# lh3/psmc

Measured on AMD Instinct MI355X. Metric: genome bins/sec through forward-backward (n=64), higher is better.
Workload: dtype f64; 1 GPU; configs[2]: whole-genome .psmcfa-like batch, 30000001 bins x 64 states in 90 segments per GPU, -p 4+25*2+4+6, one E-step (EM iteration) per step, parameters of a different EM round every step; mode=fast, bins_per_gpu=30000001, bins_total=30000001, n_states=64, segments=90, longest_segment=2490000, tiles=8127, speculative_overlap_bins=3072, structured_sweeps=True, tile_bins=3712

## Files before the change

### psmc_amd/csrc/api.hip

```cpp
#include "psmc_hip_ctx.h"

static void destroy_kids(psmc_hip_ctx *c);

static int make_streams(psmc_hip_ctx *c)
{
	hipStream_t *st[5] = {&c->stream, &c->stream2, &c->stream3, &c->stream4, &c->stream5};
	for (hipStream_t *s : st) if (*s) { (void)hipStreamSynchronize(*s); (void)hipStreamDestroy(*s); *s = nullptr; }
	if (c->cu_count <= 0) {
		for (hipStream_t *s : st) if (hipStreamCreateWithFlags(s, hipStreamNonBlocking) != hipSuccess) return PSMC_HIP_EDEVICE;
		return 0;
	}
	int cus = 0;
	if (hipDeviceGetAttribute(&cus, hipDeviceAttributeMultiprocessorCount, c->device) != hipSuccess || cus <= 0) return PSMC_HIP_EDEVICE;
	if (c->cu_first < 0 || c->cu_first + c->cu_count > cus) return PSMC_HIP_EINVAL;
	std::vector<uint32_t> mask((size_t)(cus + 31) / 32, 0u);
	for (int i = c->cu_first; i < c->cu_first + c->cu_count; ++i) mask[(size_t)i >> 5] |= 1u << (i & 31);
	for (hipStream_t *s : st) if (hipExtStreamCreateWithCUMask(s, (uint32_t)mask.size(), mask.data()) != hipSuccess) return PSMC_HIP_EDEVICE;
	return 0;
}

extern "C" int psmc_hip_device_cus(int device)
{
	int cus = 0;
	if (hipDeviceGetAttribute(&cus, hipDeviceAttributeMultiprocessorCount, device) != hipSuccess) { (void)hipGetLastError(); return 0; }
// ... 29 lines not shown
extern "C" int psmc_hip_device_count(void)
{
	int n = 0;
	if (hipGetDeviceCount(&n) != hipSuccess) return 0;
	return n;
}

extern "C" const char *psmc_hip_strerror(int err)
{
	switch (err) {
	case PSMC_HIP_OK: return "ok";
	case PSMC_HIP_EINVAL: return "invalid argument";
	case PSMC_HIP_ENOMEM: return "out of memory";
	case PSMC_HIP_EDEVICE: return "HIP runtime error";
	case PSMC_HIP_ENOTSUP: return "not supported in this build";
	case PSMC_HIP_ESTATE: return "call order violated";
	case PSMC_HIP_ECONVERGE: return "fast-mode tile boundaries did not converge";
	default: return "unknown error";
	}
}
extern "C" const char *psmc_hip_last_error(const psmc_hip_ctx *ctx) { return ctx ? ctx->err.c_str() : ""; }

extern "C" int psmc_hip_create(psmc_hip_ctx **out, int n_states, int device, int mode)
{
	if (!out) return PSMC_HIP_EINVAL;
	*out = nullptr;
	if (n_states < 1) return PSMC_HIP_EINVAL;
	if (mode != PSMC_HIP_MODE_EXACT && mode != PSMC_HIP_MODE_FAST) return PSMC_HIP_EINVAL;
	if (n_states > PSMC_HIP_MAX_STATES) return PSMC_HIP_ENOTSUP;
	int nd = psmc_hip_device_count();
	if (nd <= 0 || device < 0 || device >= nd) return PSMC_HIP_EDEVICE;
	if (hipSetDevice(device) != hipSuccess) return PSMC_HIP_EDEVICE;
	psmc_hip_ctx *c = new (std::nothrow) psmc_hip_ctx();
	if (!c) return PSMC_HIP_ENOMEM;
	c->n = n_states; c->ns = n_states > 128 ? (n_states + 63) / 64 * 64 : (n_states > 64 ? 128 : 64); c->device = device; c->mode = mode;
	c->par_len = c->ns > 128 ? 2 * (size_t)c->ns * c->ns + 4 * (size_t)c->ns : psmc_hip_ctx::PAR_LEN;
	if (make_streams(c) != 0) { psmc_hip_destroy(c); return PSMC_HIP_EDEVICE; }
	for (int i = 0; i < 14; ++i)
		if (hipEventCreate(&c->evx[i]) != hipSuccess) { delete c; return PSMC_HIP_EDEVICE; }
	for (int i = 0; i < 10; ++i)
		if (hipEventCreate(&c->ev[i]) != hipSuccess) { delete c; return PSMC_HIP_EDEVICE; }
	if (hipHostMalloc((void **)&c->h_par, c->par_len * sizeof(double), hipHostMallocDefault) != hipSuccess ||
	    hipMalloc((void **)&c->d_par, c->par_len * sizeof(double)) != hipSuccess) {
		psmc_hip_destroy(c);
		return PSMC_HIP_ENOMEM;
	}
	if (const char *env = getenv("PSMC_HIP_OPTIONS")) {
		std::string all(env);
		size_t at = 0;
		while (at < all.size()) {
			size_t end = all.find(',', at);
			if (end == std::string::npos) end = all.size();
			const std::string kv = all.substr(at, end - at);
			const size_t eq = kv.find('=');
			at = end + 1;
			if (kv.empty()) continue;
			char *endp = nullptr;
			const double val = eq == std::string::npos ? 0.0 : strtod(kv.c_str() + eq + 1, &endp);
			const bool parsed = eq != std::string::npos && eq + 1 < kv.size() && endp && *endp == '\0';
			if (parsed && kv.compare(0, eq, "rccl") == 0) continue;
			if (!parsed || psmc_hip_set_option(c, kv.substr(0, eq).c_str(), val) != PSMC_HIP_OK) {
				fprintf(stderr, "[psmc_hip] PSMC_HIP_OPTIONS: bad entry \"%s\" (unknown key, value out of range, or not a number)\n", kv.c_str());
				psmc_hip_destroy(c);
				return PSMC_HIP_EINVAL;
			}
		}
	}
	*out = c;
	return PSMC_HIP_OK;
}

static void destroy_kids(psmc_hip_ctx *c)
{
	if (c->x_twin) { psmc_hip_destroy(c->x_twin); c->x_twin = nullptr; }
	for (psmc_hip_ctx *k : c->kids) psmc_hip_destroy(k);
	c->kids.clear();
	c->share_T = 0;
}

extern "C" void psmc_hip_destroy(psmc_hip_ctx *c)
{
	if (!c) return;
	(void)hipSetDevice(c->device);
	destroy_kids(c);
	if (c->parent) {
		void *mine[] = {c->d_seg_off, c->d_seg_len, c->d_work, c->d_chunks, c->d_entry, c->d_bexit, c->d_Cpart, c->d_Epart, c->d_LLpart,
		                c->d_stage, c->d_stats, c->d_warm, c->d_bentry, c->d_dirty, c->d_cnt, c->d_gate, c->d_queue, c->d_touch, c->d_items, c->d_ftiles, c->d_Kcol,
		                c->d_segA, c->d_segE, c->d_segA0, c->d_chk};
		for (void *p : mine) if (p) (void)hipFree(p);
		if (c->h_cnt) (void)hipHostFree(c->h_cnt);
		if (c->h_ritems) (void)hipHostFree(c->h_ritems);
		if (c->h_mlen) (void)hipHostFree(c->h_mlen);
		if (c->h_chunks) (void)hipHostFree(c->h_chunks);
		if (c->h_mis) (void)hipHostFree(c->h_mis);
		if (c->d_prevx) (void)hipFree(c->d_prevx);
		if (c->d_finv) (void)hipFree(c->d_finv);
		delete c;
		return;
	}
	if (c->stream) (void)hipStreamSynchronize(c->stream);
	free_wide_fast(c);
	if (c->stream2) (void)hipStreamSynchronize(c->stream2);
	if (c->stream3) (void)hipStreamSynchronize(c->stream3);
	if (c->stream4) (void)hipStreamSynchronize(c->stream4);
	if (c->stream5) (void)hipStreamSynchronize(c->stream5);
	if (!c->obs_borrowed && c->d_obs) (void)hipFree(c->d_obs);
	void *ptrs[] = {c->d_seg_off, c->d_seg_len, c->d_work, c->d_par, c->d_f, c->d_b, c->d_s, c->d_segA, c->d_segE,
	                c->d_segA0, c->d_chk, c->d_chunks, c->d_entry, c->d_bexit, c->d_Cpart, c->d_Epart, c->d_LLpart,
	                c->d_stage, c->d_stats, c->d_warm, c->d_bentry, c->d_dirty, c->d_cnt, c->d_gate, c->d_queue, c->d_touch, c->d_sb, c->d_items, c->d_ftiles, c->d_Kcol,
	                c->d_bw_seg, c->d_bw_par, c->d_bw_tab, c->d_bpar, c->d_s_all, c->d_cu_mask, c->d_lkp, c->d_lkoff, c->d_b2};
	for (void *p : ptrs) if (p) (void)hipFree(p);
	if (c->h_par) (void)hipHostFree(c->h_par);
	if (c->h_cnt) (void)hipHostFree(c->h_cnt);
	if (c->h_ritems) (void)hipHostFree(c->h_ritems);
	if (c->h_mlen) (void)hipHostFree(c->h_mlen);
	if (c->h_chunks) (void)hipHostFree(c->h_chunks);
	if (c->h_mis) (void)hipHostFree(c->h_mis);
	if (c->d_prevx) (void)hipFree(c->d_prevx);
	if (c->d_finv) (void)hipFree(c->d_finv);
	for (int i = 0; i < 10; ++i) if (c->ev[i]) (void)hipEventDestroy(c->ev[i]);
	for (int i = 0; i < 14; ++i) if (c->evx[i]) (void)hipEventDestroy(c->evx[i]);
	if (c->stream4) (void)hipStreamDestroy(c->stream4);
	if (c->stream5) (void)hipStreamDestroy(c->stream5);
	if (c->stream2) (void)hipStreamDestroy(c->stream2);
	if (c->stream3) (void)hipStreamDestroy(c->stream3);
	if (c->stream) (void)hipStreamDestroy(c->stream);
	delete c;
}

extern "C" int psmc_hip_set_option(psmc_hip_ctx *c, const char *key, double v)
{
	if (!c || !key) return PSMC_HIP_EINVAL;
	std::string k(key);
	if (k == "batch_first") { if (v < 0 || v > 1e6) return PSMC_HIP_EINVAL; c->batch_first = (int)v; return PSMC_HIP_OK; }
	destroy_kids(c);
	if (k == "chunk") { if (v < 0) return PSMC_HIP_EINVAL; c->chunk = (int)v; c->plan_dirty = true; }
	else if (k == "warmup") { if (v < 0) return PSMC_HIP_EINVAL; c->warmup = (int)v; c->warmup_set = true; c->plan_dirty = true; }
	else if (k == "max_rounds") c->max_rounds = (int)v;
	else if (k == "structured") { c->struct_opt = v != 0 ? 1 : 0; }
	else if (k == "learn") { c->learn = v != 0 ? 1 : 0; }
	else if (k == "merge") { c->merge = v != 0 ? 1 : 0; c->plan_dirty = true; c->chunk_cap = 0; }
	else if (k == "adapt") { c->adapt = v != 0 ? 1 : 0; c->plan_dirty = true; c->chunk_cap = 0; }
	else if (k == "prev_start") { c->prev_start = v != 0 ? 1 : 0; c->prev_ok = false; c->plan_dirty = true; c->chunk_cap = 0; }
	else if (k == "warm_shift") { if (v < 0 || v > 4) return PSMC_HIP_EINVAL; c->warm_shift = (int)v; c->warm_shift_set = true; c->plan_dirty = true; }
	else if (k == "merge1") { if (v < -1 || v > 1) return PSMC_HIP_EINVAL; c->merge1 = (int)v; c->plan_dirty = true; }
	else if (k == "phase1") { if (v < -1 || v > 1) return PSMC_HIP_EINVAL; c->phase1 = (int)v; }
	else if (k == "phase1_waves") { if (v < 1 || v > 4) return PSMC_HIP_EINVAL; c->phase1_waves = (int)v; }
	else if (k == "lanes8") { if (v < -1 || v > 1) return PSMC_HIP_EINVAL; c->lanes8 = (int)v; }
	else if (k == "gap_tiles") { c->gap_tiles = v != 0 ? 1 : 0; c->plan_dirty = true; c->items_dirty = true; }
	else if (k == "coarse") { if (v < -1 || v > 16) return PSMC_HIP_EINVAL; c->coarse = (int)v; c->plan_dirty = true; c->items_dirty = true; }
	else if (k == "kc_sub") { if (v < 1 || v > 16) return PSMC_HIP_EINVAL; c->kc_sub = (int)v; c->kc_sub_set = true; c->plan_dirty = true; c->items_dirty = true; }
	else if (k == "two_phase") { if (v != -1 && v != 0 && v != 2) return PSMC_HIP_EINVAL; c->two_phase = (int)v; c->plan_dirty = true; c->items_dirty = true; }
	else if (k == "kc_min") { if (v < -1) return PSMC_HIP_EINVAL; c->kc_min = (int)v; c->items_dirty = true; }
	else if (k == "ckpt") { c->ckpt = v != 0 ? 1 : 0; }
	else if (k == "fuse") { c->fuse = v != 0 ? 1 : 0; c->plan_dirty = true; }
	else if (k == "fuse128") { if (v != 0 && v != 2) return PSMC_HIP_EINVAL; c->fuse128 = (int)v; c->plan_dirty = true; c->items_dirty = true; }
	else if (k == "group_cap") { if (v < 0) return PSMC_HIP_EINVAL; c->group_cap = (int)v; c->items_dirty = true; }
	else if (k == "share_learn") { c->share_learn = v != 0 ? 1 : 0; }
	else if (k == "exact_refwd") { if (v < -1 || v > 2) return PSMC_HIP_EINVAL; c->exact_refwd = (int)v; c->reserved_refwd = -1; c->reserved_cap = 0; if (c->d_b2) { (void)hipFree(c->d_b2); c->d_b2 = nullptr; c->b2_bins = c->b2_alloc = 0; } }
	else if (k == "batch_sort") { c->batch_sort = v != 0 ? 1 : 0; }
	else if (k == "batch_tailfill") c->batch_tailfill = v != 0;
	else if (k == "batch_major") c->batch_major = v != 0;
	else if (k == "batch_bins") { if (v < 0) return PSMC_HIP_EINVAL; c->batch_bins = (int64_t)v; }
	else if (k == "overlap") c->overlap = v != 0 ? 1 : 0;
	else if (k == "warm_tol") c->warm_tol = v;
	else if (k == "wide_fast") { if (v != 0 && v != 1) return PSMC_HIP_EINVAL; c->wide_fast = (int)v; }
	else if (k == "wide_decode") { if (v != 0 && v != 1) return PSMC_HIP_EINVAL; c->wide_decode = (int)v; }
	else if (k == "rep_impl") c->rep_impl = v < 0 ? -1 : (v != 0 ? 1 : 0);
	else return PSMC_HIP_EINVAL;
	return PSMC_HIP_OK;
}

int set_segments_common(psmc_hip_ctx *c, int n_seg, const int32_t *L)
{
	destroy_kids(c);
	c->reserved_refwd = -1; c->reserved_cap = 0;
	if (c->d_b2) { (void)hipFree(c->d_b2); c->d_b2 = nullptr; c->b2_bins = c->b2_alloc = 0; }
	c->n_seg = n_seg;
	c->L.assign(L, L + n_seg);
	int rc;
	if ((rc = dev_alloc(c, &c->d_seg_off, (size_t)n_seg))) return rc;
	if ((rc = dev_alloc(c, &c->d_seg_len, (size_t)n_seg))) return rc;
	HIPCHK(c, hipMemcpy(c->d_seg_off, c->off.data(), sizeof(int64_t) * n_seg, hipMemcpyHostToDevice));
	HIPCHK(c, hipMemcpy(c->d_seg_len, c->L.data(), sizeof(int32_t) * n_seg, hipMemcpyHostToDevice));
	std::vector<int32_t> all(n_seg);
	for (int i = 0; i < n_seg; ++i) all[i] = i;
	return psmc_hip_select(c, n_seg, all.data());
}

extern "C" int psmc_hip_load_segments(psmc_hip_ctx *c, int n_seg, const uint8_t *const *seq, const int32_t *L)
{
	if (!c || n_seg < 1 || !seq || !L) return fail(c, PSMC_HIP_EINVAL, "load_segments: bad argument");
	HIPCHK(c, hipSetDevice(c->device));
	c->off.resize(n_seg);
	int64_t tot = 0;
	for (int i = 0; i < n_seg; ++i) {
		if (L[i] < 1 || !seq[i]) return fail(c, PSMC_HIP_EINVAL, "load_segments: empty segment");
		c->off[i] = tot;
		tot += ((int64_t)L[i] + 63) & ~(int64_t)63;
	}
	c->total = tot;
	std::vector<uint8_t> host((size_t)tot + 256, 2);
	for (int i = 0; i < n_seg; ++i) {
		for (int32_t j = 0; j < L[i]; ++j)
			if (seq[i][j] > 2) return fail(c, PSMC_HIP_EINVAL, "load_segments: symbol outside {0,1,2}");
		memcpy(host.data() + c->off[i], seq[i], (size_t)L[i]);
	}
	if (!c->obs_borrowed && c->d_obs) { (void)hipFree(c->d_obs); }
	c->d_obs = nullptr; c->obs_borrowed = false;
	int rc;
	if ((rc = dev_alloc(c, &c->d_obs, host.size()))) return rc;
	HIPCHK(c, hipMemcpy(c->d_obs, host.data(), host.size(), hipMemcpyHostToDevice));
	return set_segments_common(c, n_seg, L);
}

extern "C" int psmc_hip_load_segments_device(psmc_hip_ctx *c, int n_seg, const void *d_obs, const int64_t *off,
                                             const int32_t *L)
{
	if (!c || n_seg < 1 || !d_obs || !off || !L) return fail(c, PSMC_HIP_EINVAL, "load_segments_device: bad argument");
	HIPCHK(c, hipSetDevice(c->device));
	int64_t end = 0;
	for (int i = 0; i < n_seg; ++i) {
		if (L[i] < 1 || (off[i] & 63) || off[i] < end) return fail(c, PSMC_HIP_EINVAL, "load_segments_device: bad layout");
		end = off[i] + (((int64_t)L[i] + 63) & ~(int64_t)63);
	}
	if (!c->obs_borrowed && c->d_obs) (void)hipFree(c->d_obs);
	c->d_obs = (uint8_t *)d_obs; c->obs_borrowed = true;
	c->off.assign(off, off + n_seg);
	c->total = end;
	return set_segments_common(c, n_seg, L);
}

extern "C" int psmc_hip_select(psmc_hip_ctx *c, int n_sel, const int32_t *idx)
{
	if (!c || n_sel < 1 || !idx) return fail(c, PSMC_HIP_EINVAL, "select: bad argument");
	if (c->n_seg < 1) return fail(c, PSMC_HIP_ESTATE, "select: no segments loaded");
	std::vector<int32_t> pos(c->n_seg, -1);
	c->sel.assign(idx, idx + n_sel);
	c->work.clear(); c->mult.clear(); c->sel2work.resize(n_sel);
	for (int i = 0; i < n_sel; ++i) {
		if (idx[i] < 0 || idx[i] >= c->n_seg) return fail(c, PSMC_HIP_EINVAL, "select: index out of range");
		if (pos[idx[i]] < 0) { pos[idx[i]] = (int32_t)c->work.size(); c->work.push_back(idx[i]); c->mult.push_back(0); }
		c->sel2work[i] = pos[idx[i]];
		c->mult[pos[idx[i]]]++;
	}
	HIPCHK(c, hipSetDevice(c->device));
	int rc;
	if ((rc = dev_alloc(c, &c->d_work, c->work.size()))) return rc;
	HIPCHK(c, hipMemcpy(c->d_work, c->work.data(), sizeof(int32_t) * c->work.size(), hipMemcpyHostToDevice));
	c->plan_dirty = true;
	++c->sel_serial;
	return PSMC_HIP_OK;
}

bool factor_structure(int n, int S, const double *a , double *sp )
{
	double *P = sp, *R = sp + S, *qa = sp + 2 * S, *cc = sp + 3 * S, *dd = sp + 4 * S;
	memset(sp, 0, 5 * (size_t)S * sizeof(double));
	if (n < 3) return false;
	const double pl = a[(n - 1) * S + 0], pu = a[0 * S + (n - 1)];
	if (!(pl > 1e-280) || !(pu > 1e-280)) return false;
	for (int l = 0; l < n - 1; ++l) qa[l] = a[(n - 1) * S + l] / pl;
	for (int k = 1; k < n; ++k) P[k] = a[k * S + 0];
	for (int l = 1; l < n; ++l) cc[l] = a[0 * S + l] / pu;
	for (int k = 0; k < n - 1; ++k) R[k] = a[k * S + (n - 1)];
	const double tol = 64 * 2.220446049250313e-16;
	for (int k = 0; k < n; ++k) {
		for (int l = 0; l < n; ++l) {
			if (l == k) continue;
			const double v = a[k * S + l], w = l < k ? P[k] * qa[l] : R[k] * cc[l];
			if (!(fabs(v - w) <= tol * fabs(v) + 1e-290)) return false;
		}
		dd[k] = a[k * S + k] - P[k] * qa[k] - R[k] * cc[k];
		if (!(dd[k] >= 0.0)) return false;
	}
	return true;
}

static void fill_kcc(int S, const double *sp, const double *e3 , double *out )
{
	const double *P = sp, *R = sp + S, *qa = sp + 2 * S, *cv = sp + 3 * S, *dd = sp + 4 * S;
	for (int dir = 0; dir < 2; ++dir) {
		double *t = out + (size_t)dir * 11 * S;
		const double *mS = dir == 0 ? P : cv, *wS = dir == 0 ? qa : R, *mP = dir == 0 ? R : qa, *wP = dir == 0 ? cv : P;
		for (int k = 0; k < S; ++k) { t[k] = mS[k]; t[S + k] = mP[k]; }
		for (int sy = 0; sy < 3; ++sy)
			for (int k = 0; k < S; ++k) {
				const double ev = e3[sy * S + k];
				double *u = t + 2 * S + (size_t)sy * 3 * S;
				u[k] = wS[k] * ev; u[S + k] = wP[k] * ev; u[2 * S + k] = dd[k] * ev;
			}
	}
}

bool fill_params(const psmc_hip_ctx *c, const double *a, const double *e, const double *a0, double *dst)
{
	const int n = c->n;
	if (c->ns > 128) {
		const size_t S = (size_t)c->ns;
		double *pa = dst, *pt = pa + S * S, *pe = pt + S * S, *pa0 = pe + 3 * S;
		memset(pa, 0, c->par_len * sizeof(double));
		for (int k = 0; k < n; ++k) {
			for (int l = 0; l < n; ++l) { pa[k * S + l] = a[(size_t)k * n + l]; pt[l * S + k] = a[(size_t)k * n + l]; }
			pe[k] = e[k]; pe[S + k] = e[n + k];
			pa0[k] = a0[k];
		}
// ... 298 lines not shown
```

### psmc_amd/csrc/api_batch.hip

```cpp
#include "psmc_hip_ctx.h"

namespace {
struct RepSel { std::vector<int32_t> work, sel2work; int64_t bins = 0; };
}

static int batch_selections(psmc_hip_ctx *c, int n_rep, const int32_t *sel_off, const int32_t *sel_idx, std::vector<RepSel> &reps)
{
	std::vector<int32_t> pos(c->n_seg);
	reps.assign(n_rep, RepSel());
	for (int r = 0; r < n_rep; ++r) {
		const int n_sel = sel_off[r + 1] - sel_off[r];
		if (n_sel < 1) return fail(c, PSMC_HIP_EINVAL, "estep_batch: empty selection");
		std::fill(pos.begin(), pos.end(), -1);
		RepSel &R = reps[r];
		R.sel2work.resize(n_sel);
		for (int i = 0; i < n_sel; ++i) {
			const int32_t sg = sel_idx[sel_off[r] + i];
			if (sg < 0 || sg >= c->n_seg) return fail(c, PSMC_HIP_EINVAL, "estep_batch: index out of range");
			if (pos[sg] < 0) { pos[sg] = (int32_t)R.work.size(); R.work.push_back(sg); R.bins += ((int64_t)c->L[sg] + 63) & ~(int64_t)63; }
			R.sel2work[i] = pos[sg];
		}
	}
	return 0;
}
// ... 225 lines not shown
		}
		if (c->bpar_cap < (size_t)n_rep) { if ((rc = dev_alloc(c, &c->d_bpar, (size_t)n_rep * PL))) return rc; c->bpar_cap = (size_t)n_rep; }
		if (refwd && !c->d_cu_mask && (rc = dev_alloc(c, &c->d_cu_mask, (size_t)4096))) return rc;
		size_t lk_worst = 0;
		for (int g = 0; g < n_launches; ++g) {
			size_t t = 0;
			for (int i = l_first[g]; i < l_first[g + 1]; ++i) t += wseg[i] >= 0 ? (size_t)(c->L[wseg[i]] / LKP_DIV + LKP_MIN) : 1;
			lk_worst = std::max(lk_worst, t);
		}
		if (c->lkp_cap < lk_worst) { if ((rc = dev_alloc(c, &c->d_lkp, lk_worst))) return rc; c->lkp_cap = lk_worst; }
		if (c->lkoff_cap < worst_entries) { if ((rc = dev_alloc(c, &c->d_lkoff, worst_entries))) return rc; c->lkoff_cap = worst_entries; }
		if (fwd_all && c->s_all_cap < (size_t)all_bins + 128) { if ((rc = dev_alloc(c, &c->d_s_all, (size_t)all_bins + 128))) return rc; c->s_all_cap = (size_t)all_bins + 128; }
	}
	static const bool dbg_t = getenv("PSMC_HIP_DEBUG_TIMES") != nullptr;
	auto now = []() { return dbg_now(); };
	{
		std::vector<double> hp((size_t)n_rep * PL);
		for (int r = 0; r < n_rep; ++r) (void)fill_params(c, a + (size_t)r * n * n, e + (size_t)r * 2 * n, a0 + (size_t)r * n, hp.data() + (size_t)r * PL);
		HIPCHK(c, hipStreamSynchronize(c->stream));
		HIPCHK(c, hipMemcpyAsync(c->d_bw_seg, wseg.data(), sizeof(int32_t) * n_all, hipMemcpyHostToDevice, c->stream));
		HIPCHK(c, hipMemcpyAsync(c->d_bw_par, wpar.data(), sizeof(int32_t) * n_all, hipMemcpyHostToDevice, c->stream));
		HIPCHK(c, hipMemcpyAsync(c->d_bw_tab, wtab.data(), sizeof(int64_t) * n_all, hipMemcpyHostToDevice, c->stream));
		HIPCHK(c, hipMemcpyAsync(c->d_bw_tab + n_all, wtab_s.data(), sizeof(int64_t) * n_all, hipMemcpyHostToDevice, c->stream));
		HIPCHK(c, hipMemcpyAsync(c->d_bpar, hp.data(), sizeof(double) * hp.size(), hipMemcpyHostToDevice, c->stream));
		HIPCHK(c, hipStreamSynchronize(c->stream));
	}
	c->tables_batch = true;
	double fwd_all_s = 0.0;
	if (fwd_all) {
		const double t0 = now();
		EstepLaunch p;
		fill_common(c, p, c->stream, c->d_bpar);
		p.d_work = c->d_bw_seg; p.n_work = n_all; p.d_work_par = c->d_bw_par; p.d_work_tab = c->d_bw_tab + n_all; p.par_stride = (int64_t)PL; p.work_align = align;
		p.exact_refwd = 1; p.exact_only = 1; p.d_s = c->d_s_all;
		if (launch_exact(p) != 0) return fail(c, PSMC_HIP_EDEVICE, "launch_exact (batch, forward pass of all entries)", hipGetLastError());
		if (dbg_t) { (void)hipStreamSynchronize(c->stream); fwd_all_s = now() - t0; }
	}
	if ((double)n_all * (double)(S * S) * 8.0 > 16e9) {
		c->err = "estep_batch: the per-entry statistics of this call (" + std::to_string(n_all) + " entries x " + std::to_string(S) + "^2 doubles) need more than 16 GB of host memory: send fewer replicates per call at this many states";
		return PSMC_HIP_ENOMEM;
	}
	c->h_segA.resize((size_t)n_all * S * S); c->h_segE.resize((size_t)n_all * 3 * S);
	std::vector<double> lk_all((size_t)n_all, 0.0);
	std::vector<int> last_launch(n_rep, 0);
	{
		std::vector<int> launch_of((size_t)n_all, 0);
		for (int g = 0; g < n_launches; ++g) for (int i = l_first[g]; i < l_first[g + 1]; ++i) launch_of[i] = g;
		for (int r = 0; r < n_rep; ++r) for (int w : ent_of[r]) if (w >= 0) last_launch[r] = std::max(last_launch[r], launch_of[w]);
	}
	std::vector<double> sA((size_t)n * n), sE((size_t)2 * n);
	double t_sums = 0.0;
	auto finalize = [&](int r) {
		const RepSel &R = reps[r];
		std::fill(sA.begin(), sA.end(), 0.0); std::fill(sE.begin(), sE.end(), 0.0);
		double ll = 0.0;
		for (size_t i = 0; i < R.sel2work.size(); ++i) {
			const int w = ent_of[r][R.sel2work[i]];
			const double *hA = &c->h_segA[(size_t)w * S * S], *hE = &c->h_segE[(size_t)w * 3 * S];
			ll += lk_all[(size_t)w];
			for (int k = 0; k < n; ++k)
				for (int l = 0; l < n; ++l) sA[(size_t)k * n + l] += hA[k * S + l];
			for (int b = 0; b < 2; ++b)
				for (int l = 0; l < n; ++l) sE[(size_t)b * n + l] += hE[b * S + l];
		}
		if (A) memcpy(A + (size_t)r * n * n, sA.data(), sizeof(double) * n * n);
		if (E) memcpy(E + (size_t)r * 2 * n, sE.data(), sizeof(double) * 2 * n);
		if (LL) LL[r] = ll;
		if (sums) {
			double *q = sums + (size_t)r * 5 * n;
			memset(q, 0, sizeof(double) * 5 * n);
			for (int k = 0; k < n; ++k)
				for (int l = 0; l < n; ++l) {
					const double v = sA[(size_t)k * n + l];
					if (l < k) { q[k] += v; q[3 * n + l] += v; } else if (l > k) { q[n + k] += v; q[4 * n + l] += v; } else q[2 * n + k] = v;
				}
		}
	};
	std::vector<int32_t> finished;
	for (int g = 0; g < n_launches; ++g) {
		const double t_a = now();
		const int e0 = l_first[g], nw = l_first[g + 1] - e0;
		int64_t run = 0; int32_t longest = 0;
		for (int i = e0; i < e0 + nw; ++i) if (wseg[i] >= 0) { run = std::max(run, wtab[i] + padded_len(wseg[i])); longest = std::max(longest, c->L[wseg[i]]); }
		EstepLaunch p;
		fill_common(c, p, c->stream, c->d_bpar);
		p.d_work = c->d_bw_seg + e0; p.n_work = nw; p.d_work_par = c->d_bw_par + e0; p.d_work_tab = c->d_bw_tab + e0; p.par_stride = (int64_t)PL; p.work_align = align;
		p.exact_refwd = refwd ? (c->exact_refwd == 1 ? 1 : 2) : 0;
		p.d_cu_mask = c->d_cu_mask;
		if (fwd_all) { p.exact_only = 2; p.d_work_tab_s = c->d_bw_tab + n_all + e0; p.d_s = c->d_s_all; }
		p.d_segA = c->d_segA; p.d_segE = c->d_segE; p.d_segA0 = c->d_segA0; p.d_chk = c->d_chk;
		const double t_b = now();
		if (launch_exact(p) != 0) return fail(c, PSMC_HIP_EDEVICE, "launch_exact (batch)", hipGetLastError());
		if (dbg_t) (void)hipStreamSynchronize(c->stream);
		const double t_c = now();
		std::vector<int64_t> lkoff((size_t)nw);
		int64_t lk_tot = 0;
		for (int i = 0; i < nw; ++i) { lkoff[i] = lk_tot; lk_tot += wseg[e0 + i] >= 0 ? c->L[wseg[e0 + i]] / LKP_DIV + LKP_MIN : 1; }
		HIPCHK(c, hipMemcpyAsync(c->d_lkoff, lkoff.data(), sizeof(int64_t) * nw, hipMemcpyHostToDevice, c->stream));
		if (launch_lk_products(c->stream, p, fwd_all ? c->d_s_all : c->d_s, c->d_lkoff, c->d_lkp) != 0) return fail(c, PSMC_HIP_EDEVICE, "launch_lk_products", hipGetLastError());
		c->h_lkp.resize((size_t)lk_tot);
		HIPCHK(c, hipMemcpyAsync(c->h_segA.data() + (size_t)e0 * S * S, c->d_segA, sizeof(double) * nw * S * S, hipMemcpyDeviceToHost, c->stream));
		HIPCHK(c, hipMemcpyAsync(c->h_segE.data() + (size_t)e0 * 3 * S, c->d_segE, sizeof(double) * nw * 3 * S, hipMemcpyDeviceToHost, c->stream));
		HIPCHK(c, hipMemcpyAsync(c->h_lkp.data(), c->d_lkp, sizeof(double) * (size_t)lk_tot, hipMemcpyDeviceToHost, c->stream));
		HIPCHK(c, hipStreamSynchronize(c->stream));
		const double t_d = now();
		collect_timing(c);
		int n_over = 0;
		for (int i = 0; i < nw; ++i) {
			if (wseg[e0 + i] < 0) continue;
			const int32_t sg = wseg[e0 + i];
			const double *q = &c->h_lkp[(size_t)lkoff[i]];
			const int cnt = (int)q[0], cap_i = c->L[sg] / LKP_DIV + LKP_MIN;
			if (cnt >= 1 && cnt < cap_i) {
				double sum = 0.0;
				for (int j = 1; j <= cnt; ++j) sum += log(q[j]);
				lk_all[(size_t)e0 + i] = sum;
			} else {
				++n_over;
				c->h_s.resize((size_t)c->L[sg]);
				HIPCHK(c, hipMemcpyAsync(c->h_s.data(), (fwd_all ? c->d_s_all + wtab_s[e0 + i] : c->d_s + wtab[e0 + i]), sizeof(double) * (size_t)c->L[sg], hipMemcpyDeviceToHost, c->stream));
				HIPCHK(c, hipStreamSynchronize(c->stream));
				lk_all[(size_t)e0 + i] = host_lk(c->h_s.data(), c->L[sg]);
			}
		}
		if (dbg_t && n_over) fprintf(stderr, "[psmc_hip] batch launch %d: %d entries logged more products than their buffer holds (host hmm_lk)\n", g, n_over);
		if (dbg_t) fprintf(stderr, "[psmc_hip] batch launch %d: %d entries (longest %d bins), %.1f M table bins | prepare %.3f s, kernels %.3f (fwd %.0f bwd %.0f expect %.0f ms%s), read-back %.3f, hmm_lk %.3f\n",
		                   g, nw, (int)longest, run / 1e6, t_b - t_a, t_c - t_b, c->last_ms[1], c->last_ms[2], c->last_ms[3],
		                   fwd_all ? (g == 0 ? (std::string("; forward pass of all entries ") + std::to_string(fwd_all_s) + " s").c_str() : "; fwd: see launch 0") : "", t_d - t_c, now() - t_d);
		++c->last_batch_groups;
		const double t_f = now();
		finished.clear();
		for (int r = 0; r < n_rep; ++r) if (last_launch[r] == g) { finalize(r); finished.push_back(r); }
		t_sums += now() - t_f;
		if (done && !finished.empty()) done(user, (int)finished.size(), finished.data());
	}
	if (dbg_t) {
		std::string per;
		for (int g = 0; g < n_launches; ++g) per += (g ? " " : "") + std::to_string(std::count(last_launch.begin(), last_launch.end(), g));
		fprintf(stderr, "[psmc_hip] batch: %d replicates, %d entries in %d launches (replicates complete after launch 0..: %s), host sums %.3f s\n", n_rep, n_all, n_launches, per.c_str(), t_sums);
	}
	return PSMC_HIP_OK;
}

static psmc_hip_ctx *batch_child(psmc_hip_ctx *c, int r)
{
	while ((int)c->kids.size() <= r) {
		psmc_hip_ctx *k = new (std::nothrow) psmc_hip_ctx();
		if (!k) return nullptr;
		k->n = c->n; k->ns = c->ns; k->device = c->device; k->mode = c->mode; k->parent = c;
		k->chunk = c->chunk > 0 ? c->chunk : c->share_T;
		k->warmup = c->warmup; k->max_rounds = c->max_rounds; k->rep_impl = c->rep_impl;
		k->n_sub = c->n_sub; k->target_waves = c->target_waves; k->overlap = c->overlap; k->warm_tol = c->warm_tol; k->struct_opt = c->struct_opt;
		k->struct_tiles_set = c->struct_tiles_set; k->struct_tiles = c->struct_tiles;
		k->two_phase = c->two_phase; k->kc_div = c->kc_div; k->kc_min = c->kc_min; k->ckpt = c->ckpt; k->fuse = c->fuse;
		k->learn = c->learn; k->group_cap = c->group_cap; k->warm_shift = c->warm_shift; k->kc_sub = c->kc_sub; k->kcol_prio = c->kcol_prio;
		k->fuse128 = c->fuse128; k->coarse = c->coarse; k->gate = c->gate; k->lanes8 = c->lanes8; k->gap_tiles = c->gap_tiles; k->exact_refwd = c->exact_refwd;
		k->merge = c->merge; k->adapt = c->adapt; k->prev_start = c->prev_start;
		k->merge1 = c->merge1; k->merge_order = c->merge_order; k->runs_late = c->runs_late; k->warm_shift_set = c->warm_shift_set; k->kc_sub_set = c->kc_sub_set;
		k->stream = c->stream; k->stream2 = c->stream2; k->stream3 = c->stream3; k->stream4 = c->stream4; k->stream5 = c->stream5;
		for (int i = 0; i < 14; ++i) k->evx[i] = c->evx[i];
		for (int i = 0; i < 10; ++i) k->ev[i] = c->ev[i];
		k->h_par = c->h_par; k->d_par = c->d_par; k->par_len = c->par_len;
		k->d_obs = c->d_obs; k->obs_borrowed = true; k->off = c->off; k->total = c->total;
		if (set_segments_common(k, c->n_seg, c->L.data()) != 0) { c->err = k->err; psmc_hip_destroy(k); return nullptr; }
		c->kids.push_back(k);
	}
	return c->kids[r];
}

static int batch_exact_once(psmc_hip_ctx *c, int r, const int32_t *idx, int n_sel, const double *a, const double *e, const double *a0,
                            double *A, double *sums, double *E, double *LL, const char *why)
{
	const int n = c->n;
	fprintf(stderr, "[psmc_hip] replicate %d: fast E-step did not converge (%s); repeating this E-step with the exact kernels\n", c->batch_first + r, why);
	int rc = 0;
	if (!c->x_twin) {
		if ((rc = psmc_hip_create(&c->x_twin, n, c->device, PSMC_HIP_MODE_EXACT))) return fail(c, rc, "estep_batch: cannot create the exact twin context");
		if ((rc = psmc_hip_load_segments_device(c->x_twin, c->n_seg, c->d_obs, c->off.data(), c->L.data()))) {
			c->err = "exact twin: " + c->x_twin->err; psmc_hip_destroy(c->x_twin); c->x_twin = nullptr; return rc;
		}
	}
	std::vector<double> Af;
	double *Ao = A;
	if (!Ao) { Af.resize((size_t)n * n); Ao = Af.data(); }
	if ((rc = psmc_hip_select(c->x_twin, n_sel, idx)) || (rc = psmc_hip_estep(c->x_twin, a, e, a0, Ao, E, nullptr, LL, nullptr))) { c->err = "exact twin: " + c->x_twin->err; return rc; }
	if (sums) {
		memset(sums, 0, sizeof(double) * 5 * (size_t)n);
		for (int k = 0; k < n; ++k)
			for (int l = 0; l < n; ++l) {
				const double v = Ao[(size_t)k * n + l];
				if (l < k) { sums[k] += v; sums[3 * n + l] += v; } else if (l > k) { sums[n + k] += v; sums[4 * n + l] += v; } else sums[2 * n + k] = v;
			}
	}
	++c->n_exact_fallbacks;
	return PSMC_HIP_OK;
}

static int batch_fast(psmc_hip_ctx *c, int n_rep, const double *a, const double *e, const double *a0, const int32_t *sel_off,
                      const int32_t *sel_idx, double *A, double *sums, double *E, double *LL, psmc_hip_batch_done_fn done, void *user)
{
	const int n = c->n;
	if (c->share_T == 0 && c->share_learn) {
		int T = c->chunk;
		if (T <= 0) {
			std::vector<RepSel> reps;
			int rc0 = batch_selections(c, n_rep, sel_off, sel_idx, reps);
			if (rc0) return rc0;
			int64_t most = 0; size_t nw = 1;
			for (const RepSel &R : reps) {
				int64_t bins = 0;
				for (int32_t sg : R.work) bins += c->L[sg];
				if (bins > most) { most = bins; nw = R.work.size(); }
			}
			T = auto_tile_len(c, most, nw, true);
		}
		c->share_T = T;
		c->sh_glue_f.assign(c->n_seg, {}); c->sh_glue_b.assign(c->n_seg, {}); c->sh_wf.assign(c->n_seg, {}); c->sh_wb.assign(c->n_seg, {});
		for (int sg = 0; sg < c->n_seg; ++sg) {
			const size_t nt = ((size_t)c->L[sg] + T - 1) / T;
			c->sh_glue_f[sg].assign(nt, 0); c->sh_glue_b[sg].assign(nt, 0); c->sh_wf[sg].assign(nt, c->warmup); c->sh_wb[sg].assign(nt, c->warmup);
		}
	}
	static const bool dbg_t = getenv("PSMC_HIP_DEBUG_TIMES") != nullptr;
	const double t_call = dbg_now();
	double t_est = 0.0;
	for (int r = 0; r < n_rep; ++r) {
		const double t_k = dbg_now();
		psmc_hip_ctx *k = batch_child(c, c->batch_first + r);
		c->dbg_acc[0] += dbg_now() - t_k;
		if (!k) return fail(c, PSMC_HIP_ENOMEM, "estep_batch: cannot create the replicate context");
		const int n_sel = sel_off[r + 1] - sel_off[r];
		if (n_sel < 1) return fail(c, PSMC_HIP_EINVAL, "estep_batch: empty selection");
		const int32_t *idx = sel_idx + sel_off[r];
		int rc = 0;
		{
			const double t_s = dbg_now();
			if ((int)k->sel.size() != n_sel || memcmp(k->sel.data(), idx, sizeof(int32_t) * n_sel) != 0) rc = psmc_hip_select(k, n_sel, idx);
			c->dbg_acc[1] += dbg_now() - t_s;
		}
		const double t_e = dbg_now();
		const double *ar = a + (size_t)r * n * n, *er = e + (size_t)r * 2 * n, *a0r = a0 + (size_t)r * n;
		if (rc == 0) {
			double *Ar = A ? A + (size_t)r * n * n : nullptr, *Sr = sums ? sums + (size_t)r * 5 * n : nullptr, *Er = E ? E + (size_t)r * 2 * n : nullptr, *Lr = LL ? LL + r : nullptr;
			if (A) rc = psmc_hip_estep(k, ar, er, a0r, Ar, Er, nullptr, Lr, nullptr);
			if (rc == 0 && sums) rc = psmc_hip_estep_factored(k, ar, er, a0r, Sr, Er, Lr);
			if (rc == PSMC_HIP_ECONVERGE) rc = batch_exact_once(c, r, idx, n_sel, ar, er, a0r, Ar, Sr, Er, Lr, k->err.c_str());
		}
		t_est += dbg_now() - t_e;
		if (rc) { c->err = "replicate " + std::to_string(r) + ": " + k->err; return rc; }
		if (done) { const int32_t rr = r; done(user, 1, &rr); }
	}
	if (dbg_t) {
		const double *q = c->dbg_acc;
		fprintf(stderr, "[psmc_hip] fast batch on device %d: %d replicates %.3f s | contexts %.3f, select %.3f, E-steps %.3f (plan %.3f, items %.3f, launches %.3f, rest %.3f); "
		                "%.0f repair rounds, %.0f repaired tiles\n", c->device, n_rep, dbg_now() - t_call, q[0], q[1], t_est, q[2], q[3], q[4], t_est - q[2] - q[3] - q[4], q[6], q[7]);
		for (double &v : c->dbg_acc) v = 0.0;
	}
	c->tables_batch = true;
	c->last_batch_groups = n_rep;
	return PSMC_HIP_OK;
}

extern "C" int psmc_hip_estep_batch(psmc_hip_ctx *c, int n_rep, const double *a, const double *e, const double *a0,
                                    const int32_t *sel_off, const int32_t *sel_idx, double *A, double *sums, double *E, double *LL)
{
	return psmc_hip_estep_batch_cb(c, n_rep, a, e, a0, sel_off, sel_idx, A, sums, E, LL, nullptr, nullptr);
}

extern "C" int psmc_hip_estep_batch_cb(psmc_hip_ctx *c, int n_rep, const double *a, const double *e, const double *a0,
                                       const int32_t *sel_off, const int32_t *sel_idx, double *A, double *sums, double *E, double *LL,
                                       psmc_hip_batch_done_fn done, void *user)
{
	if (!c || n_rep < 1 || !a || !e || !a0 || !sel_off || !sel_idx || (!A && !sums)) return fail(c, PSMC_HIP_EINVAL, "estep_batch: bad argument");
	if (c->parent) return fail(c, PSMC_HIP_EINVAL, "estep_batch: not on a replicate context");
	if (c->n_seg < 1) return fail(c, PSMC_HIP_ESTATE, "estep_batch: no segments loaded");
	HIPCHK(c, hipSetDevice(c->device));
	c->wd_kind = WD_NONE;
	if (c->mode == PSMC_HIP_MODE_EXACT || c->ns > 128) return batch_exact(c, n_rep, a, e, a0, sel_off, sel_idx, A, sums, E, LL, done, user);
	return batch_fast(c, n_rep, a, e, a0, sel_off, sel_idx, A, sums, E, LL, done, user);
}

extern "C" int psmc_hip_batch_info(psmc_hip_ctx *c, int out[2])
{
	if (!c || !out) return PSMC_HIP_EINVAL;
	out[0] = c->last_batch_groups; out[1] = (int)c->kids.size();
	return PSMC_HIP_OK;
}
```

### psmc_amd/csrc/api_fast.hip

```cpp
#include "psmc_hip_ctx.h"

int ensure_fast_buffers(psmc_hip_ctx *c)
{
	if (c->d_stage && c->d_stats && c->d_warm && c->d_cnt && c->h_cnt && c->d_gate) return 0;
	int rc;
	const size_t sl = (size_t)c->ns * c->ns + 3 * (size_t)c->ns + 1;
	if ((rc = dev_alloc(c, &c->d_stage, (size_t)RED_ROWS * sl))) return rc;
	if ((rc = dev_alloc(c, &c->d_stats, sl))) return rc;
	if ((rc = dev_alloc(c, &c->d_warm, (size_t)2))) return rc;
	if ((rc = dev_alloc(c, &c->d_cnt, (size_t)4))) return rc;
	if ((rc = dev_alloc(c, &c->d_gate, (size_t)4))) return rc;
	if (!c->h_cnt && (hipHostMalloc((void **)&c->h_cnt, 4 * sizeof(int), hipHostMallocMapped) != hipSuccess ||
	                  hipHostGetDevicePointer((void **)&c->m_cnt, c->h_cnt, 0) != hipSuccess)) {
		c->h_cnt = nullptr;
		return fail(c, PSMC_HIP_ENOMEM, "hipHostMalloc (mapped)");
	}
	return 0;
}

int auto_tile_len(const psmc_hip_ctx *c, int64_t bins, size_t n_work, bool st)
{
	const int64_t ROUND1 = 4096;
	int64_t want = st ? c->struct_tiles : c->target_waves;
	if (st && !c->struct_tiles_set && bins < 2 * ROUND1 * (int64_t)std::max(c->warmup, 1))
		want = std::max<int64_t>(ROUND1 - (int64_t)n_work, ROUND1 / 2);
	const int T = (int)((bins + want - 1) / want);
	return std::max(256, (T + 63) & ~63);
}

static int plan_fast(psmc_hip_ctx *c)
{
	int64_t bins = 0;
	for (int32_t s : c->work) bins += c->L[s];
	int T = c->chunk;
	const bool st = c->use_struct;
	const int64_t ROUND1 = 4096;
	bool one_round = false;
	if (T <= 0) T = auto_tile_len(c, bins, c->work.size(), st);
	c->chunks.clear(); c->chunk_seg.clear(); c->chunk_idx.clear();
	for (size_t w = 0; w < c->work.size(); ++w) {
		const int32_t s = c->work[w];
		for (int32_t lo = 1; lo <= c->L[s]; lo += T) {
			c->chunk_seg.push_back(s); c->chunk_idx.push_back((lo - 1) / T);
			Chunk ch;
			ch.off = c->off[s]; ch.L = c->L[s]; ch.lo = lo; ch.hi = std::min(c->L[s], lo + T - 1); ch.mult = c->mult[w];
			ch.flags = 0; ch.wf = ch.wb = c->warmup;
			if (ch.lo - c->warmup <= 1) ch.flags |= CHUNK_ANCHOR_F;
			if ((int64_t)ch.hi + c->warmup + 1 >= ch.L) ch.flags |= CHUNK_ANCHOR_B;
			if (ch.hi == ch.L) ch.flags |= CHUNK_LAST;
			c->chunks.push_back(ch);
		}
	}
	const int nc = (int)c->chunks.size();
	c->chunk_used = T;
	c->planned_struct = st;
	one_round = st && nc <= ROUND1;
	c->two_phase_used = c->two_phase >= 0 ? c->two_phase : (one_round ? 0 : 2);
	c->merge1_used = c->merge1 >= 0 ? c->merge1 : (one_round ? 1 : 0);
	c->warm_shift_used = c->warm_shift_set ? c->warm_shift : (one_round ? 0 : 1);
	c->coarse_used = c->coarse >= 0 ? std::max(c->coarse, 1) : (one_round && nc > 2048 && T < c->warmup ? 2 : 1);
	c->kc_sub_used = c->kc_sub_set ? c->kc_sub : std::max(1, std::min(4, (int)((8 * (int64_t)T + T + c->warmup - 1) / std::max(T + c->warmup, 1))));
	c->n_sub_used = st ? (fused_counts(c) ? 1 : std::max(1, std::min(c->n_sub, (9216 + nc - 1) / std::max(nc, 1)))) : c->n_sub;
	c->glue_f.assign(nc, 0); c->glue_b.assign(nc, 0);
	if (c->parent && c->parent->share_T == T && st) {
		const psmc_hip_ctx *P = c->parent;
		for (int b = 0; b < nc; ++b) {
			const int sg = c->chunk_seg[b], ix = c->chunk_idx[b];
			if (sg >= (int)P->sh_glue_f.size() || ix >= (int)P->sh_glue_f[sg].size()) continue;
			c->glue_f[b] = P->sh_glue_f[sg][ix]; c->glue_b[b] = P->sh_glue_b[sg][ix];
			c->chunks[b].wf = std::max(c->chunks[b].wf, P->sh_wf[sg][ix]); c->chunks[b].wb = std::max(c->chunks[b].wb, P->sh_wb[sg][ix]);
		}
	}
	c->items_dirty = true;
	int rc;
	c->gap.assign(nc, 0);
	if (nc > c->chunk_cap) {
		if ((rc = dev_alloc(c, &c->d_chunks, (size_t)nc))) return rc;
		if ((rc = dev_alloc(c, &c->d_entry, (size_t)nc * c->ns))) return rc;
		if ((rc = dev_alloc(c, &c->d_bexit, (size_t)(nc + 1) * c->ns))) return rc;
		if ((rc = dev_alloc(c, &c->d_bentry, (size_t)nc * c->ns))) return rc;
		if ((rc = dev_alloc(c, &c->d_dirty, (size_t)2 * nc))) return rc;
		if ((rc = dev_alloc(c, &c->d_touch, (size_t)3 * nc))) return rc;
		if ((rc = dev_alloc(c, &c->d_finv, (size_t)nc))) return rc;
		if (c->h_mlen) { (void)hipHostFree(c->h_mlen); c->h_mlen = nullptr; c->m_mlen = nullptr; }
		if (c->h_mis) { (void)hipHostFree(c->h_mis); c->h_mis = nullptr; c->m_mis = nullptr; }
		if (c->prev_start && (rc = dev_alloc(c, &c->d_prevx, (size_t)nc * c->ns))) return rc;
		if ((c->merge || c->adapt) &&
		    (hipHostMalloc((void **)&c->h_mlen, (size_t)nc * sizeof(int), hipHostMallocMapped) != hipSuccess ||
		     hipHostGetDevicePointer((void **)&c->m_mlen, c->h_mlen, 0) != hipSuccess ||
		     hipHostMalloc((void **)&c->h_mis, (size_t)2 * nc * sizeof(double), hipHostMallocMapped) != hipSuccess ||
		     hipHostGetDevicePointer((void **)&c->m_mis, c->h_mis, 0) != hipSuccess))
			return fail(c, PSMC_HIP_ENOMEM, "hipHostMalloc (mapped)");
		if ((rc = dev_alloc(c, &c->d_LLpart, (size_t)nc))) return rc;
		if ((rc = dev_alloc(c, &c->d_items, (size_t)32 * nc + 64))) return rc;
		if ((rc = dev_alloc(c, &c->d_ftiles, (size_t)2 * (nc + 16)))) return rc;
		if (c->h_ritems) { (void)hipHostFree(c->h_ritems); c->h_ritems = nullptr; }
		if (hipHostMalloc((void **)&c->h_ritems, (size_t)4 * nc * sizeof(int), hipHostMallocMapped) != hipSuccess ||
		    hipHostGetDevicePointer((void **)&c->m_ritems, c->h_ritems, 0) != hipSuccess)
			return fail(c, PSMC_HIP_ENOMEM, "hipHostMalloc (mapped)");
		c->chunk_cap = nc;
	}
	if ((rc = dev_alloc(c, &c->d_Epart, (size_t)nc * c->n_sub_used * 3 * c->ns))) return rc;
	if ((rc = ensure_fast_buffers(c))) return rc;
	HIPCHK(c, hipMemcpy(c->d_chunks, c->chunks.data(), sizeof(Chunk) * nc, hipMemcpyHostToDevice));
	if (st && c->gap_tiles) {
		std::vector<int> fl(nc, 0);
		if (launch_tile_allmiss(c->stream, c->d_obs, c->d_chunks, nc, c->d_dirty) != 0) return fail(c, PSMC_HIP_EDEVICE, "k_tile_allmiss", hipGetLastError());
		HIPCHK(c, hipMemcpyAsync(fl.data(), c->d_dirty, sizeof(int) * nc, hipMemcpyDeviceToHost, c->stream));
		HIPCHK(c, hipMemsetAsync(c->d_dirty, 0, sizeof(int) * nc, c->stream));
		HIPCHK(c, hipStreamSynchronize(c->stream));
		for (int b = 0; b < nc; ++b) {
			const Chunk &ch = c->chunks[b];
			c->gap[b] = fl[b] && ch.lo > 1 && ch.hi < ch.L && ch.hi - ch.lo + 1 == T;
		}
		auto same = [&](int x, int y) { return x >= 0 && y < nc && c->chunks[x].off == c->chunks[y].off; };
		for (int b = 0; b < nc; ++b) {
			if (c->gap[b]) { if (same(b - 1, b)) c->glue_f[b] = 1; if (same(b, b + 1)) c->glue_b[b] = 1; }
			if (b > 0 && c->gap[b - 1] && same(b - 1, b)) c->glue_f[b] = 1;
			if (b + 1 < nc && c->gap[b + 1] && same(b, b + 1)) c->glue_b[b] = 1;
		}
	}
	c->plan_dirty = false; c->chunks_dirty = false; c->prev_ok = false;
	return 0;
}

static int build_items(psmc_hip_ctx *c, bool two_phase_bwd, int coarse)
{
	const int nc = (int)c->chunks.size(), W = c->warmup;
	const int cf = std::max(1, coarse), cb = two_phase_bwd ? 1 : cf;
	std::vector<int> odd(nc, 0), idx(nc, 0);
	for (int b = 1; b < nc; ++b) if (c->chunks[b].off == c->chunks[b - 1].off) { odd[b] = !odd[b - 1]; idx[b] = idx[b - 1] + 1; }
	std::vector<std::pair<long long, std::pair<int, int>>> kf, kb;
	auto key = [](int steps, bool run, bool phase_b) { return (run ? -(1ll << 40) : (phase_b ? (1ll << 40) : 0ll)) - steps; };
	std::vector<char> from_above(nc, 0), in_run(nc, 0), in_run_f(nc, 0), in_run_b(nc, 0);
	std::vector<std::pair<int, int>> gf, gb;
	auto same_seg = [&](int x, int y) { return c->chunks[x].off == c->chunks[y].off; };
	const bool gaps = c->gap_tiles && (int)c->gap.size() == nc;
	std::vector<int64_t> eff(nc + 1, 0);
	for (int b = 0; b < nc; ++b) eff[b + 1] = eff[b] + ((gaps && c->gap[b]) ? 0 : c->chunks[b].hi - c->chunks[b].lo + 1);
	auto span_ok = [&](int b, int e) { return eff[e + 1] - eff[b] <= (int64_t)c->group_cap; };
	for (int b = 0; b < nc;) {
		int e = b + 1;
		while (e < nc && c->glue_f[e] && same_seg(e, b) && span_ok(b, e)) ++e;
		if (e - b > 1) for (int t = b; t < e; ++t) in_run[t] = in_run_f[t] = 1;
		else
			while (e < nc && e - b < cf && same_seg(e, b) && idx[e] % cf != 0 && !c->glue_f[e] && !(e + 1 < nc && c->glue_f[e + 1] && same_seg(e + 1, e))) ++e;
		gf.push_back({b, e - b});
		b = e;
	}
	for (int b = 0; b < nc;) {
		int e = b + 1;
		while (e < nc && c->glue_b[e - 1] && same_seg(e, b) && span_ok(b, e) &&
		       c->chunks[e].lo < c->chunks[e].L)
			++e;
		if (e - b > 1) for (int t = b; t < e; ++t) in_run[t] = in_run_b[t] = 1;
		else
			while (e < nc && e - b < cb && same_seg(e, b) && idx[e] % cb != 0 && !c->glue_b[e - 1] && !(e + 1 < nc && c->glue_b[e] && same_seg(e + 1, e)) &&
			       c->chunks[e].lo < c->chunks[e].L)
				++e;
		gb.push_back({b, e - b});
		b = e;
	}
	int n_run = 0;
	for (int b = 0; b < nc; ++b) n_run += in_run[b];
	const int cap_b = (nc + 7) / 8 * 4;
	c->runs_in_b = two_phase_bwd && c->runs_late && n_run > 0 && n_run <= cap_b / 2;
	int above_budget = c->runs_in_b ? cap_b - n_run : nc;
	for (const auto &gr : gb) {
		const int b = gr.first, e = b + gr.second;
		const Chunk &lo = c->chunks[b], &top = c->chunks[e - 1];
		bool pb = two_phase_bwd && e - b == 1 && odd[b] && b + 1 < nc && c->chunks[b + 1].off == lo.off && c->chunks[b + 1].lo < c->chunks[b + 1].L;
		if (pb && c->runs_in_b && (in_run[b] || in_run[b + 1] || above_budget <= 0)) pb = false;
		if (pb) { from_above[b] = 1; --above_budget; }
		kb.push_back({key(std::min(top.hi + chunk_warm_b(top, W) + 1, top.L) - lo.lo, in_run_b[b] != 0, pb), {b, e - b}});
	}
	std::vector<int> la, lb;
	{
		std::vector<int> freet;
		for (int b = 0; b < nc; ++b) {
			if (from_above[b]) lb.push_back(b | (1 << 30));
			else if (b > 0 && from_above[b - 1]) la.push_back(b);
			else if (c->runs_in_b && in_run[b]) lb.push_back(b);
			else freet.push_back(b);
		}
		const bool single = lb.empty() && nc <= 4096;
		for (int b : freet) { if (single || la.size() <= lb.size()) la.push_back(b); else lb.push_back(b); }
	}
	for (const auto &gr : gf) {
		const int b = gr.first, e = b + gr.second;
		const Chunk &h = c->chunks[b], &l = c->chunks[e - 1];
		kf.push_back({key(l.hi - std::max(1, h.lo - chunk_warm_f(h, W)) + 1, in_run_f[b] != 0, false), {b, e - b}});
	}
	std::sort(kf.begin(), kf.end()); std::sort(kb.begin(), kb.end());
	std::vector<int> h((size_t)4 * nc, 0), mem((size_t)4 * nc, 0);
	c->n_mem_f = c->n_mem_b = 0;
	for (size_t i = 0; i < kf.size(); ++i) {
		h[2 * i] = kf[i].second.first; h[2 * i + 1] = kf[i].second.second;
		if (in_run_f[kf[i].second.first])
			for (int t = 0; t < kf[i].second.second; ++t) { mem[2 * (size_t)c->n_mem_f] = kf[i].second.first + t; mem[2 * (size_t)c->n_mem_f + 1] = 1; ++c->n_mem_f; }
	}
	for (size_t i = 0; i < kb.size(); ++i) {
		h[(size_t)2 * nc + 2 * i] = kb[i].second.first; h[(size_t)2 * nc + 2 * i + 1] = kb[i].second.second;
		if (in_run_b[kb[i].second.first])
			for (int t = 0; t < kb[i].second.second; ++t) {
				mem[(size_t)2 * nc + 2 * (size_t)c->n_mem_b] = kb[i].second.first + t; mem[(size_t)2 * nc + 2 * (size_t)c->n_mem_b + 1] = 1; ++c->n_mem_b;
			}
	}
	c->n_items_f = (int)kf.size(); c->n_items_b = (int)kb.size();
	c->order_f.clear();
	for (const auto &it : kf) if (!in_run_f[it.second.first]) c->order_f.push_back(it.second.first);
	c->n_long_f = c->n_long_b = 0;
	while (c->n_long_f < c->n_items_f && in_run_f[kf[c->n_long_f].second.first]) ++c->n_long_f;
	while (c->n_long_b < c->n_items_b && in_run_b[kb[c->n_long_b].second.first]) ++c->n_long_b;
	c->n_B_b = 0;
	for (int b = 0; b < nc; ++b) c->n_B_b += from_above[b];
	{
		c->n_list_a = (int)la.size(); c->n_list_b = (int)lb.size();
		c->count_group = c->ns == 128 && c->fuse128 == 2 ? 16 : 4;
		while (la.size() % c->count_group) la.push_back(-1);
		while (lb.size() % c->count_group) lb.push_back(-1);
		la.insert(la.end(), lb.begin(), lb.end());
		if (!la.empty()) HIPCHK(c, hipMemcpy(c->d_ftiles, la.data(), sizeof(int) * la.size(), hipMemcpyHostToDevice));
	}
	c->items_two_phase = two_phase_bwd ? 2 : 0; c->items_coarse = coarse;
	HIPCHK(c, hipMemcpy(c->d_items, h.data(), sizeof(int) * h.size(), hipMemcpyHostToDevice));
	{
		std::vector<int> sg;
		for (size_t i = (size_t)c->n_long_b; i < kb.size(); ++i)
			for (int t = kb[i].second.second - 1; t >= 0; --t) { sg.push_back(kb[i].second.first + t); sg.push_back(1); }
		c->n_singles_b = (int)sg.size() / 2;
		if (!sg.empty()) HIPCHK(c, hipMemcpy(c->d_items + (size_t)24 * nc, sg.data(), sizeof(int) * sg.size(), hipMemcpyHostToDevice));
	}
	HIPCHK(c, hipMemcpy(c->d_items + (size_t)8 * nc, mem.data(), sizeof(int) * mem.size(), hipMemcpyHostToDevice));
	{
		std::vector<int> fx;
		for (int b = 0; b < nc; ++b)
			if (!in_run_f[b] && !(b > 0 && in_run_f[b - 1] && same_seg(b - 1, b))) { fx.push_back(b); fx.push_back(1); }
		c->n_fix_f = (int)fx.size() / 2;
		if (!fx.empty()) HIPCHK(c, hipMemcpy(c->d_items + (size_t)30 * nc, fx.data(), sizeof(int) * fx.size(), hipMemcpyHostToDevice));
	}
	{
		const int n4f = c->n_items_f - c->n_long_f, n4b = c->n_items_b - c->n_long_b - c->n_B_b;
		std::vector<std::pair<long long, int>> qk;
		for (int k = 0; 4 * k < n4f; ++k) {
			long long st = 0;
			for (int i = c->n_long_f + 4 * k; i < std::min(c->n_long_f + 4 * k + 4, c->n_items_f); ++i) {
				const Chunk &h = c->chunks[kf[i].second.first], &l = c->chunks[kf[i].second.first + kf[i].second.second - 1];
				st = std::max(st, (long long)(l.hi - std::max(1, h.lo - chunk_warm_f(h, W)) + 1));
			}
			qk.push_back({-st * 504, 2 * k});
		}
		for (int k = 0; 4 * k < n4b; ++k) {
			long long st = 0;
			for (int i = c->n_long_b + 4 * k; i < std::min(c->n_long_b + 4 * k + 4, c->n_long_b + n4b); ++i) {
				const Chunk &lo = c->chunks[kb[i].second.first], &top = c->chunks[kb[i].second.first + kb[i].second.second - 1];
				const int q = std::min(top.hi + chunk_warm_b(top, W) + 1, top.L);
				st = std::max(st, (long long)(q - (coarse > 1 ? std::min(lo.hi, lo.L - 1) : std::min(top.hi, top.L - 1))));
			}
			qk.push_back({-st * 534, 2 * k + 1});
		}
		std::stable_sort(qk.begin(), qk.end(), [](const std::pair<long long, int> &x, const std::pair<long long, int> &y) { return x.first < y.first; });
		std::vector<int> qv(qk.size());
		for (size_t i = 0; i < qk.size(); ++i) qv[i] = qk[i].second;
		if (c->queue_cap < qv.size()) { int rc; if ((rc = dev_alloc(c, &c->d_queue, qv.size()))) return rc; c->queue_cap = qv.size(); }
		c->n_queue = (int)qv.size();
		if (!qv.empty()) HIPCHK(c, hipMemcpy(c->d_queue, qv.data(), sizeof(int) * qv.size(), hipMemcpyHostToDevice));
	}
	std::vector<int> wl((size_t)4 * nc, 0), kc, runs_f, runs_b, kslot, kuniq;
	int gap_slot[2] = {-1, -1};
	auto push_kc = [&](int t, int dir) {
		const int j = (int)kc.size() / 2;
		kc.push_back(t); kc.push_back(dir);
		if (gaps && c->gap[t] && c->chunk_used % 4 == 0) {
			if (gap_slot[dir] < 0) { gap_slot[dir] = (int)kuniq.size(); kuniq.push_back(j); }
			kslot.push_back(gap_slot[dir]);
		} else { kslot.push_back((int)kuniq.size()); kuniq.push_back(j); }
	};
	c->n_wl_f = c->n_wl_b = 0;
	const int kc_min = c->kc_min >= 0 ? c->kc_min : (c->ns == 128 ? (nc > 4096 ? 12 : 8) : (nc > 4096 ? 5 : 4));
	const bool chains = kc_min >= 2;
	const int head_count = c->ns == 64 ? 0 : 1;
	auto add_runs = [&](const std::vector<std::pair<long long, std::pair<int, int>>> &k, int n_long, bool bwd) {
		int &nw = bwd ? c->n_wl_b : c->n_wl_f;
		std::vector<int> &rv = bwd ? runs_b : runs_f;
		int *w = wl.data() + (bwd ? (size_t)2 * nc : 0);
		int budget = std::max(64, nc / c->kc_div);
		for (int i = 0; i < n_long; ++i) {
			int first = k[i].second.first, count = k[i].second.second;
			int cost = 0;
			for (int tt = first; tt < first + count; ++tt) cost += (gaps && c->gap[tt] && c->chunk_used % 4 == 0) ? 0 : 1;
			cost = std::max(cost - 1, 1);
			const bool chain = chains && count >= kc_min && cost <= budget;
			if (chain) budget -= cost;
			if (chain && !bwd && c->chunks[first].lo == 1) {
				w[2 * nw] = first; w[2 * nw + 1] = (head_count == 0 && count - 1 >= 2) ? -1 : 2; ++nw;
				first += 1; count -= 1;
				if (count >= 2) {
					rv.push_back(first); rv.push_back(count); rv.push_back((int)(kc.size() / 2)); rv.push_back(0);
					for (int t = first; t < first + count - 1; ++t) push_kc(t, 0);
				}
			} else if (chain) {
				w[2 * nw] = bwd ? first + count - 1 : first; w[2 * nw + 1] = head_count; ++nw;
				rv.push_back(first); rv.push_back(count); rv.push_back((int)(kc.size() / 2)); rv.push_back(0);
				if (!bwd) for (int t = first; t < first + count - 1; ++t) push_kc(t, 0);
				else for (int t = first + count - 1; t > first; --t) push_kc(t, 1);
			} else { w[2 * nw] = first; w[2 * nw + 1] = (head_count == 0 && !bwd) ? -(count - 1) : count; ++nw; }
		}
	};
	add_runs(kf, c->n_long_f, false);
	add_runs(kb, c->n_long_b, true);
	c->n_chain_f = (int)runs_f.size() / 4; c->n_chain_b = (int)runs_b.size() / 4; c->n_kc = (int)kc.size() / 2; c->n_kuniq = (int)kuniq.size();
	if ((size_t)c->n_kc > (size_t)2 * nc || (size_t)(c->n_chain_f + c->n_chain_b) > (size_t)nc) return fail(c, PSMC_HIP_ESTATE, "build_items: list overflow");
	HIPCHK(c, hipMemcpy(c->d_items + (size_t)12 * nc, wl.data(), sizeof(int) * wl.size(), hipMemcpyHostToDevice));
	if (c->n_kc > 0) {
		std::vector<int> runs(runs_f); runs.insert(runs.end(), runs_b.begin(), runs_b.end());
		HIPCHK(c, hipMemcpy(c->d_items + (size_t)16 * nc, kc.data(), sizeof(int) * kc.size(), hipMemcpyHostToDevice));
		HIPCHK(c, hipMemcpy(c->d_items + (size_t)20 * nc, runs.data(), sizeof(int) * runs.size(), hipMemcpyHostToDevice));
		HIPCHK(c, hipMemcpy(c->d_items + (size_t)26 * nc, kslot.data(), sizeof(int) * kslot.size(), hipMemcpyHostToDevice));
		HIPCHK(c, hipMemcpy(c->d_items + (size_t)28 * nc, kuniq.data(), sizeof(int) * kuniq.size(), hipMemcpyHostToDevice));
		const size_t nsub = kcol2_on(c) ? (size_t)c->kc_sub_used : 1;
		const size_t need = (size_t)c->n_kuniq * nsub * ((size_t)c->ns * c->ns + c->ns);
		if (need > c->kcol_cap) { int rc; if ((rc = dev_alloc(c, &c->d_Kcol, need))) return rc; c->kcol_cap = need; }
	}
	c->items_dirty = false;
	if (getenv("PSMC_HIP_DEBUG"))
		fprintf(stderr, "[psmc_hip] buffers: obs %p (+%lld) chunks %p (%d) items %p entry %p bentry %p bexit %p f %p b %p s %p sb %p Cpart %p Epart %p ftiles %p touch %p par %p Kcol %p\n",
		        (void *)c->d_obs, (long long)c->total + 256, (void *)c->d_chunks, nc, (void *)c->d_items, (void *)c->d_entry, (void *)c->d_bentry, (void *)c->d_bexit,
		        (void *)c->d_f, (void *)c->d_b, (void *)c->d_s, (void *)c->d_sb, (void *)c->d_Cpart, (void *)c->d_Epart, (void *)c->d_ftiles, (void *)c->d_touch, (void *)c->d_par, (void *)c->d_Kcol);
	if (getenv("PSMC_HIP_DEBUG"))
		fprintf(stderr, "[psmc_hip] items: %d tiles of %d bins, fwd %d items (%d runs, %d run tiles, %d walks, %d chains), bwd %d items (%d runs, %d run tiles, %d walks, %d chains, %d from above), %d transfer matrices, fused lists %d + %d\n",
		        nc, c->chunk_used, c->n_items_f, c->n_long_f, c->n_mem_f, c->n_wl_f, c->n_chain_f, c->n_items_b, c->n_long_b, c->n_mem_b, c->n_wl_b, c->n_chain_b, c->n_B_b, c->n_kc, c->n_list_a, c->n_list_b);
	return 0;
}

static void learn_groups(psmc_hip_ctx *c)
{
	const int nc = (int)c->chunks.size(), W = c->warmup;
	const int cap = W << c->warm_shift_used;
	for (int b : c->flagged_f)
		if (b > 0 && b < nc && !c->glue_f[b] && c->chunks[b - 1].off == c->chunks[b].off) {
			Chunk &ch = c->chunks[b];
			if (ch.wf < cap && ch.lo - ch.wf > 1) { ch.wf = std::min(cap, std::max(2 * ch.wf, W)); c->chunks_dirty = true; }
			else c->glue_f[b] = 1;
			c->items_dirty = true;
		}
	for (int b : c->flagged_b)
		if (b >= 0 && b + 1 < nc && !c->glue_b[b] && c->chunks[b + 1].off == c->chunks[b].off) {
			Chunk &ch = c->chunks[b];
			if (ch.wb < cap && (int64_t)ch.hi + ch.wb + 1 < ch.L) { ch.wb = std::min(cap, std::max(2 * ch.wb, W)); c->chunks_dirty = true; }
			else c->glue_b[b] = 1;
			c->items_dirty = true;
		}
	if (c->parent && c->parent->share_T == c->chunk_used && (!c->flagged_f.empty() || !c->flagged_b.empty())) {
		psmc_hip_ctx *P = c->parent;
		auto put = [&](int b) {
			if (b < 0 || b >= nc) return;
			const int sg = c->chunk_seg[b], ix = c->chunk_idx[b];
			if (sg >= (int)P->sh_glue_f.size() || ix >= (int)P->sh_glue_f[sg].size()) return;
			P->sh_glue_f[sg][ix] |= c->glue_f[b]; P->sh_glue_b[sg][ix] |= c->glue_b[b];
			P->sh_wf[sg][ix] = std::max(P->sh_wf[sg][ix], c->chunks[b].wf); P->sh_wb[sg][ix] = std::max(P->sh_wb[sg][ix], c->chunks[b].wb);
		};
		for (int b : c->flagged_f) put(b);
		for (int b : c->flagged_b) put(b);
	}
}

static void adapt_warmups(psmc_hip_ctx *c)
{
	const int nc = (int)c->chunks.size();
	const int cap = c->warmup << c->warm_shift_used, floor_w = std::min(c->warmup, 256);
	const double tol = c->warm_tol;
	bool changed = false;
	for (int b = 0; b < nc; ++b) {
		const double m = c->h_mis[b];
		if (!(m > 0.0)) continue;
		if (c->glue_f[b] || (b + 1 < nc && c->glue_f[b + 1] && c->chunks[b + 1].off == c->chunks[b].off)) continue;
		Chunk &ch = c->chunks[b];
		if (ch.lo - ch.wf <= 1) continue;
		int w = ch.wf;
		if (m > tol) {
			const int ml = c->h_mlen[b];
			w = std::min(std::max(cap, w), w + (ml > 0 ? 16 * ml + 64 : w));
		} else {
			const double slack = log10(tol / std::max(m, 1e-17)), keep = 2.0;
			if (slack > keep) w = std::max(floor_w, w - (((int)std::min((slack - keep) * 160.0, w / 8.0) + 15) & ~15));
		}
		if (w != ch.wf) { ch.wf = w; changed = true; }
	}
	if (changed) {
		c->chunks_dirty = true;
		int64_t total = 0, waste = 0;
		for (size_t i = 0; i + 3 < c->order_f.size(); i += 4) {
			int64_t s4 = 0, mx = 0;
			for (int r = 0; r < 4; ++r) { const Chunk &ch = c->chunks[c->order_f[i + r]]; const int64_t st = (int64_t)ch.hi - std::max(1, ch.lo - ch.wf) + 1; s4 += st; mx = std::max(mx, st); }
			total += 4 * mx; waste += 4 * mx - s4;
		}
		if (total > 0 && waste * 100 > total * 3) c->items_dirty = true;
	}
}

int enqueue_fast(psmc_hip_ctx *c, const double *a, const double *e, const double *a0, double *d_out,
                        hipStream_t st)
{
	HIPCHK(c, hipSetDevice(c->device));
	if (c->n_seg < 1) return fail(c, PSMC_HIP_ESTATE, "estep: no segments loaded");
	int rc;
	c->dec_kind = DEC_NONE;
	const unsigned long long serial0 = dbg_root(c)->tab_serial;
	if ((rc = ensure_tables(c, false))) return rc;
	c->tables_batch = false;
	if ((rc = stage_params(c, a, e, a0, st))) return rc;
	if (!c->want_factored && !(c->use_struct && fused_counts(c)) && (rc = ensure_tables(c, true))) return rc;
	if (c->ns == 128 && !c->use_struct)
		return fail(c, PSMC_HIP_ENOTSUP, "fast mode beyond 64 states needs a transition matrix of the PSMC form (structured sweeps)");
	if (c->want_factored && !c->use_struct)
		return fail(c, PSMC_HIP_ENOTSUP, "factored statistics need a transition matrix of the PSMC form");
	{
		const double t0 = dbg_now();
		if ((c->plan_dirty || c->planned_struct != c->use_struct) && (rc = plan_fast(c))) return rc;
		dbg_root(c)->dbg_acc[2] += dbg_now() - t0;
	}
	EstepLaunch p;
	fill_common(c, p, st);
	p.d_chunks = c->d_chunks; p.n_chunks = (int)c->chunks.size(); p.warmup = c->warmup; p.n_sub = c->n_sub_used;
	const bool two_phase_bwd = c->two_phase_used >= 1 && p.fused == 1;
	p.merge1 = c->merge1_used; p.merge_order = c->merge_order >= 0 ? c->merge_order : (c->chunk_used < c->warmup ? 1 : 0);
	if (c->chunks_dirty) {
		psmc_hip_ctx *R = dbg_root(c);
		if (R->h_chunks_cap < c->chunks.size()) {
			if (R->h_chunks) { (void)hipHostFree(R->h_chunks); R->h_chunks = nullptr; }
			if (hipHostMalloc((void **)&R->h_chunks, sizeof(Chunk) * c->chunks.size(), hipHostMallocDefault) != hipSuccess) return fail(c, PSMC_HIP_ENOMEM, "hipHostMalloc");
			R->h_chunks_cap = c->chunks.size();
		}
		HIPCHK(c, hipStreamSynchronize(st));
		memcpy(R->h_chunks, c->chunks.data(), sizeof(Chunk) * c->chunks.size());
		HIPCHK(c, hipMemcpyAsync(c->d_chunks, R->h_chunks, sizeof(Chunk) * c->chunks.size(), hipMemcpyHostToDevice, st));
		c->chunks_dirty = false;
	}
	const int coarse = (c->use_struct && p.fused != 0) ? c->coarse_used : 1;
	{
		const double t0 = dbg_now();
		if (c->use_struct && (c->items_dirty || c->items_two_phase != (two_phase_bwd ? 2 : 0) || c->items_coarse != coarse) && (rc = build_items(c, two_phase_bwd, coarse))) return rc;
		dbg_root(c)->dbg_acc[3] += dbg_now() - t0;
	}
	p.lanes8 = (c->lanes8 >= 0 ? c->lanes8 != 0 && p.fused != 0 : p.fused == 2 && p.n_chunks > 4096) && c->ns == 64 ? 1 : 0;
	{
		const size_t nc_ = c->chunks.size(), S_ = (size_t)c->ns;
		const size_t need = p.fused == 2 ? nc_ * 7 * S_ + 64 : (p.fused == 1 ? (nc_ / 4 + 8) * S_ * S_ : nc_ * (size_t)c->n_sub_used * S_ * S_);
		if (c->cpart_cap < need) { if ((rc = dev_alloc(c, &c->d_Cpart, need))) return rc; c->cpart_cap = need; }
	}
	{
		c->merge_used = c->merge != 0 && c->h_mlen && c->use_struct && p.fused == 1 && c->ns == 64 && c->chunk_used % 16 == 0;
		p.merge = c->merge_used ? 1 : 0;
		p.d_fmerge = c->d_touch + 2 * (size_t)p.n_chunks; p.d_finv = c->d_finv; p.m_mlen = c->m_mlen; p.h_mlen = c->h_mlen; p.m_mis = c->m_mis;
		p.d_fix_f = c->d_items + 30 * (size_t)p.n_chunks; p.n_fix_f = c->n_fix_f;
		if (c->h_mlen) memset(c->h_mlen, 0, sizeof(int) * p.n_chunks);
		if (c->h_mis) for (int b = 0; b < p.n_chunks; ++b) c->h_mis[b] = -1.0;
		const bool prev = c->prev_start && c->d_prevx && c->prev_ok && c->use_struct && c->prev_serial == serial0 && c->prev_f == c->d_f && c->prev_ckpt == p.ckpt;
		p.d_prevx = prev ? c->d_prevx : nullptr;
		c->prev_ok = false;
	}
	p.d_gate = (c->gate >= 0 ? c->gate != 0 : coarse > 1) ? c->d_gate : nullptr;
	if (c->phase1 != 0 && c->use_struct && p.fused == 1 && c->ns == 64 && !p.lanes8 && !p.merge1 && c->overlap && c->n_queue > 0) {
		int cus = c->cu_count;
		if (cus <= 0 && (hipDeviceGetAttribute(&cus, hipDeviceAttributeMultiprocessorCount, c->device) != hipSuccess || cus <= 0)) return fail(c, PSMC_HIP_EDEVICE, "hipDeviceGetAttribute");
		p.d_queue = c->d_queue; p.n_queue = c->n_queue; p.d_qhead = c->d_gate + 2;
		p.q_grid = std::min(c->n_queue, 4 * cus * c->phase1_waves);
	}
	p.coarse = coarse; p.d_singles_b = c->d_items + 24 * (size_t)p.n_chunks; p.n_singles_b = c->n_singles_b;
	p.n_B_b = c->n_B_b; p.runs_in_b = c->runs_in_b ? 1 : 0; p.n_list_a = c->n_list_a; p.n_list_b = c->n_list_b; p.d_ftiles = c->d_ftiles; p.count_group = c->count_group;
	c->timing_two_launches = p.fused == 1 && p.n_list_b > 0;
	p.d_items_f = c->d_items; p.d_items_b = c->d_items + 2 * p.n_chunks;
	p.d_ritems_f = c->d_items + 4 * p.n_chunks; p.d_ritems_b = c->d_items + 6 * p.n_chunks;
	p.n_items_f = c->n_items_f; p.n_items_b = c->n_items_b; p.tile_len = c->chunk_used; p.h_ritems = c->h_ritems; p.m_ritems = c->m_ritems; p.m_cnt = c->m_cnt;
	c->flagged_f.clear(); c->flagged_b.clear();
	p.flagged_f = &c->flagged_f; p.flagged_b = &c->flagged_b;
	p.d_entry = c->d_entry; p.d_bentry = c->d_bentry; p.d_bexit = c->d_bexit; p.d_Cpart = c->d_Cpart; p.d_Epart = c->d_Epart;
	p.d_dirty = c->d_dirty; p.d_cnt = c->d_cnt; p.h_cnt = c->h_cnt; p.tol = c->warm_tol; p.max_rounds = c->max_rounds;
	p.d_touch_f = c->d_touch; p.d_touch_b = c->d_touch + p.n_chunks; p.d_dirty_b = c->d_dirty + p.n_chunks;
	p.stream2 = c->stream2; p.stream3 = c->stream3; p.stream4 = c->stream4; p.overlap = c->overlap;
	p.n_long_f = c->n_long_f; p.n_long_b = c->n_long_b; p.n_mem_f = c->n_mem_f; p.n_mem_b = c->n_mem_b;
	p.d_members_f = c->d_items + 8 * p.n_chunks; p.d_members_b = c->d_items + 10 * p.n_chunks;
	p.d_wl_f = c->d_items + 12 * (size_t)p.n_chunks; p.d_wl_b = c->d_items + 14 * (size_t)p.n_chunks; p.n_wl_f = c->n_wl_f; p.n_wl_b = c->n_wl_b;
	p.d_kc = c->d_items + 16 * (size_t)p.n_chunks; p.d_kruns = c->d_items + 20 * (size_t)p.n_chunks;
	p.n_kc = c->n_kc; p.n_chain_f = c->n_chain_f; p.n_chain_b = c->n_chain_b;
	p.d_kslot = c->d_items + 26 * (size_t)p.n_chunks; p.d_kuniq = c->d_items + 28 * (size_t)p.n_chunks; p.n_kuniq = c->n_kuniq;
	p.kcol_prio = c->kcol_prio;
	p.d_Kcol = c->d_Kcol; p.kc_sub = kcol2_on(c) ? c->kc_sub_used : 1;
	p.d_Kexp = c->d_Kcol ? c->d_Kcol + (size_t)c->n_kuniq * p.kc_sub * c->ns * c->ns : nullptr; p.stream5 = c->stream5;
	for (int i = 0; i < 14; ++i) p.evx[i] = c->evx[i];
	p.d_LLpart = c->d_LLpart; p.d_stage = c->d_stage; p.d_stats = d_out; p.d_warm = c->d_warm;
	p.tiny_total = (double)c->sel.size() * HMM_TINY_H;
	if (p.d_prevx) launch_gather_prev(p, st, c->n_long_f, c->n_items_f - c->n_long_f, c->d_prevx);
	{
		const double t0 = dbg_now();
		if (launch_fast(p, &c->report) != 0) return fail(c, PSMC_HIP_EDEVICE, "launch_fast", hipGetLastError());
		psmc_hip_ctx *R = dbg_root(c);
		R->dbg_acc[4] += dbg_now() - t0;
		R->dbg_acc[6] += c->report.fwd_rounds + c->report.bwd_rounds; R->dbg_acc[7] += c->report.fwd_tiles + c->report.bwd_tiles;
	}
	if (getenv("PSMC_HIP_DEBUG_FLAGGED")) {
		auto dump = [&](const char *dir, const std::vector<int> &fl, const std::vector<uint8_t> &glue, bool bwd) {
			std::vector<int> u(fl); std::sort(u.begin(), u.end()); u.erase(std::unique(u.begin(), u.end()), u.end());
			fprintf(stderr, "[psmc_hip] flagged %s: %zu tile repairs, %zu distinct tiles, rounds %d:", dir, fl.size(), u.size(), bwd ? c->report.bwd_rounds : c->report.fwd_rounds);
			for (size_t i = 0; i < u.size() && i < 400; ++i) {
				const int b = u[i]; const Chunk &ch = c->chunks[b];
				int seg = 0; while (seg + 1 < c->n_seg && c->off[seg + 1] <= ch.off) ++seg;
				fprintf(stderr, " [t%d seg%d %d..%d w%d g%d x%d m%.1e ml%d]", b, seg, ch.lo, ch.hi, bwd ? ch.wb : ch.wf, (int)glue[b], (int)std::count(fl.begin(), fl.end(), b),
				        c->h_mis ? c->h_mis[(bwd ? c->chunks.size() : 0) + b] : 0.0, (!bwd && c->h_mlen) ? c->h_mlen[b] : 0);
			}
			fprintf(stderr, "\n");
		};
		dump("fwd", c->flagged_f, c->glue_f, false); dump("bwd", c->flagged_b, c->glue_b, true);
	}
	if (!c->report.converged) return fail(c, PSMC_HIP_ECONVERGE, "fast mode: tile boundaries did not converge within max_rounds");
	if (c->merge_used && c->h_mlen)
		for (size_t b = 0; b < c->chunks.size(); ++b) {
			c->report.merged += c->h_mlen[b] > 0;
			if (c->h_mlen[b] < 0 || (c->h_mlen[b] > 0 && !c->adapt)) c->flagged_f.push_back((int)b);
		}
	if (c->use_struct && c->adapt && c->merge_used && c->h_mis) adapt_warmups(c);
	if (c->use_struct && c->learn) learn_groups(c);
	if (c->use_struct) { c->prev_ok = true; c->prev_serial = dbg_root(c)->tab_serial; c->prev_f = c->d_f; c->prev_ckpt = p.ckpt; }
	c->dec_kind = c->merge_used ? DEC_MERGED : (p.fused != 0 ? DEC_NO_BT : DEC_FAST);
	c->dec_serial = dbg_root(c)->tab_serial;
	return 0;
}

int read_warm(psmc_hip_ctx *c, hipStream_t st)
{
	unsigned long long w[2];
	HIPCHK(c, hipMemcpyAsync(w, c->d_warm, sizeof(w), hipMemcpyDeviceToHost, st));
	HIPCHK(c, hipStreamSynchronize(st));
	memcpy(&c->warm_err[0], &w[0], 8); memcpy(&c->warm_err[1], &w[1], 8);
	return 0;
}

extern "C" int psmc_hip_estep_device(psmc_hip_ctx *c, const double *a, const double *e, const double *a0,
                                     void *d_stats, void *stream)
{
	if (!c || !a || !e || !a0 || !d_stats) return fail(c, PSMC_HIP_EINVAL, "estep_device: bad argument");
	if (c->mode != PSMC_HIP_MODE_FAST) return fail(c, PSMC_HIP_ENOTSUP, "estep_device: fast mode only");
	c->timing_valid = false;
	return enqueue_fast(c, a, e, a0, (double *)d_stats, (hipStream_t)stream);
}

extern "C" int psmc_hip_fast_diag(psmc_hip_ctx *c, double *wf, double *wb, int *n_chunks, int *warmup_used)
{
	if (!c) return PSMC_HIP_EINVAL;
	if (c->mode != PSMC_HIP_MODE_FAST || !c->d_warm) return fail(c, PSMC_HIP_ESTATE, "fast_diag: no fast E-step yet");
	HIPCHK(c, hipSetDevice(c->device));
	unsigned long long w[2];
	HIPCHK(c, hipMemcpy(w, c->d_warm, sizeof(w), hipMemcpyDeviceToHost));
	memcpy(&c->warm_err[0], &w[0], 8); memcpy(&c->warm_err[1], &w[1], 8);
	if (wf) *wf = c->warm_err[0];
	if (wb) *wb = c->warm_err[1];
	if (n_chunks) *n_chunks = (int)(c->wf_ran ? c->wf_chunks.size() : c->chunks.size());
	if (warmup_used) *warmup_used = c->wf_ran ? c->wf_W : c->warmup;
	return PSMC_HIP_OK;
}

extern "C" int psmc_hip_fast_repairs(psmc_hip_ctx *c, int out[6])
{
	if (!c || !out) return PSMC_HIP_EINVAL;
	out[0] = c->report.fwd_rounds; out[1] = c->report.bwd_rounds;
	out[2] = c->report.fwd_tiles; out[3] = c->report.bwd_tiles;
	out[4] = c->report.merged; out[5] = c->report.recounted;
	return PSMC_HIP_OK;
}

void unpack_factored(const double *h, int n, double *sums, double *E, double *LL)
{
	if (sums) memcpy(sums, h, sizeof(double) * 5 * n);
	if (E) memcpy(E, h + (size_t)5 * n, sizeof(double) * 2 * n);
	if (LL) *LL = h[(size_t)7 * n];
}

extern "C" int psmc_hip_estep_factored(psmc_hip_ctx *c, const double *a, const double *e, const double *a0, double *sums,
                                       double *E, double *LL)
{
	if (!c || !a || !e || !a0) return fail(c, PSMC_HIP_EINVAL, "estep_factored: bad argument");
	if (c->mode != PSMC_HIP_MODE_FAST) return fail(c, PSMC_HIP_ENOTSUP, "estep_factored: fast mode only");
	HIPCHK(c, hipSetDevice(c->device));
	if (c->ns > 128 && c->wide_fast) return estep_factored_wide(c, a, e, a0, sums, E, LL);
	int rc;
	if ((rc = ensure_fast_buffers(c))) return rc;
	c->want_factored = true;
	rc = enqueue_fast(c, a, e, a0, c->d_stats, c->stream);
	c->want_factored = false;
	if (rc) return rc;
	if ((rc = read_warm(c, c->stream))) return rc;
	collect_timing(c);
	const int n = c->n;
	std::vector<double> h((size_t)7 * n + 1);
	HIPCHK(c, hipMemcpy(h.data(), c->d_stats, sizeof(double) * h.size(), hipMemcpyDeviceToHost));
	unpack_factored(h.data(), n, sums, E, LL);
	return PSMC_HIP_OK;
}

extern "C" int psmc_hip_estep_factored_device(psmc_hip_ctx *c, const double *a, const double *e, const double *a0, void *d_stats, void *stream)
{
	if (!c || !a || !e || !a0 || !d_stats) return fail(c, PSMC_HIP_EINVAL, "estep_factored_device: bad argument");
	if (c->mode != PSMC_HIP_MODE_FAST) return fail(c, PSMC_HIP_ENOTSUP, "estep_factored_device: fast mode only");
	HIPCHK(c, hipSetDevice(c->device));
	c->timing_valid = false;
	if (c->ns > 128 && c->wide_fast) return estep_wide_fast(c, a, e, a0, (double *)d_stats, (hipStream_t)stream);
	c->want_factored = true;
	const int rc = enqueue_fast(c, a, e, a0, (double *)d_stats, (hipStream_t)stream);
	c->want_factored = false;
	return rc;
}

extern "C" int psmc_hip_fast_info(psmc_hip_ctx *c, int out[8])
{
	if (!c || !out) return PSMC_HIP_EINVAL;
	if (c->wf_ran) {
		const int nc = (int)c->wf_chunks.size();
		out[0] = 1; out[1] = c->wf_T; out[2] = nc; out[3] = nc; out[4] = 3; out[5] = 0; out[6] = 1; out[7] = 0;
		return PSMC_HIP_OK;
	}
	out[0] = c->use_struct ? 1 : 0; out[1] = c->chunk_used; out[2] = c->use_struct ? c->n_items_f : (int)c->chunks.size();
	out[3] = c->use_struct ? c->n_items_b : (int)c->chunks.size();
	out[4] = c->last_fused; out[5] = c->last_ckpt; out[6] = c->timing_two_launches ? 2 : 1; out[7] = c->merge1_used;
	return PSMC_HIP_OK;
}

extern "C" int psmc_hip_fast_plan(psmc_hip_ctx *c, double out[8])
{
	if (!c || !out) return PSMC_HIP_EINVAL;
	if (c->plan_dirty || c->chunks.empty()) return fail(c, PSMC_HIP_ESTATE, "fast_plan: no current plan (run a fast E-step first)");
	const int nc = (int)c->chunks.size();
	double sf = 0, sb = 0, mf = 0, mb = 0; int nf = 0, nb = 0, gf = 0, gb = 0;
	for (int b = 0; b < nc; ++b) {
		const Chunk &ch = c->chunks[b];
		if (c->glue_f[b]) ++gf; else if (!(ch.flags & CHUNK_ANCHOR_F)) { sf += ch.wf; mf = std::max(mf, (double)ch.wf); ++nf; }
		if (c->glue_b[b]) ++gb; else if (!(ch.flags & (CHUNK_ANCHOR_B | CHUNK_LAST))) { sb += ch.wb; mb = std::max(mb, (double)ch.wb); ++nb; }
	}
	out[0] = nc; out[1] = c->chunk_used; out[2] = nf ? sf / nf : 0.0; out[3] = nb ? sb / nb : 0.0; out[4] = mf; out[5] = mb; out[6] = gf; out[7] = gb;
	return PSMC_HIP_OK;
}

int estep_fast(psmc_hip_ctx *c, const double *a, const double *e, const double *a0, double *A, double *E,
                      double *A0, double *LL, double *chk)
{
	const int n = c->n;
	int rc = enqueue_fast(c, a, e, a0, c->d_stats, c->stream);
	if (rc) return rc;
	if ((rc = read_warm(c, c->stream))) return rc;
	collect_timing(c);
	std::vector<double> h((size_t)n * n + 2 * n + 1);
	HIPCHK(c, hipMemcpy(h.data(), c->d_stats, sizeof(double) * h.size(), hipMemcpyDeviceToHost));
	if (A) memcpy(A, h.data(), sizeof(double) * n * n);
	if (E) memcpy(E, h.data() + (size_t)n * n, sizeof(double) * 2 * n);
	if (LL) *LL = h[(size_t)n * n + 2 * n];
	if (A0) memset(A0, 0, sizeof(double) * n);
	if (chk) for (size_t i = 0; i < c->sel.size(); ++i) chk[i] = 1.0;
	return PSMC_HIP_OK;
}

extern "C" int psmcdbg_check_bentry(psmc_hip_ctx *c)
{
	if (!c || c->ns != 64 || !c->d_bentry || !c->d_ftiles) return -1;
	(void)hipSetDevice(c->device);
	(void)hipDeviceSynchronize();
	const int nc = (int)c->chunks.size();
	const int ga = (c->n_list_a + 3) / 4, gb = (c->n_list_b + 3) / 4, ng = ga + gb;
	std::vector<int> tl(4 * (size_t)ng), tf(nc), tb(nc);
	const std::vector<Chunk> &ch = c->chunks;
	(void)hipMemcpy(tl.data(), c->d_ftiles, sizeof(int) * tl.size(), hipMemcpyDeviceToHost);
	(void)hipMemcpy(tf.data(), c->d_touch, sizeof(int) * tf.size(), hipMemcpyDeviceToHost);
	(void)hipMemcpy(tb.data(), c->d_touch + nc, sizeof(int) * tb.size(), hipMemcpyDeviceToHost);
	const double *d_e = c->d_par + 4 * 4096;
	{
			std::vector<double> ha(64 * 64), he(3 * 64), hb((size_t)nc * 64), hx((size_t)nc * 64);
			(void)hipMemcpy(ha.data(), c->d_par, sizeof(double) * ha.size(), hipMemcpyDeviceToHost);
			(void)hipMemcpy(he.data(), d_e, sizeof(double) * he.size(), hipMemcpyDeviceToHost);
			(void)hipMemcpy(hb.data(), c->d_bentry, sizeof(double) * hb.size(), hipMemcpyDeviceToHost);
			(void)hipMemcpy(hx.data(), c->d_bexit, sizeof(double) * hx.size(), hipMemcpyDeviceToHost);
			for (int k = 0; k < 64; ++k) he[128 + k] = 1.0;
			std::vector<int> from_above(nc, 0), in_list(nc, 0);
			for (size_t i = 0; i < tl.size(); ++i) if (tl[i] >= 0) { from_above[tl[i] & ~(1 << 30)] = (tl[i] >> 30) & 1; in_list[tl[i] & ~(1 << 30)] = i < 4 * (size_t)ga ? 1 : 2; }
			for (int b0 = 0; b0 < nc;) {
				int b1 = b0; while (b1 + 1 < nc && ch[b1 + 1].off == ch[b0].off) ++b1;
				const int L = ch[b0].L;
				std::vector<uint8_t> o(L);
				(void)hipMemcpy(o.data(), c->d_obs + ch[b0].off, (size_t)L, hipMemcpyDeviceToHost);
				std::vector<double> bt(64), y(64);
				for (int k = 0; k < 64; ++k) bt[k] = he[(o[L - 1] & 3) * 64 + k];
				int b = b1;
				for (int pp = L - 1; pp >= 1; --pp) {
					while (b >= b0 && std::min(ch[b].hi, L - 1) < ch[b].lo) --b;
					if (b >= b0 && pp == std::min(ch[b].hi, L - 1)) {
						double sx = 0, sy = 0, num = 0, den = 0;
						for (int k = 0; k < 64; ++k) { sx += hb[(size_t)b * 64 + k]; sy += bt[k]; }
						for (int k = 0; k < 64; ++k) { num = std::max(num, std::fabs(hb[(size_t)b * 64 + k] / sx - bt[k] / sy)); den = std::max(den, bt[k] / sy); }
						if (!(num / den < 1e-9))
							fprintf(stderr, "[psmc_hip] RECHECK bentry of tile %d (lo %d hi %d L %d list %d from_above %d tf %d tb %d; above: tf %d tb %d list %d) off by %.2e, sum %.3e; rounds %d/%d\n",
							        b, ch[b].lo, ch[b].hi, L, in_list[b], from_above[b], tf[b], tb[b], b + 1 <= b1 ? tf[b + 1] : -1, b + 1 <= b1 ? tb[b + 1] : -1, b + 1 <= b1 ? in_list[b + 1] : -1, num / den, sx,
							        c->report.fwd_rounds, c->report.bwd_rounds);
						--b;
					}
					double tot = 0;
					for (int k = 0; k < 64; ++k) { double acc = 0; for (int l = 0; l < 64; ++l) acc += ha[k * 64 + l] * bt[l]; y[k] = acc; }
					for (int k = 0; k < 64; ++k) { bt[k] = he[(o[pp - 1] & 3) * 64 + k] * y[k]; tot += bt[k]; }
					for (int k = 0; k < 64; ++k) bt[k] /= tot;
				}
				b0 = b1 + 1;
			}
		}
	return 0;
}
```

### psmc_amd/csrc/estep_fast.hip

```cpp
#include <hip/hip_runtime.h>
#include <cmath>
#include <algorithm>
#include "wave_prims.h"
#include "psmc_hip_internal.h"

namespace psmc {

typedef double d4_t __attribute__((ext_vector_type(4)));

__device__ __forceinline__ double pick_ef(int sym, double e0, double e1) {
	return sym == 0 ? e0 : (sym == 1 ? e1 : 1.0);
}

__device__ __forceinline__ double fast_rcp(double x) {
	double r = __builtin_amdgcn_rcp(x);
	double t = __builtin_fma(-x, r, 1.0);
	r = __builtin_fma(r, t, r);
	t = __builtin_fma(-x, r, 1.0);
	r = __builtin_fma(r, t, r);
	return r;
}

__device__ __forceinline__ double wave_max(double v) {
#pragma unroll
// ... 280 lines not shown
	for (int m = 0; m < 4; ++m)
#pragma unroll
		for (int nn = 0; nn < 4; ++nn)
#pragma unroll
			for (int r = 0; r < 4; ++r) out[(16 * m + t + 4 * r) * S + 16 * nn + i] = acc[m][nn][r] * mult;
	if (qn == 0) {
		double *os = Spart + (int64_t)part * (3 * S) + 64 * qm;
#pragma unroll
		for (int b = 0; b < 3; ++b)
#pragma unroll
			for (int m = 0; m < 4; ++m) {
				double v = Sacc[b][m];
				v += __shfl_xor(v, 16, 64);
				v += __shfl_xor(v, 32, 64);
				if (t == 0) os[b * S + 16 * m + i] = v * mult;
			}
	}
}

template <int S>
__global__ __launch_bounds__(64) void k_ll(const Chunk *__restrict__ chunks, const double *__restrict__ f,
                                             const double *__restrict__ invd, const double *__restrict__ entry,
                                             double *__restrict__ LLpart, const int *__restrict__ fmerge, const double *__restrict__ finv)
{
	const int lane = threadIdx.x;
	const Chunk c = chunks[blockIdx.x];
	const double *io = invd + c.off;
	double prod = 1.0, ll = 0.0;
	const int first = (max(c.lo, 2) + NORM_EVERY - 1) & ~(NORM_EVERY - 1);
	for (int p = first + NORM_EVERY * lane; p <= c.hi; p += NORM_EVERY * 64) {
		prod *= io[p - 1];
		if (prod > 1e280 || prod < 1e-280) { ll -= log(prod); prod = 1.0; }
	}
	ll -= log(prod);
	ll = wave_add(ll);
	if (c.lo > 1) {
		double u = f[(c.off + c.lo - 2) * S + lane], v = entry[(int64_t)blockIdx.x * S + lane];
		if (S == 128) { u += f[(c.off + c.lo - 2) * S + 64 + lane]; v += entry[(int64_t)blockIdx.x * S + 64 + lane]; }
		ll += log(wave_add(u)) - log(wave_add(v));
	}
	if (c.hi == c.L) {
		double v = f[(c.off + c.L - 1) * S + lane];
		if (S == 128) v += f[(c.off + c.L - 1) * S + 64 + lane];
		ll += log(wave_add(v));
	}
	if (fmerge && fmerge[blockIdx.x] > 0) ll -= log(finv[blockIdx.x]);
	if (lane == 0) LLpart[blockIdx.x] = ll * (double)c.mult;
}

template <int S>
__global__ __launch_bounds__(256) void k_reduce1(const double *__restrict__ Cpart, const double *__restrict__ Spart,
                                                   int nC, int nS, const double *__restrict__ LLpart, int nchunks,
                                                   double *__restrict__ stage)
{
	constexpr int SL = S * S + 3 * S + 1;
	const int y = blockIdx.y, tid = threadIdx.x;
	double *st = stage + (int64_t)y * SL;
	if ((int)blockIdx.x < S * S / 256) {
		const int i = blockIdx.x * 256 + tid;
		double s = 0.0;
		for (int j = y; j < nC; j += RED_ROWS) s += Cpart[(int64_t)j * (S * S) + i];
		st[i] = s;
	} else {
		for (int i = tid; i < 3 * S; i += 256) {
			double s = 0.0;
			for (int j = y; j < nS; j += RED_ROWS) s += Spart[(int64_t)j * (3 * S) + i];
			st[S * S + i] = s;
		}
		if (tid == 255) {
			double s = 0.0;
			for (int j = y; j < nchunks; j += RED_ROWS) s += LLpart[j];
			st[S * S + 3 * S] = s;
		}
	}
}
template <int S>
__global__ __launch_bounds__(256) void k_reduce2(const double *__restrict__ stage, const double *__restrict__ a,
                                                   const double *__restrict__ e, double tiny_total, int n,
                                                   double *__restrict__ out)
{
	constexpr int SL = S * S + 3 * S + 1;
	const int i = blockIdx.x * 256 + threadIdx.x;
	if (i >= SL) return;
	double s = 0.0;
	for (int y = 0; y < RED_ROWS; ++y) s += stage[(int64_t)y * SL + i];
	if (i < S * S) {
		const int k = i / S, l = i % S;
		if (k < n && l < n) out[k * n + l] = a[i] * s + tiny_total;
	} else if (i < S * S + 3 * S) {
		const int b = (i - S * S) / S, k = (i - S * S) % S;
		if (b < 2 && k < n) out[n * n + b * n + k] = s + tiny_total;
	} else {
		out[n * n + 2 * n] = s;
	}
}

template <bool REPAIR>
static void launch_fwd(const EstepLaunch &p, hipStream_t st)
{
	const dim3 g(p.n_chunks), b(64);
	if (p.rep_impl == 0)
		hipLaunchKernelGGL((k_fwd_fast<0, REPAIR>), g, b, 0, st, p.d_a, p.d_e, p.d_a0, p.d_obs, p.d_chunks, p.warmup,
		                   p.tol, p.d_dirty, p.d_f, p.d_s, p.d_entry, p.d_touch_f);
	else
		hipLaunchKernelGGL((k_fwd_fast<1, REPAIR>), g, b, 0, st, p.d_a, p.d_e, p.d_a0, p.d_obs, p.d_chunks, p.warmup,
		                   p.tol, p.d_dirty, p.d_f, p.d_s, p.d_entry, p.d_touch_f);
}
template <bool REPAIR>
static void launch_bwd(const EstepLaunch &p, hipStream_t st)
{
	const dim3 g(p.n_chunks), b(64);
	const double *aT = p.d_aeT + 2 * 4096;
	if (p.rep_impl == 0)
		hipLaunchKernelGGL((k_bwd_fast<0, REPAIR>), g, b, 0, st, aT, p.d_e, p.d_obs, p.d_chunks, p.warmup, p.tol,
		                   p.d_dirty_b, p.d_b, p.d_sb, p.d_bentry, p.d_bexit, p.d_touch_b);
	else
		hipLaunchKernelGGL((k_bwd_fast<1, REPAIR>), g, b, 0, st, aT, p.d_e, p.d_obs, p.d_chunks, p.warmup, p.tol,
		                   p.d_dirty_b, p.d_b, p.d_sb, p.d_bentry, p.d_bexit, p.d_touch_b);
}
static void launch_expect(const EstepLaunch &p, hipStream_t st, int redo)
{
	const int nC = p.n_chunks * p.n_sub;
	{
		if (p.ns == 128)
			hipLaunchKernelGGL(k_expect_mfma<128>, dim3(nC * 4), dim3(64), 0, st, p.d_chunks, p.n_sub, p.d_obs, p.d_f, p.d_b, p.d_sb,
			                   p.d_re, p.d_Cpart, p.d_Epart, p.d_touch_f, p.d_touch_b, redo);
		else
			hipLaunchKernelGGL(k_expect_mfma<64>, dim3(nC), dim3(64), 0, st, p.d_chunks, p.n_sub, p.d_obs, p.d_f, p.d_b, p.d_sb,
			                   p.d_re, p.d_Cpart, p.d_Epart, p.d_touch_f, p.d_touch_b, redo);
	}
}

int launch_fast(const EstepLaunch &p, FastReport *rep)
{
	if (p.n_chunks <= 0) return 0;
	(void)hipGetLastError();
	const dim3 g(p.n_chunks), b(64);
	const bool ov = p.overlap != 0;
	hipStream_t sm = p.stream, sa = ov ? p.stream2 : p.stream, sx = ov ? p.stream3 : p.stream;
	rep->fwd_rounds = rep->bwd_rounds = rep->fwd_tiles = rep->bwd_tiles = rep->merged = rep->recounted = 0;
	rep->converged = 1;
	(void)hipMemsetAsync(p.d_warm, 0, 2 * sizeof(unsigned long long), sm);
	(void)hipMemsetAsync(p.d_touch_f, 0, 3 * sizeof(int) * (size_t)p.n_chunks, sm);
	if (p.d_gate) (void)hipMemsetAsync(p.d_gate, 0, 2 * sizeof(int), sm);
	if (p.q_grid > 0) (void)hipMemsetAsync(p.d_qhead, 0, sizeof(int), sm);
	if (p.ev[0]) (void)hipEventRecord(p.ev[0], sm);
	(void)hipEventRecord(p.evx[0], sm);
	if (ov) (void)hipStreamWaitEvent(sa, p.evx[0], 0);
	const bool lw = p.structured && (p.n_long_f > 0 || p.n_long_b > 0) && (ov || p.fused);
	const bool lf = lw && p.n_long_f > 0, lb = lw && p.n_long_b > 0;
	const int ff0 = lf ? p.n_long_f : 0, fb0 = lb ? p.n_long_b : 0;
	const bool mg = p.merge1 && p.structured && p.fused && ov;
	hipStream_t sw = ov ? (mg ? sa : p.stream4) : sm, sk = ov ? p.stream5 : sm;
	if (lw) {
		if (ov && sw != sa) (void)hipStreamWaitEvent(sw, p.evx[0], 0);
		launch_walks(p, sw);
	}
	const bool gated = lw && ov && p.d_gate != nullptr && sw != sm;
	const int rw = p.lanes8 && p.ns == 64 && p.fused ? 8 : 4;
	if (gated) launch_gate(sm, p.d_gate, walk_blocks(p));
	if (mg) {
		launch_sweeps(p, sm, ff0, p.n_items_f - ff0, fb0, p.n_items_b - fb0 - p.n_B_b, true);
		if (p.merge) launch_fwd_struct(p, sm, 6, 0, p.n_fix_f);
		(void)hipEventRecord(p.evx[1], sm);
	}
	if (lw) {
		if (p.n_kc > 0) {
			if (ov) (void)hipStreamWaitEvent(sk, p.evx[0], 0);
			if (gated && sk != sm) launch_gate(sk, p.d_gate + 1, std::min(2048, mg ? (p.n_items_f - ff0 + rw - 1) / rw + (p.n_items_b - fb0 - p.n_B_b + rw - 1) / rw : (p.q_grid > 0 ? p.q_grid : (p.structured ? (p.n_items_f - ff0 + rw - 1) / rw : 0))));
			launch_kchain(p, sk, sw, p.evx[8]);
		}
		(void)hipEventRecord(p.evx[6], sw);
		if (lf) launch_fwd_struct(p, sw, 3, 0, p.n_mem_f);
		(void)hipEventRecord(p.evx[7], sw);
		if (ov) (void)hipStreamWaitEvent(sk, p.fused ? p.evx[7] : p.evx[6], 0);
		if (lb && !p.fused) launch_bwd_struct(p, sk, 3, 0, p.n_mem_b);
		if (p.fused != 2) (void)hipEventRecord(p.evx[9], sk);
	}
	const bool one = p.structured && !p.fused;
	if (mg) {
	} else if (one) {
		if (p.ev[7]) (void)hipEventRecord(p.ev[7], sm);
		launch_sweeps(p, sm, ff0, p.n_items_f - ff0, fb0, p.n_items_b - fb0, false);
		if (p.ev[6]) (void)hipEventRecord(p.ev[6], sm);
	} else if (p.q_grid > 0) launch_phase1_queue(p, sm, ff0, p.n_items_f - ff0, fb0, p.n_items_b - fb0 - p.n_B_b);
	else if (p.structured) launch_fwd_struct(p, sm, 0, ff0, p.n_items_f - ff0);
	else launch_fwd<false>(p, sm);
	if (!mg && p.merge) launch_fwd_struct(p, sm, 6, 0, p.n_fix_f);
	if (!mg) (void)hipEventRecord(p.evx[1], sm);
	if (p.merge && lf) {
		if (ov && sw != sm) (void)hipStreamWaitEvent(sw, p.evx[1], 0);
		launch_fwd_struct(p, sw, 7, 0, p.n_mem_f);
		(void)hipEventRecord(p.evx[7], sw);
	}
	if (p.ev[5]) (void)hipEventRecord(p.ev[5], sm);
	if (one && ov) (void)hipStreamWaitEvent(sa, p.evx[1], 0);
	if (!one && p.ev[7]) (void)hipEventRecord(p.ev[7], sa);
	if (p.fused) {
		if (!mg && p.q_grid <= 0) launch_bwd_struct(p, sa, 4, fb0, p.n_items_b - fb0 - p.n_B_b);
		if (p.fused == 2 && lw) {
			if (lb) { if (ov) (void)hipStreamWaitEvent(sk, p.evx[1], 0); launch_bwd_acc(p, sk, 3, 0, p.n_mem_b); }
			(void)hipEventRecord(p.evx[9], sk);
		}
		(void)hipStreamWaitEvent(sa, p.evx[1], 0);
		const bool late = p.fused == 1 && p.runs_in_b && p.n_list_b > 0;
		if (lw && ov && sw != sa && !late) (void)hipStreamWaitEvent(sa, p.evx[7], 0);
		if (p.ev[8]) (void)hipEventRecord(p.ev[8], sa);
		if (p.fused == 2) { if (p.coarse > 1) launch_bwd_acc(p, sa, 6, 0, p.n_singles_b); else launch_bwd_acc(p, sa, 0, fb0, p.n_items_b - fb0); }
		else {
			launch_bwd_count(p, sa, 0, false);
			if (p.n_list_b > 0) {
				if (lw && ov && sw != sa && late) (void)hipStreamWaitEvent(sa, p.evx[7], 0);
				(void)hipEventRecord(p.evx[11], sa);
				(void)hipEventRecord(p.evx[12], sa);
				launch_bwd_count(p, sa, 1, false);
			}
		}
		if (p.ev[9]) (void)hipEventRecord(p.ev[9], sa);
		if (p.ev[6]) (void)hipEventRecord(p.ev[6], sa);
	} else {
		if (!one) {
			if (p.structured) launch_bwd_struct(p, sa, 0, fb0, p.n_items_b - fb0);
			else launch_bwd<false>(p, sa);
			if (p.ev[6]) (void)hipEventRecord(p.ev[6], sa);
		}
		if (ov) {
			(void)hipEventRecord(p.evx[2], sa);
			(void)hipStreamWaitEvent(sx, p.evx[1], 0); (void)hipStreamWaitEvent(sx, p.evx[2], 0);
			if (lw) { (void)hipStreamWaitEvent(sx, p.evx[7], 0); (void)hipStreamWaitEvent(sx, p.evx[9], 0); }
			if (p.ev[8]) (void)hipEventRecord(p.ev[8], sx);
			launch_expect(p, sx, 0);
			if (p.ev[9]) (void)hipEventRecord(p.ev[9], sx);
			(void)hipEventRecord(p.evx[3], sx);
		}
	}
	struct Chain { hipStream_t st; hipEvent_t rb; int slot; bool bwd, done, pending; int round; };
	Chain ch[2] = {{sm, p.evx[4], 0, false, false, false, 0}, {sa, p.evx[5], 1, true, false, false, 0}};
	auto post_verify = [&](Chain &c) -> int {
		(void)hipMemsetAsync(p.d_cnt + c.slot, 0, sizeof(int), c.st);
		(void)hipMemsetAsync(p.d_warm + c.slot, 0, sizeof(unsigned long long), c.st);
#define PSMC_LV(BW, S, MINE, DIRTY, CNT) hipLaunchKernelGGL((k_verify<BW, S>), g, b, 0, c.st, p.d_chunks, p.n_chunks, p.tol, p.d_f, \
			MINE, p.d_bexit, DIRTY, CNT, p.d_warm, (BW && !p.fused) ? 1 : 0, \
			(p.m_mis && c.round == 0 && (BW || !p.merge)) ? p.m_mis + (BW ? p.n_chunks : 0) : nullptr)
		if (!c.bwd) { if (p.ns == 128) PSMC_LV(false, 128, p.d_entry, p.d_dirty, p.d_cnt); else PSMC_LV(false, 64, p.d_entry, p.d_dirty, p.d_cnt); }
		else { if (p.ns == 128) PSMC_LV(true, 128, p.d_bentry, p.d_dirty_b, p.d_cnt + 1); else PSMC_LV(true, 64, p.d_bentry, p.d_dirty_b, p.d_cnt + 1); }
#undef PSMC_LV
		launch_compact(p, c.st, c.bwd);
		if (hipEventRecord(c.rb, c.st) != hipSuccess) return -1;
		c.pending = true;
		return 0;
	};
	if (lw && ov) { if (sw != sm) (void)hipStreamWaitEvent(sm, p.evx[7], 0); (void)hipStreamWaitEvent(sa, p.evx[9], 0); }
	auto launch_ll = [&](hipStream_t st) {
		const int *fm = p.merge ? p.d_fmerge : nullptr;
		if (p.ns == 128) hipLaunchKernelGGL(k_ll<128>, g, b, 0, st, p.d_chunks, p.d_f, p.d_s, p.d_entry, p.d_LLpart, fm, p.d_finv);
		else hipLaunchKernelGGL(k_ll<64>, g, b, 0, st, p.d_chunks, p.d_f, p.d_s, p.d_entry, p.d_LLpart, fm, p.d_finv);
		PSMC_DBG("k_ll", p.n_chunks, 0, 0);
	};
	auto launch_reduce = [&](hipStream_t sm) {
		const int nS = p.n_chunks * p.n_sub, nC = p.fused == 1 ? (p.n_list_a + p.count_group - 1) / p.count_group + (p.n_list_b + p.count_group - 1) / p.count_group : nS;
		if (p.fused == 2) {
			launch_reduce_factored(p, sm);
		} else if (p.ns == 128) {
			hipLaunchKernelGGL(k_reduce1<128>, dim3(128 * 128 / 256 + 1, RED_ROWS), dim3(256), 0, sm, p.d_Cpart, p.d_Epart, nC, nS, p.d_LLpart,
			                   p.n_chunks, p.d_stage);
			hipLaunchKernelGGL(k_reduce2<128>, dim3((128 * 128 + 3 * 128 + 1 + 255) / 256), dim3(256), 0, sm, p.d_stage, p.d_a, p.d_e,
			                   p.tiny_total, p.n_states, p.d_stats);
		} else {
			hipLaunchKernelGGL(k_reduce1<64>, dim3(17, RED_ROWS), dim3(256), 0, sm, p.d_Cpart, p.d_Epart, nC, nS, p.d_LLpart,
			                   p.n_chunks, p.d_stage);
			hipLaunchKernelGGL(k_reduce2<64>, dim3((STATS_LEN + 255) / 256), dim3(256), 0, sm, p.d_stage, p.d_a, p.d_e,
			                   p.tiny_total, p.n_states, p.d_stats);
		}
		if (p.ev[4]) (void)hipEventRecord(p.ev[4], sm);
	};
	if (post_verify(ch[0]) || post_verify(ch[1])) return -1;
	static const bool recheck = getenv("PSMC_HIP_DEBUG_RECHECK") != nullptr;
	const bool optimistic = p.fused != 0 && ov && !recheck;
	if (optimistic) {
		(void)hipStreamWaitEvent(sx, p.evx[4], 0);
		launch_ll(sx);
		(void)hipEventRecord(p.evx[2], sa); (void)hipStreamWaitEvent(sx, p.evx[2], 0);
		if (p.ev[1]) (void)hipEventRecord(p.ev[1], sx);
		if (p.ev[2]) (void)hipEventRecord(p.ev[2], sx);
		if (p.ev[3]) (void)hipEventRecord(p.ev[3], sx);
		launch_reduce(sx);
		(void)hipEventRecord(p.evx[10], sx);
	}
	bool ll_stale = !optimistic;
	while (!(ch[0].done && ch[1].done)) {
		bool progressed = false;
		for (int d = 0; d < 2; ++d) {
			Chain &c = ch[d];
			if (c.done || !c.pending) continue;
			const hipError_t q = ov ? hipEventQuery(c.rb) : hipEventSynchronize(c.rb);
			if (q == hipErrorNotReady) continue;
			if (q != hipSuccess) return -1;
			c.pending = false; progressed = true;
			const int nd = p.h_cnt[c.slot];
			if (nd == 0) { c.done = true; continue; }
			if (c.round >= p.max_rounds) { rep->converged = 0; c.done = true; continue; }
			++c.round;
			if (p.structured) {
				std::vector<int> *fl = c.bwd ? p.flagged_b : p.flagged_f;
				if (fl) for (int i = 0; i < nd; ++i) fl->push_back(p.h_ritems[(size_t)c.slot * 2 * p.n_chunks + 2 * i]);
			}
			if (!c.bwd) {
				rep->fwd_rounds++; rep->fwd_tiles += nd; ll_stale = true;
				if (p.structured) launch_fwd_struct(p, c.st, 1, 0, nd); else launch_fwd<true>(p, c.st);
			} else {
				rep->bwd_rounds++; rep->bwd_tiles += nd;
				if (p.fused == 2) launch_bwd_acc(p, c.st, 1, 0, nd);
				else if (p.fused) launch_bwd_struct(p, c.st, 5, 0, nd);
				else if (p.structured) launch_bwd_struct(p, c.st, 1, 0, nd);
				else launch_bwd<true>(p, c.st);
			}
			if (post_verify(c)) return -1;
		}
		if (!progressed) __builtin_ia32_pause();
	}
	const bool repaired = rep->fwd_rounds + rep->bwd_rounds > 0;
	if (optimistic) (void)hipStreamWaitEvent(sm, p.evx[10], 0);
	if (optimistic && !repaired) return (int)hipGetLastError();
	if (hipStreamSynchronize(sm) != hipSuccess) return -1;
	if (p.ev[1]) (void)hipEventRecord(p.ev[1], sm);
	if (ll_stale) launch_ll(sm);
	if (p.fused) {
		if (ov) { (void)hipEventRecord(p.evx[2], sa); (void)hipStreamWaitEvent(sm, p.evx[2], 0); }
// ... 55 lines not shown
```

### psmc_amd/csrc/estep_struct.hip

```cpp
#include <hip/hip_runtime.h>
#include "wave_prims.h"
#include "struct_prims.h"
#include "psmc_hip_internal.h"

namespace psmc {

#ifdef PSMC_TRACE_SWEEP
__device__ unsigned long long g_trace_f[4 * 16384], g_trace_b[4 * 16384], g_trace_w[4 * 16384];
__device__ __forceinline__ void trace_put(unsigned long long *t, int block, int slot, unsigned long long v) {
	if ((threadIdx.x & 63) == 0 && block < 16384) t[4 * block + slot] = v;
}
__device__ __forceinline__ unsigned long long trace_hw() {
	const unsigned hw = __builtin_amdgcn_s_getreg((31 << 11) | (0 << 6) | 4), xcc = __builtin_amdgcn_s_getreg((31 << 11) | (0 << 6) | 20);
	return (unsigned long long)hw | ((unsigned long long)(xcc & 0xf) << 32);
}
#define PSMC_TRACE(t, block, slot, v) trace_put(t, block, slot, v)
#else
#define PSMC_TRACE(t, block, slot, v) ((void)0)
#endif

template <int J> __device__ __forceinline__ int sym_of(unsigned w) { return (int)((w >> (8 * J)) & 3u); }
__device__ __forceinline__ unsigned sym_word(const uint4 sv, int g) { return g == 0 ? sv.x : (g == 1 ? sv.y : (g == 2 ? sv.z : sv.w)); }
__device__ __forceinline__ int64_t readlane_i64(int64_t v, int lane) {
	const unsigned lo = (unsigned)__builtin_amdgcn_readlane((int)(unsigned)v, lane);
// ... 329 lines not shown
__device__ __forceinline__ void bwd_block(const StructParN<NPL> &c, const Half8Masks &hm, const double *lds_e, int k0, int m, const uint4 sv, int base,
                                          int p_first, int p_low, int T, BwdCursor &cur, double (&x)[NPL], double *bto,
                                          double *sbo, double *bentry, double *bexit)
{
#pragma unroll 1
	for (int g = 3; g >= 0; --g) {
		const unsigned w = sym_word(sv, g);
		const int pb = base + 4 * g;
		bwd_step<MODE, 3, NPL, LPT>(c, hm, lds_e, k0, m, w, pb, p_first, p_low, T, cur, x, bto, sbo, bentry, bexit);
		bwd_step<MODE, 2, NPL, LPT>(c, hm, lds_e, k0, m, w, pb, p_first, p_low, T, cur, x, bto, sbo, bentry, bexit);
		bwd_step<MODE, 1, NPL, LPT>(c, hm, lds_e, k0, m, w, pb, p_first, p_low, T, cur, x, bto, sbo, bentry, bexit);
		bwd_step<MODE, 0, NPL, LPT>(c, hm, lds_e, k0, m, w, pb, p_first, p_low, T, cur, x, bto, sbo, bentry, bexit);
	}
}

template <bool REPAIR, int NPL, int LPT = 16>
__device__ __forceinline__ void bwd_struct_body(int block, const double *__restrict__ sp, const double *__restrict__ e,
                                                const uint8_t *__restrict__ obs, const Chunk *__restrict__ chunks,
                                                const SweepItem *__restrict__ items, int n_items, int W, int T,
                                                int flags, double *__restrict__ bt, double *__restrict__ sb,
                                                double *__restrict__ bentry, double *__restrict__ bexit,
                                                int *__restrict__ touch_b)
{
	constexpr int S = LPT * NPL, R = 64 / LPT;
	__shared__ double lds_e[4 * S];
	const int lane = threadIdx.x, m = lane & (LPT - 1), k0 = NPL * m;
	const Half8Masks hm = half8_masks(lane);
	fill_lds_e<NPL, LPT>(lds_e, e, lane);
	__syncthreads();
	const int slot = block * R + lane / LPT;
	const SweepItem it = items[slot < n_items ? slot : 0];
#ifdef PSMC_TRACE_SWEEP
	const bool trb = !REPAIR && (flags & (SWEEP_TOP_ONLY | SWEEP_COARSE));
	const unsigned long long trb_c0 = __builtin_readcyclecounter();
	if (trb) PSMC_TRACE(g_trace_b, block, 0, wall_clock64());
#endif
	if (REPAIR || (__any(it.count > 1) && !(flags & SWEEP_COARSE))) __builtin_amdgcn_s_setprio(3);
	else if ((flags & (SWEEP_TOP_ONLY | SWEEP_COARSE)) && (flags & SWEEP_MERGED)) __builtin_amdgcn_s_setprio(1);
	const int t_top = it.first + it.count - 1;
	const Chunk c = chunks[t_top];
	const int L = c.L;
	BwdCursor cur;
	cur.lo = c.lo; cur.top = min(c.hi, L - 1); cur.tile = t_top;
	const int p_low = (flags & SWEEP_TOP_ONLY) ? cur.top
	                  : ((!REPAIR && (flags & SWEEP_WALK)) ? min(chunks[it.first].hi, chunks[it.first].L - 1) : chunks[it.first].lo);
	const bool valid = slot < n_items && cur.top >= cur.lo;
	const bool walk = (flags & (SWEEP_WALK | SWEEP_TOP_ONLY)) != 0, from_entry = (flags & SWEEP_FROM_ENTRY) != 0;
	cur.store = !walk;
	const uint8_t *o = obs + c.off;
	double *bto = bt + c.off * S + k0, *sbo = sb + c.off;
	StructParN<NPL> sc;
	load_struct_par<NPL, LPT>(sp, k0, false, sc);
	double x[NPL];
	int p_first;
	if (REPAIR) {
		if (valid && m == 0 && !(flags & SWEEP_NO_TOUCH)) touch_b[t_top] = 1;
		if (from_entry) loadN<NPL>(bentry + (int64_t)t_top * S + k0, x);
		else loadN<NPL>(bexit + (int64_t)(t_top + 1) * S + k0, x);
		p_first = cur.top;
	} else {
		const int q = min(c.hi + chunk_warm_b(c, W) + 1, L);
		ev_load<NPL, LPT>(lds_e + ((int)o[q - 1] & 3) * S, k0, x);
		p_first = q - 1;
	}
	const int b_first = max((p_first - 1) >> 4, 0);
	const int nblk = valid ? b_first - ((p_low - 1) >> 4) + 1 : 0;
	int64_t roff[R]; int rbf[R], rnb[R];
	int nb_max = 0;
#pragma unroll
	for (int r = 0; r < R; ++r) {
		roff[r] = readlane_i64(c.off, LPT * r);
		rbf[r] = __builtin_amdgcn_readlane(b_first, LPT * r);
		rnb[r] = __builtin_amdgcn_readlane(nblk, LPT * r);
		nb_max = max(nb_max, rnb[r]);
	}
#ifdef PSMC_TRACE_SWEEP
	if (trb) PSMC_TRACE(g_trace_b, block, 3, trace_hw() | ((unsigned long long)nb_max << 40));
#endif
	for (int bi = 0; bi < nb_max; ++bi) {
		int bb[R];
#pragma unroll
		for (int r = 0; r < R; ++r) bb[r] = rbf[r] - min(bi, max(rnb[r] - 1, 0));
		const uint4 sv = row_symbols(obs, roff, bb, lane / LPT);
		if (bi < nblk) {
			const int base = (b_first - bi) << 4;
			int mode = (base + 1 > cur.lo && base + 16 < cur.top) ? 1 : ((base + 1 > cur.top && base + 16 <= p_first) ? 2 : 0);
			if (walk && mode == 1) mode = 2;
			if (__all(mode == 1)) bwd_block<1, NPL, LPT>(sc, hm, lds_e, k0, m, sv, base, p_first, p_low, T, cur, x, bto, sbo, bentry, bexit);
			else if (__all(mode == 2)) bwd_block<2, NPL, LPT>(sc, hm, lds_e, k0, m, sv, base, p_first, p_low, T, cur, x, bto, sbo, bentry, bexit);
			else bwd_block<0, NPL, LPT>(sc, hm, lds_e, k0, m, sv, base, p_first, p_low, T, cur, x, bto, sbo, bentry, bexit);
		}
	}
#ifdef PSMC_TRACE_SWEEP
	if (trb) { PSMC_TRACE(g_trace_b, block, 2, wall_clock64()); PSMC_TRACE(g_trace_b, block, 1, __builtin_readcyclecounter() - trb_c0); }
#endif
}

template <bool REPAIR, int NPL, int LPT = 16>
__global__ __launch_bounds__(64) void k_bwd_struct(const double *__restrict__ sp, const double *__restrict__ e,
                                                     const uint8_t *__restrict__ obs, const Chunk *__restrict__ chunks,
                                                     const SweepItem *__restrict__ items, int n_items, int W, int T,
                                                     int flags, double *__restrict__ bt, double *__restrict__ sb,
                                                     double *__restrict__ bentry, double *__restrict__ bexit,
                                                     int *__restrict__ touch_b)
{
	bwd_struct_body<REPAIR, NPL, LPT>(blockIdx.x, sp, e, obs, chunks, items, n_items, W, T, flags, bt, sb, bentry, bexit, touch_b);
}

template <bool CK>
__global__ __launch_bounds__(64) void k_phase1_queue(const double *__restrict__ sp, const double *__restrict__ e,
                                                       const double *__restrict__ a0, const uint8_t *__restrict__ obs,
                                                       const Chunk *__restrict__ chunks, const SweepItem *__restrict__ items_f, int n_f,
                                                       const SweepItem *__restrict__ items_b, int n_b, int W, int T, int flags_f,
                                                       int flags_b, double *__restrict__ f, double *__restrict__ invd,
                                                       double *__restrict__ entry, double *__restrict__ bt, double *__restrict__ sb,
                                                       double *__restrict__ bentry, double *__restrict__ bexit, int *__restrict__ touch_f,
                                                       int *__restrict__ touch_b, const int *__restrict__ q, int n_q,
                                                       int *__restrict__ head, int *__restrict__ started, const FwdCtl ctl)
{
	announce_start(started);
	for (;;) {
		int i = 0;
		if (threadIdx.x == 0) i = atomicAdd(head, 1);
		i = __builtin_amdgcn_readfirstlane(i);
		if (i >= n_q) break;
		const int w = q[i];
		__builtin_amdgcn_s_setprio(0);
		if ((w & 1) == 0)
			fwd_struct_body<false, 4, CK>(w >> 1, sp, e, a0, obs, chunks, items_f, n_f, W, T, flags_f, f, invd, entry, touch_f, ctl);
		else
			bwd_struct_body<false, 4>(w >> 1, sp, e, obs, chunks, items_b, n_b, W, T, flags_b, bt, sb, bentry, bexit, touch_b);
	}
}

template <int NPL>
__global__ __launch_bounds__(64) void k_walk_struct(const double *__restrict__ sp, const double *__restrict__ e,
                                                      const double *__restrict__ a0, const uint8_t *__restrict__ obs,
                                                      const Chunk *__restrict__ chunks, const SweepItem *__restrict__ items_f,
                                                      int n_f, const SweepItem *__restrict__ items_b, int n_b, int W, int T,
                                                      double *__restrict__ entry, double *__restrict__ bentry,
                                                      double *__restrict__ bexit, int *__restrict__ started)
{
	announce_start(started);
	const int nbf = (n_f + 3) / 4;
	if ((int)blockIdx.x < nbf)
		fwd_struct_body<false, NPL>(blockIdx.x, sp, e, a0, obs, chunks, items_f, n_f, W, T, SWEEP_WALK, nullptr, nullptr, entry, nullptr);
	else
		bwd_struct_body<false, NPL>(blockIdx.x - nbf, sp, e, obs, chunks, items_b, n_b, W, T, SWEEP_WALK, nullptr, nullptr, bentry, bexit,
		                       nullptr);
}

__device__ __forceinline__ double walk_ev(int sym, double e0, double e1) { return sym == 0 ? e0 : (sym == 1 ? e1 : 1.0); }

__global__ __launch_bounds__(64) void k_walk1_struct(const double *__restrict__ sp, const double *__restrict__ e,
                                                       const double *__restrict__ a0, const uint8_t *__restrict__ obs,
                                                       const Chunk *__restrict__ chunks, const SweepItem *__restrict__ items_f,
                                                       int n_f, const SweepItem *__restrict__ items_b, int n_b, int W, int T,
                                                       double *__restrict__ entry, double *__restrict__ bentry,
                                                       double *__restrict__ bexit, int *__restrict__ started)
{
	const int lane = threadIdx.x, block = (int)blockIdx.x;
	announce_start(started);
#ifdef PSMC_TRACE_SWEEP
	PSMC_TRACE(g_trace_w, block, 0, wall_clock64()); PSMC_TRACE(g_trace_w, block, 3, trace_hw());
	struct TraceEnd { int b; __device__ ~TraceEnd() { if (threadIdx.x == 0 && b < 16384) g_trace_w[4 * b + 2] = wall_clock64(); } } trace_end{block};
#endif
	__builtin_amdgcn_s_setprio(3);
	const WaveScanMasks wm = wave_scan_masks(lane);
	const double e0 = e[lane], e1 = e[64 + lane];
	if (block < n_f) {
		const SweepItem it = items_f[block];
		const Chunk c = chunks[it.first];
		const bool warm_only = it.count <= 0;
		const int thru = warm_only ? -it.count : it.count;
		const int p_last = thru == 0 ? c.lo - 1 : chunks[it.first + thru - 1].hi;
		const uint8_t *o = obs + c.off;
		StructPar1 s1; s1.mS = sp[lane]; s1.wS = sp[128 + lane]; s1.mP = sp[64 + lane]; s1.wP = sp[192 + lane]; s1.dd = sp[256 + lane];
		double x = a0[lane];
		int p_first;
		const int ws = max(1, c.lo - chunk_warm_f(c, W));
		if (ws == 1) { x *= walk_ev((int)o[0] & 3, e0, e1); p_first = 2; } else p_first = ws;
		int tile = c.lo >= p_first ? it.first : it.first + 1, next_lo = c.lo >= p_first ? c.lo : c.lo + T;
		const int g_first = (p_first - 1) >> 2, g_last = (p_last - 1) >> 2;
		unsigned w = *reinterpret_cast<const unsigned *>(o + 4 * g_first);
		for (int g = g_first; g <= g_last; ++g) {
			const unsigned wn = *reinterpret_cast<const unsigned *>(o + 4 * min(g + 1, g_last));
#pragma unroll
			for (int j = 0; j < 4; ++j) {
				const int p = 4 * g + j + 1;
				if (p < p_first || p > p_last) continue;
				if (p == next_lo) { entry[(int64_t)tile * 64 + lane] = x; ++tile; next_lo += T; }
				double ev = walk_ev((int)((w >> (8 * j)) & 3u), e0, e1);
				if (j == 3) ev *= rcp_newton(first_lane_f64(wave_sum_nat(x)));
				x = struct_step1(s1, x, wm) * ev;
			}
			w = wn;
		}
		if (warm_only) entry[(int64_t)(it.first + thru) * 64 + lane] = x;
	} else {
		const SweepItem it = items_b[block - n_f];
		const bool warm_only = it.count == 0;
		int tile = it.first + max(it.count, 1) - 1;
		const Chunk c = chunks[tile];
		int lo = c.lo, top = min(c.hi, c.L - 1);
		const int L = c.L, p_low = warm_only ? top + 1 : chunks[it.first + 1].lo;
		if (top < lo) return;
		const uint8_t *o = obs + c.off;
		StructPar1 s1; s1.mS = sp[192 + lane]; s1.wS = sp[64 + lane]; s1.mP = sp[128 + lane]; s1.wP = sp[lane]; s1.dd = sp[256 + lane];
		const int q = min(c.hi + chunk_warm_b(c, W) + 1, L);
		double x = walk_ev((int)o[q - 1] & 3, e0, e1);
		const int p_first = q - 1;
		const int g_first = (p_first - 1) >> 2, g_last = (p_low - 1) >> 2;
		unsigned w = *reinterpret_cast<const unsigned *>(o + 4 * g_first);
		for (int g = g_first; g >= g_last; --g) {
			const unsigned wn = *reinterpret_cast<const unsigned *>(o + 4 * max(g - 1, g_last));
#pragma unroll
			for (int j = 3; j >= 0; --j) {
				const int p = 4 * g + j + 1;
				if (p > p_first || p < p_low) continue;
				double ev = walk_ev((int)((w >> (8 * j)) & 3u), e0, e1);
				if (j == 3) ev *= rcp_newton(first_lane_f64(wave_sum_nat(x)));
				if (p == top) bentry[(int64_t)tile * 64 + lane] = x;
				x = struct_step1(s1, x, wm) * ev;
				if (p == lo) { bexit[(int64_t)tile * 64 + lane] = x; --tile; top = lo - 1; lo -= T; }
			}
			w = wn;
		}
		if (warm_only || it.count > 1) bentry[(int64_t)tile * 64 + lane] = x;
	}
}

struct KcTile { int tile, dir; };
__host__ __device__ inline void kc_range(const Chunk &c, int dir, int &lo, int &top)
{
	const bool fwd = dir == 0;
	top = fwd ? c.hi : min(c.hi, c.L - 1);
	lo = fwd ? c.lo : min(((c.lo + 3) & ~3) + 1, top + 1);
}

template <int NPL>
__global__ __launch_bounds__(64) void k_kcol_struct(const double *__restrict__ sp, const double *__restrict__ e,
                                                      const uint8_t *__restrict__ obs, const Chunk *__restrict__ chunks,
                                                      const KcTile *__restrict__ kc, const int *__restrict__ uniq, double *__restrict__ Kcol,
                                                      double *__restrict__ Kexp)
{
	constexpr int S = 16 * NPL, BPT = S / 4;
	__shared__ double lds_e[4 * S];
	const int lane = threadIdx.x, m = lane & 15, k0 = NPL * m;
	fill_lds_e<NPL, 16>(lds_e, e, lane);
	__syncthreads();
	const int j = blockIdx.x / BPT, col = 4 * (blockIdx.x % BPT) + (lane >> 4);
	__builtin_amdgcn_s_setprio(2);
	const KcTile kt = kc[uniq[j]];
	const Chunk c = chunks[kt.tile];
	const bool fwd = kt.dir == 0;
	const int top = fwd ? c.hi : min(c.hi, c.L - 1);
	const int lo = fwd ? c.lo : min(((c.lo + 3) & ~3) + 1, top + 1);
	const uint8_t *o = obs + c.off;
	StructParN<NPL> sc;
	load_struct_par<NPL>(sp, k0, fwd, sc);
	double x[NPL];
#pragma unroll
	for (int i = 0; i < NPL; ++i) x[i] = (k0 + i == col) ? 1.0 : 0.0;
	int E = 0;
	const int n = top - lo + 1;
	for (int q = 0; q < n; ++q) {
		const int p = fwd ? lo + q : top - q;
		const int sym = (int)o[p - 1] & 3;
		double ev[NPL];
		ev_load<NPL>(lds_e + sym * S, k0, ev);
		if ((p & 3) == 0) {
			const double s = row_sum16(lane_sum<NPL>(x));
			const int ex = s > 0.0 ? __builtin_amdgcn_frexp_exp(s) : 0;
#pragma unroll
			for (int i = 0; i < NPL; ++i) x[i] = __builtin_amdgcn_ldexp(x[i], -ex);
			E += ex;
		}
		struct_step<NPL>(sc, x);
#pragma unroll
		for (int i = 0; i < NPL; ++i) x[i] *= ev[i];
	}
	storeN<NPL>(Kcol + ((int64_t)j * S + col) * S + k0, x);
	if (m == 0) Kexp[(int64_t)j * S + col] = (double)E;
}

template <int NQ>
__global__ __launch_bounds__(64 * NQ) void k_kcol2_struct(const double *__restrict__ kcc, const uint8_t *__restrict__ obs,
                                                            const Chunk *__restrict__ chunks, const KcTile *__restrict__ kc, const int *__restrict__ uniq,
                                                            double *__restrict__ Kcol, double *__restrict__ Kexp, int sub, int prio)
{
	constexpr int S = 32 * NQ, NCG = S / 64, KD = 11 * S;
	__shared__ double xch[2][NQ][2][64];
	__shared__ double tab[KD];
	const int lane = threadIdx.x & 63;
	const int w = __builtin_amdgcn_readfirstlane((int)(threadIdx.x >> 6));
	const int j = (int)blockIdx.x / NCG, cg = (int)blockIdx.x % NCG, jt = j / sub, js = j % sub;
	const int col = 64 * cg + lane;
	if (prio >= 2) __builtin_amdgcn_s_setprio(2); else if (prio == 1) __builtin_amdgcn_s_setprio(1);
	const KcTile kt = kc[uniq[jt]];
	const Chunk c = chunks[kt.tile];
	const bool fwd = kt.dir == 0;
	for (int i = threadIdx.x; i < KD; i += 64 * NQ) tab[i] = kcc[(fwd ? 0 : KD) + i];
	__syncthreads();
	int top, lo;
	kc_range(c, kt.dir, lo, top);
	const uint8_t *o = obs + c.off;
	const double *cc = tab + 32 * w;
	double x[32];
#pragma unroll
	for (int k = 0; k < 32; ++k) x[k] = (32 * w + k == col) ? 1.0 : 0.0;
	int E = 0;
	const int n = max(top - lo + 1, 0);
	const int q0 = (int)((int64_t)n * js / sub), q1 = (int)((int64_t)n * (js + 1) / sub);
	for (int q = q0; q < q1; ++q) {
		const int p = fwd ? lo + q : top - q;
		const int sym = min((int)o[p - 1] & 3, 2);
		const double *ce = cc + 2 * S + sym * 3 * S;
		double y[32], sS = 0.0, sP = 0.0;
#pragma unroll
		for (int k = 31; k >= 0; --k) { sS = __builtin_fma(x[k], cc[k], sS); y[k] = ce[k] * sS; }
#pragma unroll
		for (int k = 0; k < 32; ++k) {
			sP = __builtin_fma(x[k], cc[S + k], sP);
			y[k] = __builtin_fma(ce[2 * S + k], x[k], __builtin_fma(ce[S + k], sP, y[k]));
		}
		xch[q & 1][w][0][lane] = sS; xch[q & 1][w][1][lane] = sP;
		__syncthreads();
		if constexpr (NQ == 2) {
			const double S0 = xch[q & 1][0][0][lane], S1 = xch[q & 1][1][0][lane], P0 = xch[q & 1][0][1][lane], P1 = xch[q & 1][1][1][lane];
			const double T = w == 0 ? S1 : P0;
			const double *cz = ce + (w == 0 ? 0 : S);
			if ((p & 3) == 0) {
				const double mag = (S0 + S1) + (P0 + P1);
				const int ex = mag > 0.0 ? __builtin_amdgcn_frexp_exp(mag) : 0;
				const double sc = __builtin_amdgcn_ldexp(1.0, -ex);
#pragma unroll
				for (int k = 0; k < 32; ++k) x[k] = __builtin_fma(cz[k], T, y[k]) * sc;
				E += ex;
			} else {
#pragma unroll
				for (int k = 0; k < 32; ++k) x[k] = __builtin_fma(cz[k], T, y[k]);
			}
		} else {
			double Ts = 0.0, Tp = 0.0, mag = 0.0;
#pragma unroll
			for (int v = 0; v < NQ; ++v) {
				const double Sv = xch[q & 1][v][0][lane], Pv = xch[q & 1][v][1][lane];
				Ts += v > w ? Sv : 0.0; Tp += v < w ? Pv : 0.0; mag += Sv + Pv;
			}
			double sc = 1.0;
			if ((p & 3) == 0) {
				const int ex = mag > 0.0 ? __builtin_amdgcn_frexp_exp(mag) : 0;
				sc = __builtin_amdgcn_ldexp(1.0, -ex);
				E += ex;
			}
#pragma unroll
			for (int k = 0; k < 32; ++k) x[k] = __builtin_fma(ce[k], Ts, __builtin_fma(ce[S + k], Tp, y[k])) * sc;
		}
	}
	double *out = Kcol + ((int64_t)j * S + col) * S + 32 * w;
#pragma unroll
	for (int k = 0; k < 32; ++k) out[k] = x[k];
	if (w == 0) Kexp[(int64_t)j * S + col] = (double)E;
}

__device__ __forceinline__ double wave_max_f64(double v) {
#pragma unroll
	for (int m = 32; m >= 1; m >>= 1) v = fmax(v, __shfl_xor(v, m, 64));
	return v;
}
struct KcRun { int first, count, kc0, pad; };

template <int PER>
__device__ __forceinline__ void struct_step1n(const StructPar1 (&c)[PER], double (&x)[PER], const WaveScanMasks &m)
{
	if constexpr (PER == 1) { x[0] = struct_step1(c[0], x[0], m); }
	else {
		const double s1 = wave_suffix_incl(x[1] * c[1].mS, m), s0 = wave_suffix_incl(x[0] * c[0].mS, m);
		const double p0 = wave_prefix_incl_bc(x[0] * c[0].mP), p1 = wave_prefix_incl_bc(x[1] * c[1].mP);
		const double tot1 = readlane_f64(s1, 0), tot0 = readlane_f64(p0, 63);
		const double y0 = __builtin_fma(c[0].wS, s0 + tot1, __builtin_fma(c[0].wP, p0, c[0].dd * x[0]));
		const double y1 = __builtin_fma(c[1].wS, s1, __builtin_fma(c[1].wP, p1 + tot0, c[1].dd * x[1]));
		x[0] = y0; x[1] = y1;
	}
}

template <int PER>
__global__ __launch_bounds__(64 * (PER == 1 ? 2 : 8)) void k_kchain_struct(const KcRun *__restrict__ runs, int n_f, const int *__restrict__ kslot,
                                                        const double *__restrict__ Kcol,
                                                        const double *__restrict__ Kexp, const double *__restrict__ sp,
                                                        const double *__restrict__ e, const uint8_t *__restrict__ obs,
                                                        const Chunk *__restrict__ chunks, double *__restrict__ entry,
                                                        double *__restrict__ bentry, int sub)
{
	constexpr int S = 64 * PER, RW = 32 / PER, NW = S / RW;
	__shared__ double part[2][NW][S];
	const int lane = threadIdx.x & 63;
	const int w = __builtin_amdgcn_readfirstlane((int)(threadIdx.x >> 6));
	__builtin_amdgcn_s_setprio(3);
	const bool fwd = (int)blockIdx.x < n_f;
	const KcRun r = runs[blockIdx.x];
	double *vec = fwd ? entry : bentry;
	int t = fwd ? r.first : r.first + r.count - 1;
	double x[PER];
	const WaveScanMasks wm = wave_scan_masks(lane);
	StructPar1 s1[PER];
	double e0[PER], e1[PER];
#pragma unroll
	for (int q = 0; q < PER; ++q) {
		const int k = lane + 64 * q;
		x[q] = vec[(int64_t)t * S + k];
		s1[q].mS = sp[3 * S + k]; s1[q].wS = sp[S + k]; s1[q].mP = sp[2 * S + k]; s1[q].wP = sp[k]; s1[q].dd = sp[4 * S + k];
		e0[q] = e[k]; e1[q] = e[S + k];
	}
	const int n_mats = (r.count - 1) * sub;
	const int row0 = RW * w, src_h = row0 >> 6, src_l = row0 & 63;
	double ma[RW][PER], mb[RW][PER], ea[PER], eb[PER];
	auto load = [&](int j, double (&m)[RW][PER], double (&ex)[PER]) {
		const int64_t kb = ((int64_t)kslot[r.kc0 + j / sub] * sub + j % sub) * S;
#pragma unroll
		for (int i = 0; i < RW; ++i)
#pragma unroll
			for (int h = 0; h < PER; ++h) m[i][h] = Kcol[(kb + row0 + i) * S + lane + 64 * h];
#pragma unroll
		for (int h = 0; h < PER; ++h) ex[h] = Kexp[kb + lane + 64 * h];
	};
	auto product = [&](int j, const double (&m)[RW][PER], const double (&ex)[PER]) {
		double xs[PER], y[PER], em = -1e300;
#pragma unroll
		for (int h = 0; h < PER; ++h) em = fmax(em, x[h] > 0.0 ? ex[h] : -1e300);
		const double emax = wave_max_f64(em);
#pragma unroll
		for (int h = 0; h < PER; ++h) { xs[h] = x[h] > 0.0 ? __builtin_amdgcn_ldexp(x[h], (int)(ex[h] - emax)) : 0.0; y[h] = 0.0; }
		double src = xs[0];
		if constexpr (PER == 2) src = src_h ? xs[1] : xs[0];
#pragma unroll
		for (int i = 0; i < RW; ++i) {
			const double v = readlane_f64(src, src_l + i);
#pragma unroll
			for (int h = 0; h < PER; ++h) y[h] = __builtin_fma(v, m[i][h], y[h]);
		}
		double (*pp)[S] = part[j & 1];
#pragma unroll
		for (int h = 0; h < PER; ++h) pp[w][lane + 64 * h] = y[h];
		__syncthreads();
#pragma unroll
		for (int h = 0; h < PER; ++h) {
			double tsum = pp[0][lane + 64 * h];
#pragma unroll
// ... 56 lines not shown
                                                       double *__restrict__ entry, double *__restrict__ bt,
                                                       double *__restrict__ sb, double *__restrict__ bentry,
                                                       double *__restrict__ bexit, int *__restrict__ started, const double *__restrict__ prevx)
{
	announce_start(started);
	constexpr int R = 64 / LPT;
	const int nbf = (n_f + R - 1) / R, nbb = (n_b + R - 1) / R, both = 2 * min(nbf, nbb), b = blockIdx.x;
	bool fwd; int blk;
	if (!(flags_b & SWEEP_ALTERNATE)) { fwd = b < nbf; blk = fwd ? b : b - nbf; }
	else if (b < both) { fwd = (b & 1) == 0; blk = b >> 1; }
	else { fwd = nbf > nbb; blk = b - both + min(nbf, nbb); }
	if (fwd) fwd_struct_body<false, NPL, CK, LPT>(blk, sp, e, a0, obs, chunks, items_f, n_f, W, T, flags_f, f, invd, entry, nullptr, FwdCtl{prevx, 0.0, nullptr, nullptr, nullptr, nullptr});
	else bwd_struct_body<false, NPL, LPT>(blk, sp, e, obs, chunks, items_b, n_b, W, T, flags_b, bt, sb, bentry, bexit, nullptr);
}

__global__ __launch_bounds__(64) void k_compact(const int *__restrict__ dirty, int n, SweepItem *__restrict__ out,
                                                  SweepItem *__restrict__ host_out, int *__restrict__ host_cnt)
{
	const int lane = threadIdx.x;
	int base = 0;
	for (int i0 = 0; i0 < n; i0 += 64) {
		const int i = i0 + lane;
		const bool d = i < n && dirty[i] != 0;
		const unsigned long long mask = __ballot(d);
		if (d) {
			SweepItem s; s.first = i; s.count = 1;
			const int at = base + __popcll(mask & ((1ull << lane) - 1ull));
			out[at] = s;
			if (host_out) host_out[at] = s;
		}
		base += __popcll(mask);
	}
	if (lane == 0) *host_cnt = base;
	__threadfence_system();
}

void launch_fwd_struct(const EstepLaunch &p, hipStream_t st, int which, int first, int n_items)
{
	if (n_items <= 0) return;
	const bool l8 = p.lanes8 && p.ns == 64 && which == 0;
	const dim3 g(l8 ? (n_items + 7) / 8 : (n_items + 3) / 4), b(64);
	const SweepItem *items = (const SweepItem *)(which == 1 ? p.d_ritems_f : (which == 3 || which == 7 ? p.d_members_f : (which == 6 ? p.d_fix_f : p.d_items_f))) + first;
	const bool fixp = which == 6 || which == 7;
	const int flags = (which == 3 ? (SWEEP_FROM_ENTRY | SWEEP_NO_TOUCH) : 0)
	                  | (p.ckpt ? SWEEP_CKPT : 0) | (which == 0 && p.coarse > 1 ? SWEEP_COARSE : 0) | (fixp ? SWEEP_MERGE : 0);
	const FwdCtl ctl = {which == 0 ? p.d_prevx : nullptr, p.tol, fixp ? p.m_mis : nullptr, fixp ? p.m_mlen : nullptr, p.d_fmerge, p.d_finv};
#define PSMC_LF(REP, NPL, CK) hipLaunchKernelGGL((k_fwd_struct<REP, NPL, CK>), g, b, 0, st, p.d_sp, p.d_e, p.d_a0, p.d_obs, p.d_chunks, \
		items, n_items, p.warmup, p.tile_len, flags, p.d_f, p.d_s, p.d_entry, p.d_touch_f, which == 0 && p.d_gate ? p.d_gate + 1 : nullptr, ctl)
	const bool rep = which != 0;
	if (l8) {
#define PSMC_LF8(CK) hipLaunchKernelGGL((k_fwd_struct<false, 8, CK, 8>), g, b, 0, st, p.d_sp, p.d_e, p.d_a0, p.d_obs, p.d_chunks, \
		items, n_items, p.warmup, p.tile_len, flags, p.d_f, p.d_s, p.d_entry, p.d_touch_f, p.d_gate ? p.d_gate + 1 : nullptr, ctl)
		if (p.ckpt) PSMC_LF8(true); else PSMC_LF8(false);
#undef PSMC_LF8
	} else if (p.ns == 128) { if (rep) PSMC_LF(true, 8, false); else PSMC_LF(false, 8, false); }
	else if (p.ckpt) { if (rep) PSMC_LF(true, 4, true); else PSMC_LF(false, 4, true); }
	else { if (rep) PSMC_LF(true, 4, false); else PSMC_LF(false, 4, false); }
	PSMC_DBG("launch_fwd_struct", which, first, n_items);
#undef PSMC_LF
}
void launch_bwd_struct(const EstepLaunch &p, hipStream_t st, int which, int first, int n_items)
{
	if (n_items <= 0) return;
	const bool l8 = p.lanes8 && p.ns == 64 && which == 4;
	const dim3 g(l8 ? (n_items + 7) / 8 : (n_items + 3) / 4), b(64);
	const SweepItem *items = (const SweepItem *)(which == 1 || which == 5 ? p.d_ritems_b : (which == 3 ? p.d_members_b : p.d_items_b)) + first;
	const int flags = which == 5 ? SWEEP_WALK : (which == 3 ? (SWEEP_FROM_ENTRY | SWEEP_NO_TOUCH) : (which == 4 ? (p.coarse > 1 ? (SWEEP_WALK | SWEEP_COARSE) : SWEEP_TOP_ONLY) : 0));
#define PSMC_LB(REP, NPL) hipLaunchKernelGGL((k_bwd_struct<REP, NPL>), g, b, 0, st, p.d_sp, p.d_e, p.d_obs, p.d_chunks, items, \
		n_items, p.warmup, p.tile_len, flags, p.d_b, p.d_sb, p.d_bentry, p.d_bexit, p.d_touch_b)
	const bool rep = !(which == 0 || which == 4);
	if (l8)
		hipLaunchKernelGGL((k_bwd_struct<false, 8, 8>), g, b, 0, st, p.d_sp, p.d_e, p.d_obs, p.d_chunks, items, n_items, p.warmup, p.tile_len, flags,
		                   p.d_b, p.d_sb, p.d_bentry, p.d_bexit, p.d_touch_b);
	else if (p.ns == 128) { if (rep) PSMC_LB(true, 8); else PSMC_LB(false, 8); }
	else { if (rep) PSMC_LB(true, 4); else PSMC_LB(false, 4); }
	PSMC_DBG("launch_bwd_struct", which, first, n_items);
#undef PSMC_LB
}
void launch_phase1_queue(const EstepLaunch &p, hipStream_t st, int ff, int nf, int fb, int nb)
{
	if (p.n_queue <= 0 || p.q_grid <= 0) return;
	const int flags_f = (p.ckpt ? SWEEP_CKPT : 0) | (p.coarse > 1 ? SWEEP_COARSE : 0);
	const int flags_b = p.coarse > 1 ? (SWEEP_WALK | SWEEP_COARSE) : SWEEP_TOP_ONLY;
	const FwdCtl ctl = {p.d_prevx, p.tol, nullptr, nullptr, p.d_fmerge, p.d_finv};
#define PSMC_LQ(CK) hipLaunchKernelGGL(k_phase1_queue<CK>, dim3(p.q_grid), dim3(64), 0, st, p.d_sp, p.d_e, p.d_a0, p.d_obs, p.d_chunks, \
		(const SweepItem *)p.d_items_f + ff, nf, (const SweepItem *)p.d_items_b + fb, nb, p.warmup, p.tile_len, flags_f, flags_b, p.d_f, p.d_s, \
		p.d_entry, p.d_b, p.d_sb, p.d_bentry, p.d_bexit, p.d_touch_f, p.d_touch_b, p.d_queue, p.n_queue, p.d_qhead, p.d_gate ? p.d_gate + 1 : nullptr, ctl)
	if (p.ckpt) PSMC_LQ(true); else PSMC_LQ(false);
#undef PSMC_LQ
	PSMC_DBG("launch_phase1_queue", nf, nb, p.q_grid);
}
void launch_compact(const EstepLaunch &p, hipStream_t st, bool bwd)
{
	hipLaunchKernelGGL(k_compact, dim3(1), dim3(64), 0, st, bwd ? p.d_dirty_b : p.d_dirty, p.n_chunks,
	                   (SweepItem *)(bwd ? p.d_ritems_b : p.d_ritems_f),
	                   (SweepItem *)(p.m_ritems ? p.m_ritems + (size_t)(bwd ? 1 : 0) * 2 * p.n_chunks : nullptr), p.m_cnt + (bwd ? 1 : 0));
	PSMC_DBG("verify + launch_compact", bwd, p.n_chunks, 0);
}
void launch_sweeps(const EstepLaunch &p, hipStream_t st, int ff, int nf, int fb, int nb, bool top_only)
{
	const bool l8 = p.lanes8 && p.ns == 64 && top_only;
	const int nblk = l8 ? (nf + 7) / 8 + (nb + 7) / 8 : (nf + 3) / 4 + (nb + 3) / 4;
	if (nblk <= 0) return;
	const int co = top_only && p.coarse > 1 ? SWEEP_COARSE : 0;
	const int flags_f = (p.ckpt ? SWEEP_CKPT : 0) | co,
	          flags_b = (top_only ? (co ? SWEEP_WALK | co : SWEEP_TOP_ONLY) : 0) | (top_only && p.merge_order ? SWEEP_MERGED : SWEEP_ALTERNATE);
#define PSMC_LS(NPL, CK) hipLaunchKernelGGL((k_sweep_struct<NPL, CK>), dim3(nblk), dim3(64), 0, st, p.d_sp, p.d_e, p.d_a0, p.d_obs, p.d_chunks, \
		(const SweepItem *)p.d_items_f + ff, nf, (const SweepItem *)p.d_items_b + fb, nb, p.warmup, p.tile_len, flags_f, flags_b, \
		p.d_f, p.d_s, p.d_entry, p.d_b, p.d_sb, p.d_bentry, p.d_bexit, p.d_gate ? p.d_gate + 1 : nullptr, p.d_prevx)
#define PSMC_LS8(CK) hipLaunchKernelGGL((k_sweep_struct<8, CK, 8>), dim3(nblk), dim3(64), 0, st, p.d_sp, p.d_e, p.d_a0, p.d_obs, p.d_chunks, \
		(const SweepItem *)p.d_items_f + ff, nf, (const SweepItem *)p.d_items_b + fb, nb, p.warmup, p.tile_len, flags_f, flags_b, \
		p.d_f, p.d_s, p.d_entry, p.d_b, p.d_sb, p.d_bentry, p.d_bexit, p.d_gate ? p.d_gate + 1 : nullptr, p.d_prevx)
	if (l8) { if (p.ckpt) PSMC_LS8(true); else PSMC_LS8(false); }
	else if (p.ns == 128) PSMC_LS(8, false); else if (p.ckpt) PSMC_LS(4, true); else PSMC_LS(4, false);
#undef PSMC_LS8
	PSMC_DBG("launch_sweeps", nf, nb, top_only);
#undef PSMC_LS
}
__global__ __launch_bounds__(64) void k_gather_prev(const Chunk *__restrict__ chunks, const SweepItem *__restrict__ items, int S, const double *__restrict__ f,
                                                      const double *__restrict__ a0, double *__restrict__ prevx, int ck)
{
	const SweepItem it = items[blockIdx.x];
	const Chunk c = chunks[it.first];
	const int ws = max(1, c.lo - c.wf);
	const bool have = ws > 1 && !(ck && ((ws - 1) & 7));
	for (int k = threadIdx.x; k < S; k += 64) {
		double v = a0[k];
		if (have) { const double t = f[(c.off + ws - 2) * S + k]; v = (t > 0.0 && t < 1e300) ? t : v; }
		prevx[(int64_t)it.first * S + k] = v;
	}
}
void launch_gather_prev(const EstepLaunch &p, hipStream_t st, int first, int n_items, double *prevx)
{
	if (n_items <= 0) return;
	hipLaunchKernelGGL(k_gather_prev, dim3(n_items), dim3(64), 0, st, p.d_chunks, (const SweepItem *)p.d_items_f + first, p.ns, p.d_f, p.d_a0, prevx, p.ckpt);
}

__global__ __launch_bounds__(64) void k_tile_allmiss(const uint8_t *__restrict__ obs, const Chunk *__restrict__ chunks, int *__restrict__ flags)
{
	const Chunk c = chunks[blockIdx.x];
	const uint8_t *o = obs + c.off;
	int bad = 0;
	for (int p = c.lo + (int)threadIdx.x; p <= c.hi; p += 64) bad |= ((int)o[p - 1] & 3) != 2;
	const int any_bad = __any(bad);
	if (threadIdx.x == 0) flags[blockIdx.x] = any_bad ? 0 : 1;
}
int launch_tile_allmiss(hipStream_t st, const uint8_t *d_obs, const Chunk *d_chunks, int n_chunks, int *d_flags)
{
	if (n_chunks <= 0) return 0;
	hipLaunchKernelGGL(k_tile_allmiss, dim3(n_chunks), dim3(64), 0, st, d_obs, d_chunks, d_flags);
	return (int)hipGetLastError();
}

void launch_kchain(const EstepLaunch &p, hipStream_t st_cols, hipStream_t st_chain, hipEvent_t ev_cols)
{
	if (p.n_kc <= 0) return;
	if (p.ns == 128)
		hipLaunchKernelGGL(k_kcol_struct<8>, dim3(p.n_kuniq * 32), dim3(64), 0, st_cols, p.d_sp, p.d_e, p.d_obs, p.d_chunks,
		                   (const KcTile *)p.d_kc, p.d_kuniq, p.d_Kcol, p.d_Kexp);
	else
		hipLaunchKernelGGL(k_kcol2_struct<2>, dim3(p.n_kuniq * p.kc_sub), dim3(128), 0, st_cols, p.d_kcc, p.d_obs, p.d_chunks, (const KcTile *)p.d_kc, p.d_kuniq,
		                   p.d_Kcol, p.d_Kexp, p.kc_sub, p.kcol_prio);
	if (st_cols != st_chain) { (void)hipEventRecord(ev_cols, st_cols); (void)hipStreamWaitEvent(st_chain, ev_cols, 0); }
	if (p.ns == 128)
		hipLaunchKernelGGL(k_kchain_struct<2>, dim3(p.n_chain_f + p.n_chain_b), dim3(512), 0, st_chain, (const KcRun *)p.d_kruns, p.n_chain_f, p.d_kslot,
		                   p.d_Kcol, p.d_Kexp, p.d_sp, p.d_e, p.d_obs, p.d_chunks, p.d_entry, p.d_bentry, p.kc_sub);
	else
		hipLaunchKernelGGL(k_kchain_struct<1>, dim3(p.n_chain_f + p.n_chain_b), dim3(128), 0, st_chain, (const KcRun *)p.d_kruns, p.n_chain_f, p.d_kslot,
		                   p.d_Kcol, p.d_Kexp, p.d_sp, p.d_e, p.d_obs, p.d_chunks, p.d_entry, p.d_bentry, p.kc_sub);
	PSMC_DBG("launch_kchain", p.n_kc, p.n_chain_f, p.n_chain_b);
}
int walk_blocks(const EstepLaunch &p) { return p.ns == 64 ? p.n_wl_f + p.n_wl_b : (p.n_wl_f + 3) / 4 + (p.n_wl_b + 3) / 4; }
void launch_walks(const EstepLaunch &p, hipStream_t st)
{
	if (p.n_wl_f + p.n_wl_b <= 0) return;
	if (p.ns == 64) {
		hipLaunchKernelGGL(k_walk1_struct, dim3(p.n_wl_f + p.n_wl_b), dim3(64), 0, st, p.d_sp, p.d_e, p.d_a0, p.d_obs, p.d_chunks,
		                   (const SweepItem *)p.d_wl_f, p.n_wl_f, (const SweepItem *)p.d_wl_b, p.n_wl_b, p.warmup,
		                   p.tile_len, p.d_entry, p.d_bentry, p.d_bexit, p.d_gate);
		PSMC_DBG("launch_walks", p.n_wl_f, p.n_wl_b, 0);
		return;
	}
	hipLaunchKernelGGL(k_walk_struct<8>, dim3((p.n_wl_f + 3) / 4 + (p.n_wl_b + 3) / 4), dim3(64), 0, st, p.d_sp, p.d_e, p.d_a0, p.d_obs, p.d_chunks,
	                   (const SweepItem *)p.d_wl_f, p.n_wl_f, (const SweepItem *)p.d_wl_b, p.n_wl_b, p.warmup, p.tile_len,
	                   p.d_entry, p.d_bentry, p.d_bexit, p.d_gate);
	PSMC_DBG("launch_walks (four per wave)", p.n_wl_f, p.n_wl_b, 0);
}

}

#ifdef PSMC_TRACE_SWEEP
extern "C" int psmc_hip_debug_trace(int which, unsigned long long *out, int n)
{
	if (n > 16384) n = 16384;
	return (int)(which == 0 ? hipMemcpyFromSymbol(out, HIP_SYMBOL(psmc::g_trace_f), sizeof(unsigned long long) * 4 * n)
	             : which == 1 ? hipMemcpyFromSymbol(out, HIP_SYMBOL(psmc::g_trace_b), sizeof(unsigned long long) * 4 * n)
	                          : hipMemcpyFromSymbol(out, HIP_SYMBOL(psmc::g_trace_w), sizeof(unsigned long long) * 4 * n));
}
#endif
```

### psmc_amd/csrc/psmc_hip_ctx.h

```cpp
#pragma once
#include <hip/hip_runtime.h>
#include <math.h>
#include <stdio.h>
#include <stdlib.h>
#include <string.h>
#include <algorithm>
#include <atomic>
#include <chrono>
#include <string>
#include <thread>
#include <vector>
#include "psmc_hip.h"
#include "psmc_hip_internal.h"

using namespace psmc;

#define HMM_TINY_H 1e-25

constexpr int DEC_NONE = 0;
constexpr int DEC_FAST = 1;
constexpr int DEC_EXACT = 2;
constexpr int DEC_NO_BT = 3;
constexpr int DEC_MERGED = 4;
constexpr int DEC_WIDE = 5;
constexpr int WD_NONE = 0;
constexpr int WD_OK = 1;
constexpr int WD_FAILED = 2;

struct psmc_hip_ctx {
	int n = 0, ns = 64, device = 0, mode = PSMC_HIP_MODE_EXACT;
	std::string err;
	int chunk = 0, warmup = 3072, max_rounds = 4096, rep_impl = -1, n_sub = 6, target_waves = 1536, overlap = 1;
	double warm_tol = 1e-12;
	int struct_opt = 1;
	bool struct_tiles_set = false;
	int struct_tiles = 8192;
	bool use_struct = false, planned_struct = false;
	int last_fused = 0, last_ckpt = 0;
	int dec_kind = 0; unsigned long long dec_serial = 0;
	bool want_factored = false;
	int kc_sub = 4;
	int kcol_prio = 2;
	int two_phase = -1;
	int two_phase_used = 2;
	int merge1 = -1;
	int merge1_used = 0;
	int merge_order = -1;
	int lanes8 = -1;
	int gate = -1;
	int *d_gate = nullptr;
	int phase1 = -1;
	int phase1_waves = 2;
	int *d_queue = nullptr;
	size_t queue_cap = 0; int n_queue = 0;
	int coarse = -1;
	int coarse_used = 1, items_coarse = -1;
	bool warm_shift_set = false, kc_sub_set = false;
	int warm_shift_used = 1, kc_sub_used = 4;
	int kc_div = 16;
	int kc_min = -1;
	int n_wl_f = 0, n_wl_b = 0, n_kc = 0, n_chain_f = 0, n_chain_b = 0, n_singles_b = 0;
	double *d_Kcol = nullptr; size_t kcol_cap = 0;
	hipStream_t stream5 = nullptr;
	int ckpt = 1;
	int fuse = 1;
	int fuse128 = 2;
	int count_group = 4;
	int merge = 0;
	int adapt = 0;
	int prev_start = 0;
	int *h_mlen = nullptr, *m_mlen = nullptr;
	double *h_mis = nullptr, *m_mis = nullptr;
	double *d_prevx = nullptr, *d_finv = nullptr;
	std::vector<int> order_f;
	int n_fix_f = 0;
	bool merge_used = false;
	Chunk *h_chunks = nullptr; size_t h_chunks_cap = 0;
	bool prev_ok = false;
	unsigned long long prev_serial = 0, tab_serial = 0;
	const double *prev_f = nullptr; int prev_ckpt = 0;
	int learn = 1;
	int warm_shift = 1;
	bool chunks_dirty = false;
	int group_cap = 131072;
	int *d_items = nullptr;
	int *h_ritems = nullptr;
	int *m_ritems = nullptr, *m_cnt = nullptr;
	std::vector<uint8_t> glue_f, glue_b;
	std::vector<uint8_t> gap;
	int gap_tiles = 1;
	int n_kuniq = 0;
	std::vector<int> flagged_f, flagged_b;
	bool items_dirty = true;
	int n_items_f = 0, n_items_b = 0;
	int n_sub_used = 6;
	int n_seg = 0;
	std::vector<int32_t> L;
	std::vector<int64_t> off;
	int64_t total = 0;
	bool obs_borrowed = false;
	uint8_t *d_obs = nullptr;
	int64_t *d_seg_off = nullptr;
	int32_t *d_seg_len = nullptr;
	std::vector<int32_t> sel;
	std::vector<int32_t> work;
	std::vector<int32_t> sel2work;
	std::vector<int32_t> mult;
	int32_t *d_work = nullptr;
	bool plan_dirty = true;
	double *h_par = nullptr, *d_par = nullptr;
	size_t par_len = 0;
	static constexpr size_t PAR_LEN = 2 * 16384 + 3 * 128 + 128 + 3 * 128 + 5 * 128 + 2 * 11 * 128;
	static constexpr size_t RE128_OFF = 2 * 16384 + 3 * 128 + 128, SP128_OFF = RE128_OFF + 3 * 128, KCC128_OFF = SP128_OFF + 5 * 128;
	static constexpr size_t SP_OFF = 4 * 4096 + 192 + 64 + 192;
	static constexpr size_t KCC_OFF = SP_OFF + 5 * 64;
	double *d_f = nullptr, *d_b = nullptr, *d_s = nullptr, *d_sb = nullptr;
	int64_t tab_bins = 0; bool have_b = false;
	double *d_segA = nullptr, *d_segE = nullptr, *d_segA0 = nullptr, *d_chk = nullptr;
	int seg_cap = 0;
	std::vector<double> h_segA, h_segE, h_segA0, h_chk, h_s;
	std::vector<Chunk> chunks;
	Chunk *d_chunks = nullptr;
	int chunk_cap = 0, chunk_used = 0;
	double *d_entry = nullptr, *d_bentry = nullptr, *d_bexit = nullptr, *d_Cpart = nullptr, *d_Epart = nullptr,
	       *d_LLpart = nullptr;
	size_t cpart_cap = 0;
	int *d_dirty = nullptr, *d_cnt = nullptr, *h_cnt = nullptr, *d_touch = nullptr;
	hipStream_t stream2 = nullptr, stream3 = nullptr, stream4 = nullptr;
	hipEvent_t evx[14] = {nullptr, nullptr, nullptr, nullptr, nullptr, nullptr, nullptr, nullptr, nullptr, nullptr, nullptr, nullptr, nullptr, nullptr};
	bool timing_two_launches = false;
	int n_long_f = 0, n_long_b = 0, n_mem_f = 0, n_mem_b = 0;
	int n_B_b = 0, n_list_a = 0, n_list_b = 0;
	int items_two_phase = -1;
	int runs_late = 1;
	bool runs_in_b = false;
	int *d_ftiles = nullptr;
	FastReport report = {0, 0, 0, 0, 1, 0, 0};
	double *d_stage = nullptr, *d_stats = nullptr;
	unsigned long long *d_warm = nullptr;
	double warm_err[2] = {0, 0};
	hipStream_t stream = nullptr;
	hipEvent_t ev[10] = {nullptr, nullptr, nullptr, nullptr, nullptr, nullptr, nullptr, nullptr, nullptr, nullptr};
	double last_ms[7] = {0, 0, 0, 0, 0, 0, 0};
	bool timing_valid = false;
	int64_t batch_bins = 0;
	int exact_refwd = -1;
	int32_t *d_bw_seg = nullptr, *d_bw_par = nullptr; int64_t *d_bw_tab = nullptr; size_t bw_cap = 0;
	double *d_bpar = nullptr; size_t bpar_cap = 0;
	int *d_cu_mask = nullptr;
	double *d_lkp = nullptr; size_t lkp_cap = 0; std::vector<double> h_lkp;
	int64_t *d_lkoff = nullptr; size_t lkoff_cap = 0;
	double *d_s_all = nullptr; size_t s_all_cap = 0;
	int batch_sort = 1;
	int batch_tailfill = 1;
	int batch_major = 1;
	int batch_first = 0;
	double *d_b2 = nullptr; int64_t b2_bins = 0, b2_alloc = 0;
	int64_t reserved_cap = 0;
	int reserved_refwd = -1;
	int cu_first = 0, cu_count = 0;
	int last_batch_groups = 0;
	bool tables_batch = false;
	psmc_hip_ctx *x_twin = nullptr;
	int n_exact_fallbacks = 0;
	psmc_hip_ctx *parent = nullptr;
	std::vector<psmc_hip_ctx *> kids;
	int share_learn = 1;
	int share_T = 0;
	std::vector<std::vector<uint8_t>> sh_glue_f, sh_glue_b;
	std::vector<std::vector<int32_t>> sh_wf, sh_wb;
	std::vector<int32_t> chunk_seg, chunk_idx;
	double dbg_acc[8] = {0, 0, 0, 0, 0, 0, 0, 0};
	int wide_fast = 0;
	bool wf_ran = false;
	std::vector<Chunk> wf_chunks;
	Chunk *d_wf_chunks = nullptr;
	int wf_cap = 0, wf_T = 0, wf_W = 0;
	bool warmup_set = false;
	double *d_wf_X = nullptr, *d_wf_inv = nullptr; int64_t wf_bins = 0;
	double *d_wf_par = nullptr, *h_wf_par = nullptr;
	double *d_wf_entry = nullptr, *d_wf_bentry = nullptr, *d_wf_bexit = nullptr, *d_wf_part = nullptr, *d_wf_ll = nullptr;
	int *d_wf_dirty = nullptr, *d_wf_list = nullptr;
	int wide_decode = 0;
	int wd_kind = 0; unsigned long long wd_serial = 0, wd_sel = 0, sel_serial = 0;
};
inline double dbg_now() { return std::chrono::duration<double>(std::chrono::steady_clock::now().time_since_epoch()).count(); }
inline psmc_hip_ctx *dbg_root(psmc_hip_ctx *c) { return c->parent ? c->parent : c; }

inline int fail(psmc_hip_ctx *c, int code, const char *what, hipError_t e = hipSuccess)
{
	if (c) {
		c->err = what;
		if (e != hipSuccess) { c->err += ": "; c->err += hipGetErrorString(e); }
	}
	return code;
}
#define HIPCHK(c, call)                                                     \
	do {                                                                    \
		hipError_t e__ = (call);                                            \
		if (e__ != hipSuccess) return fail((c), PSMC_HIP_EDEVICE, #call, e__); \
	} while (0)

template <class T> inline int dev_alloc(psmc_hip_ctx *c, T **p, size_t n)
{
	if (*p) { (void)hipFree(*p); *p = nullptr; }
	if (n == 0) n = 1;
	hipError_t e = hipMalloc((void **)p, n * sizeof(T));
	if (e != hipSuccess) { *p = nullptr; return fail(c, PSMC_HIP_ENOMEM, "hipMalloc", e); }
	static const char *poison = getenv("PSMC_HIP_POISON");
	static int poison_count = 0;
	if (poison) {
		(void)hipMemset(*p, strcmp(poison, "vary") == 0 ? 0x3B + (poison_count++ % 8) : 0xFF, n * sizeof(T));
		(void)hipDeviceSynchronize();
// ... 26 lines not shown
```

### psmc_amd/csrc/psmc_hip_internal.h

```cpp
#pragma once
#include <cstdio>
#include <cstdlib>
#include <hip/hip_runtime.h>
#include <stdint.h>
#include <vector>

namespace psmc {

constexpr int NS = 64;
constexpr int NORM_EVERY = 4;
constexpr int STATS_LEN = NS * NS + 3 * NS + 1;

struct Chunk {
	int64_t off;
	int32_t L;
	int32_t lo;
	int32_t hi;
	int32_t mult;
	int32_t flags;
	int32_t wf, wb;
};
__host__ __device__ inline int chunk_warm_f(const Chunk &c, int) { return c.wf; }
__host__ __device__ inline int chunk_warm_b(const Chunk &c, int) { return c.wb; }
constexpr int CHUNK_ANCHOR_F = 1;
constexpr int CHUNK_ANCHOR_B = 2;
constexpr int CHUNK_LAST = 4;

struct ExWork {
	const int32_t *seg;
	const int32_t *par;
	const int64_t *tab;
	const int64_t *tab_s;
	int n;
	int64_t par_stride;
};

struct FastReport { int fwd_rounds, bwd_rounds, fwd_tiles, bwd_tiles, converged, merged, recounted; };

struct EstepLaunch {
	hipStream_t stream, stream2, stream3;
	hipEvent_t evx[14];
	int overlap;
	int rep_impl, n_states;
	const int64_t *d_work_tab_s;
	int *d_cu_mask = nullptr;
	int exact_only;
	int exact_refwd;
	int ns;
	const double *d_a;
	const double *d_aeT;
	const double *d_e;
	const double *d_a0;
	const double *d_re;
	const double *d_sp;
	int structured;
	const double *d_kcc;
	int kc_sub;
	int kcol_prio;
	int fused;
	int ckpt;
	int merge_order;
	int merge1;
	const int *d_items_f, *d_items_b;
	int n_items_f, n_items_b, tile_len;
	int n_long_f, n_long_b;
	const int *d_members_f, *d_members_b;
	int n_mem_f, n_mem_b;
	int lanes8;
	int *d_gate;
	const int *d_queue; int n_queue;
	int q_grid; int *d_qhead;
	int coarse;
	const int *d_singles_b; int n_singles_b;
	int n_B_b;
	const int *d_ftiles; int n_list_a, n_list_b;
	int count_group;
	int runs_in_b;
	hipStream_t stream4, stream5;
	const int *d_wl_f, *d_wl_b; int n_wl_f, n_wl_b;
	const int *d_kc, *d_kruns; int n_kc, n_chain_f, n_chain_b;
	const int *d_kslot, *d_kuniq; int n_kuniq;
	double *d_Kcol, *d_Kexp;
	int *d_ritems_f, *d_ritems_b;
	int *h_ritems;
	int *m_ritems, *m_cnt;
	std::vector<int> *flagged_f, *flagged_b;
	const uint8_t *d_obs;
	const int64_t *d_seg_off;
	const int32_t *d_seg_len;
	const int32_t *d_work;
	int n_work;
	const int32_t *d_work_par; const int64_t *d_work_tab; int64_t par_stride; int work_align;
	double *d_f, *d_b, *d_s;
	double *d_segA, *d_segE, *d_segA0, *d_chk;
	const Chunk *d_chunks;
	int n_chunks, warmup, n_sub;
	double *d_entry, *d_bentry, *d_bexit;
	int *d_dirty, *d_dirty_b, *d_cnt, *h_cnt;
	int *d_touch_f, *d_touch_b;
	int merge;
	const int *d_fix_f; int n_fix_f;
	int *d_fmerge;
	double *d_finv;
	int *m_mlen, *h_mlen;
	double *m_mis;
	const double *d_prevx;
	double *d_sb;
	double tol; int max_rounds;
	double *d_Cpart;
	double *d_Epart;
	double *d_LLpart;
	double *d_stage;
	double *d_stats;
	unsigned long long *d_warm;
	double tiny_total;
	hipEvent_t ev[10];
};

inline bool dbg_sync_on() { static const bool on = getenv("PSMC_HIP_DEBUG_SYNC") != nullptr; return on; }
#define PSMC_DBG(NAME, A, B, C) do { if (psmc::dbg_sync_on()) { hipError_t e_ = hipDeviceSynchronize(); \
	fprintf(stderr, "[psmc_hip] %s(%d, %d, %d): %s\n", NAME, (int)(A), (int)(B), (int)(C), hipGetErrorString(e_)); fflush(stderr); } } while (0)

constexpr int RED_ROWS = 64;

int launch_exact(const EstepLaunch &p);
constexpr int LKP_DIV = 16, LKP_MIN = 64;
int launch_lk_products(hipStream_t st, const EstepLaunch &p, const double *d_s, const int64_t *d_lk_off, double *d_out);
int launch_exact_wide(const EstepLaunch &p);
int launch_post_decode_wide(hipStream_t st, const double *f, const double *b, const double *s, int64_t off, int L, int n, int S, int32_t *path, double *maxp);
int launch_post_full_wide(hipStream_t st, const double *a, const double *e, const uint8_t *obs, const double *f, const double *b, const double *s,
                          int64_t off, int L, int n, int S, double *post, double *recomb);
int launch_post_counts_wide(hipStream_t st, const double *f, const double *b, const double *s, int64_t off, int min_l, const int32_t *cnt1,
                            int n_cnt, int n, int S, double *cnt);
int launch_fast(const EstepLaunch &p, FastReport *rep);
void launch_fwd_struct(const EstepLaunch &p, hipStream_t st, int which, int first, int n_items);
void launch_bwd_struct(const EstepLaunch &p, hipStream_t st, int which, int first, int n_items);
void launch_compact(const EstepLaunch &p, hipStream_t st, bool bwd);
void launch_gather_prev(const EstepLaunch &p, hipStream_t st, int first, int n_items, double *prevx);
int launch_tile_allmiss(hipStream_t st, const uint8_t *d_obs, const Chunk *d_chunks, int n_chunks, int *d_flags);
void launch_walks(const EstepLaunch &p, hipStream_t st);
void launch_gate(hipStream_t st, const int *ctr, int want);
int walk_blocks(const EstepLaunch &p);
void launch_kchain(const EstepLaunch &p, hipStream_t st_cols, hipStream_t st_chain, hipEvent_t ev_cols);
void launch_sweeps(const EstepLaunch &p, hipStream_t st, int ff, int nf, int fb, int nb, bool top_only);
void launch_phase1_queue(const EstepLaunch &p, hipStream_t st, int ff, int nf, int fb, int nb);
void launch_bwd_count(const EstepLaunch &p, hipStream_t st, int list, bool redo, bool all_from_bentry = false);
void launch_bwd_acc(const EstepLaunch &p, hipStream_t st, int which, int first, int n);
void launch_reduce_factored(const EstepLaunch &p, hipStream_t st);
int launch_post_decode(hipStream_t st, const double *f, const double *b, const double *s, int64_t off, int L, int n,
                       int ns, int32_t *path, double *maxp);
int launch_post_full(hipStream_t st, const double *a, const double *e, const uint8_t *obs, const double *f, const double *b,
                     const double *s, int64_t off, int L, int n, int ns, double *post, double *recomb);
int launch_post_counts(hipStream_t st, const double *f, const double *b, const double *s, int64_t off, int min_l,
                       const int32_t *cnt1, int n_cnt, int n, int ns, double *cnt);
int launch_post_fast(hipStream_t st, const double *f, const double *b, const double *sb, const double *re, const double *a,
                     const uint8_t *obs, int64_t off, int L, int n, int ns, double *post, double *recomb, int32_t *path, double *maxp);
int launch_scales_fast(hipStream_t st, const double *f, const double *invd, const double *entry, const double *a0, const double *e,
                       const uint8_t *obs, int64_t off, int L, int T, int first, int ns, double *s);
int post_counts_fast_blocks(int min_l);
int launch_post_counts_fast(hipStream_t st, const double *f, const double *b, const double *re, const uint8_t *obs, int64_t off,
                            int L, int min_l, const int32_t *cnt1, int n_cnt, int n, int ns, double *part, double *cnt);
int run_selftest(hipStream_t stream, unsigned *d_flags);
int run_microbench(hipStream_t stream, double *d_out);
int run_pipe_probe(hipStream_t stream, double *d_out, int n_waves, unsigned mask, int rounds);
int run_pipe_probe2(hipStream_t stream, double *d_out, const int *kinds8, int rounds, const void *gsrc);
int run_place_probe(hipStream_t stream, double *d_out, int n_waves, int wpb, int steps);
int run_stream_probe(hipStream_t stream, const double *src, double *dst, size_t n);
int run_hbm_probe(hipStream_t stream, int which, double *a, double *b, size_t bytes);
int run_load_probe(hipStream_t stream, double *d_out, int n_waves, int steps);
int run_load_probe_st(hipStream_t stream, double *d_out, int n_waves, int steps, double *tbl, int store_steps, int mode);

}
```

Before: 2.446 billion bins/s.

## Fuse short-run forward finish into walk kernel and move chain heads into kcol launch

Adds a walk_finish mode, on by default for 64 states. Walk blocks for short forward runs (up to 4 tiles) now run the forward member sweep themselves right after the walk, instead of waiting for a separate fwd_struct launch. Chain-head walks are folded into the k_kcol2 launch as extra blocks, and the remaining member sweep moves to the kchain stream with event dependencies. The intent is to cut the serial walk → member-sweep dependency and one stream hop, at the cost of more complex scheduling, event ordering, and a larger kcol grid.

```diff
diff --git a/psmc_amd/csrc/api.hip b/psmc_amd/csrc/api.hip
--- a/psmc_amd/csrc/api.hip
+++ b/psmc_amd/csrc/api.hip
@@ -205,6 +205,7 @@
 	else if (k == "kc_sub") { if (v < 1 || v > 16) return PSMC_HIP_EINVAL; c->kc_sub = (int)v; c->kc_sub_set = true; c->plan_dirty = true; c->items_dirty = true; }
 	else if (k == "two_phase") { if (v != -1 && v != 0 && v != 2) return PSMC_HIP_EINVAL; c->two_phase = (int)v; c->plan_dirty = true; c->items_dirty = true; }
 	else if (k == "kc_min") { if (v < -1) return PSMC_HIP_EINVAL; c->kc_min = (int)v; c->items_dirty = true; }
+	else if (k == "walk_finish") { if (v != 0 && v != 1) return PSMC_HIP_EINVAL; c->walk_finish = (int)v; c->items_dirty = true; }
 	else if (k == "ckpt") { c->ckpt = v != 0 ? 1 : 0; }
 	else if (k == "fuse") { c->fuse = v != 0 ? 1 : 0; c->plan_dirty = true; }
 	else if (k == "fuse128") { if (v != 0 && v != 2) return PSMC_HIP_EINVAL; c->fuse128 = (int)v; c->plan_dirty = true; c->items_dirty = true; }
diff --git a/psmc_amd/csrc/api_batch.hip b/psmc_amd/csrc/api_batch.hip
--- a/psmc_amd/csrc/api_batch.hip
+++ b/psmc_amd/csrc/api_batch.hip
@@ -401,7 +401,7 @@
 		k->warmup = c->warmup; k->max_rounds = c->max_rounds; k->rep_impl = c->rep_impl;
 		k->n_sub = c->n_sub; k->target_waves = c->target_waves; k->overlap = c->overlap; k->warm_tol = c->warm_tol; k->struct_opt = c->struct_opt;
 		k->struct_tiles_set = c->struct_tiles_set; k->struct_tiles = c->struct_tiles;
-		k->two_phase = c->two_phase; k->kc_div = c->kc_div; k->kc_min = c->kc_min; k->ckpt = c->ckpt; k->fuse = c->fuse;
+		k->two_phase = c->two_phase; k->kc_div = c->kc_div; k->kc_min = c->kc_min; k->walk_finish = c->walk_finish; k->ckpt = c->ckpt; k->fuse = c->fuse;
 		k->learn = c->learn; k->group_cap = c->group_cap; k->warm_shift = c->warm_shift; k->kc_sub = c->kc_sub; k->kcol_prio = c->kcol_prio;
 		k->fuse128 = c->fuse128; k->coarse = c->coarse; k->gate = c->gate; k->lanes8 = c->lanes8; k->gap_tiles = c->gap_tiles; k->exact_refwd = c->exact_refwd;
 		k->merge = c->merge; k->adapt = c->adapt; k->prev_start = c->prev_start;
diff --git a/psmc_amd/csrc/api_fast.hip b/psmc_amd/csrc/api_fast.hip
--- a/psmc_amd/csrc/api_fast.hip
+++ b/psmc_amd/csrc/api_fast.hip
@@ -92,7 +92,7 @@
 		     hipHostGetDevicePointer((void **)&c->m_mis, c->h_mis, 0) != hipSuccess))
 			return fail(c, PSMC_HIP_ENOMEM, "hipHostMalloc (mapped)");
 		if ((rc = dev_alloc(c, &c->d_LLpart, (size_t)nc))) return rc;
-		if ((rc = dev_alloc(c, &c->d_items, (size_t)32 * nc + 64))) return rc;
+		if ((rc = dev_alloc(c, &c->d_items, (size_t)33 * nc + 64))) return rc;
 		if ((rc = dev_alloc(c, &c->d_ftiles, (size_t)2 * (nc + 16)))) return rc;
 		if (c->h_ritems) { (void)hipHostFree(c->h_ritems); c->h_ritems = nullptr; }
 		if (hipHostMalloc((void **)&c->h_ritems, (size_t)4 * nc * sizeof(int), hipHostMallocMapped) != hipSuccess ||
@@ -196,8 +196,6 @@
 	c->n_mem_f = c->n_mem_b = 0;
 	for (size_t i = 0; i < kf.size(); ++i) {
 		h[2 * i] = kf[i].second.first; h[2 * i + 1] = kf[i].second.second;
-		if (in_run_f[kf[i].second.first])
-			for (int t = 0; t < kf[i].second.second; ++t) { mem[2 * (size_t)c->n_mem_f] = kf[i].second.first + t; mem[2 * (size_t)c->n_mem_f + 1] = 1; ++c->n_mem_f; }
 	}
 	for (size_t i = 0; i < kb.size(); ++i) {
 		h[(size_t)2 * nc + 2 * i] = kb[i].second.first; h[(size_t)2 * nc + 2 * i + 1] = kb[i].second.second;
@@ -231,7 +229,6 @@
 		c->n_singles_b = (int)sg.size() / 2;
 		if (!sg.empty()) HIPCHK(c, hipMemcpy(c->d_items + (size_t)24 * nc, sg.data(), sizeof(int) * sg.size(), hipMemcpyHostToDevice));
 	}
-	HIPCHK(c, hipMemcpy(c->d_items + (size_t)8 * nc, mem.data(), sizeof(int) * mem.size(), hipMemcpyHostToDevice));
 	{
 		std::vector<int> fx;
 		for (int b = 0; b < nc; ++b)
@@ -276,14 +273,15 @@
 			kslot.push_back(gap_slot[dir]);
 		} else { kslot.push_back((int)kuniq.size()); kuniq.push_back(j); }
 	};
-	c->n_wl_f = c->n_wl_b = 0;
 	const int kc_min = c->kc_min >= 0 ? c->kc_min : (c->ns == 128 ? (nc > 4096 ? 12 : 8) : (nc > 4096 ? 5 : 4));
 	const bool chains = kc_min >= 2;
 	const int head_count = c->ns == 64 ? 0 : 1;
+	const bool finish = c->walk_finish != 0 && c->ns == 64;
+	struct Wk { int first, count, kind, run; };
+	std::vector<Wk> wk_f, wk_b;
 	auto add_runs = [&](const std::vector<std::pair<long long, std::pair<int, int>>> &k, int n_long, bool bwd) {
-		int &nw = bwd ? c->n_wl_b : c->n_wl_f;
+		std::vector<Wk> &wk = bwd ? wk_b : wk_f;
 		std::vector<int> &rv = bwd ? runs_b : runs_f;
-		int *w = wl.data() + (bwd ? (size_t)2 * nc : 0);
 		int budget = std::max(64, nc / c->kc_div);
 		for (int i = 0; i < n_long; ++i) {
 			int first = k[i].second.first, count = k[i].second.second;
@@ -293,22 +291,42 @@
 			const bool chain = chains && count >= kc_min && cost <= budget;
 			if (chain) budget -= cost;
 			if (chain && !bwd && c->chunks[first].lo == 1) {
-				w[2 * nw] = first; w[2 * nw + 1] = (head_count == 0 && count - 1 >= 2) ? -1 : 2; ++nw;
+				wk.push_back({first, (head_count == 0 && count - 1 >= 2) ? -1 : 2, count - 1 >= 2 ? 0 : 1, i});
 				first += 1; count -= 1;
 				if (count >= 2) {
 					rv.push_back(first); rv.push_back(count); rv.push_back((int)(kc.size() / 2)); rv.push_back(0);
 					for (int t = first; t < first + count - 1; ++t) push_kc(t, 0);
 				}
 			} else if (chain) {
-				w[2 * nw] = bwd ? first + count - 1 : first; w[2 * nw + 1] = head_count; ++nw;
+				wk.push_back({bwd ? first + count - 1 : first, head_count, 0, i});
 				rv.push_back(first); rv.push_back(count); rv.push_back((int)(kc.size() / 2)); rv.push_back(0);
 				if (!bwd) for (int t = first; t < first + count - 1; ++t) push_kc(t, 0);
 				else for (int t = first + count - 1; t > first; --t) push_kc(t, 1);
-			} else { w[2 * nw] = first; w[2 * nw + 1] = (head_count == 0 && !bwd) ? -(count - 1) : count; ++nw; }
+			} else wk.push_back({first, (head_count == 0 && !bwd) ? -(count - 1) : count, (finish && !bwd && count <= 4) ? 2 : 1, i});
 		}
 	};
 	add_runs(kf, c->n_long_f, false);
 	add_runs(kb, c->n_long_b, true);
+	std::vector<int> fin((size_t)nc, -1);
+	{
+		auto by_kind = [](const Wk &x, const Wk &y) { return x.kind < y.kind; };
+		std::stable_sort(wk_f.begin(), wk_f.end(), by_kind); std::stable_sort(wk_b.begin(), wk_b.end(), by_kind);
+		c->n_wl_f = (int)wk_f.size(); c->n_wl_b = (int)wk_b.size();
+		c->n_hd_f = c->n_hd_b = c->n_mem_f = c->n_mem_f0 = c->n_mem_f0w = 0;
+		for (size_t i = 0; i < wk_f.size(); ++i) { wl[2 * i] = wk_f[i].first; wl[2 * i + 1] = wk_f[i].count; c->n_hd_f += wk_f[i].kind == 0; }
+		for (size_t i = 0; i < wk_b.size(); ++i) { wl[(size_t)2 * nc + 2 * i] = wk_b[i].first; wl[(size_t)2 * nc + 2 * i + 1] = wk_b[i].count; c->n_hd_b += wk_b[i].kind == 0; }
+		std::vector<char> fin_run((size_t)std::max(c->n_long_f, 1), 0), walked((size_t)std::max(c->n_long_f, 1), 0);
+		for (const Wk &x : wk_f) { if (x.kind == 2) fin_run[x.run] = 1; if (x.kind == 1) walked[x.run] = 1; }
+		auto put_run = [&](int i) {
+			for (int t = 0; t < kf[i].second.second; ++t) { mem[2 * (size_t)c->n_mem_f] = kf[i].second.first + t; mem[2 * (size_t)c->n_mem_f + 1] = 1; ++c->n_mem_f; }
+		};
+		for (int i = 0; i < c->n_long_f; ++i) if (!fin_run[i]) { put_run(i); if (walked[i]) c->n_mem_f0w += kf[i].second.second; }
+		c->n_mem_f0 = c->n_mem_f;
+		for (int r = 0; r < 5; ++r) c->n_fin_r[r] = 0;
+		for (size_t i = 0; i < wk_f.size(); ++i) if (wk_f[i].kind == 2) { fin[i] = c->n_mem_f; put_run(wk_f[i].run); c->n_fin_r[kf[wk_f[i].run].second.second] += 1; }
+	}
+	HIPCHK(c, hipMemcpy(c->d_items + (size_t)8 * nc, mem.data(), sizeof(int) * mem.size(), hipMemcpyHostToDevice));
+	HIPCHK(c, hipMemcpy(c->d_items + (size_t)32 * nc, fin.data(), sizeof(int) * fin.size(), hipMemcpyHostToDevice));
 	c->n_chain_f = (int)runs_f.size() / 4; c->n_chain_b = (int)runs_b.size() / 4; c->n_kc = (int)kc.size() / 2; c->n_kuniq = (int)kuniq.size();
 	if ((size_t)c->n_kc > (size_t)2 * nc || (size_t)(c->n_chain_f + c->n_chain_b) > (size_t)nc) return fail(c, PSMC_HIP_ESTATE, "build_items: list overflow");
 	HIPCHK(c, hipMemcpy(c->d_items + (size_t)12 * nc, wl.data(), sizeof(int) * wl.size(), hipMemcpyHostToDevice));
@@ -481,6 +499,8 @@
 	p.stream2 = c->stream2; p.stream3 = c->stream3; p.stream4 = c->stream4; p.overlap = c->overlap;
 	p.n_long_f = c->n_long_f; p.n_long_b = c->n_long_b; p.n_mem_f = c->n_mem_f; p.n_mem_b = c->n_mem_b;
 	p.d_members_f = c->d_items + 8 * p.n_chunks; p.d_members_b = c->d_items + 10 * p.n_chunks;
+	p.n_hd_f = c->n_hd_f; p.n_hd_b = c->n_hd_b; p.n_mem_f0 = c->n_mem_f0; p.n_mem_f0w = c->n_mem_f0w; p.d_wl_fin = c->d_items + 32 * (size_t)p.n_chunks;
+	p.walk_finish = c->walk_finish;
 	p.d_wl_f = c->d_items + 12 * (size_t)p.n_chunks; p.d_wl_b = c->d_items + 14 * (size_t)p.n_chunks; p.n_wl_f = c->n_wl_f; p.n_wl_b = c->n_wl_b;
 	p.d_kc = c->d_items + 16 * (size_t)p.n_chunks; p.d_kruns = c->d_items + 20 * (size_t)p.n_chunks;
 	p.n_kc = c->n_kc; p.n_chain_f = c->n_chain_f; p.n_chain_b = c->n_chain_b;
@@ -656,6 +676,15 @@
 	if (A0) memset(A0, 0, sizeof(double) * n);
 	if (chk) for (size_t i = 0; i < c->sel.size(); ++i) chk[i] = 1.0;
 	return PSMC_HIP_OK;
+}
+
+extern "C" int psmcdbg_fast_runs(psmc_hip_ctx *c, int out[8])
+{
+	if (!c || !out) return -1;
+	out[0] = c->n_fin_r[2]; out[1] = c->n_fin_r[3]; out[2] = c->n_fin_r[4];
+	out[3] = c->n_wl_f - c->n_hd_f - (c->n_fin_r[2] + c->n_fin_r[3] + c->n_fin_r[4]);
+	out[4] = c->n_chain_f; out[5] = c->n_chain_b; out[6] = c->n_hd_f; out[7] = c->n_hd_b;
+	return 0;
 }
 
 extern "C" int psmcdbg_check_bentry(psmc_hip_ctx *c)
diff --git a/psmc_amd/csrc/estep_fast.hip b/psmc_amd/csrc/estep_fast.hip
--- a/psmc_amd/csrc/estep_fast.hip
+++ b/psmc_amd/csrc/estep_fast.hip
@@ -456,13 +456,14 @@
 	const int ff0 = lf ? p.n_long_f : 0, fb0 = lb ? p.n_long_b : 0;
 	const bool mg = p.merge1 && p.structured && p.fused && ov;
 	hipStream_t sw = ov ? (mg ? sa : p.stream4) : sm, sk = ov ? p.stream5 : sm;
+	const bool wf = lw && lf && p.walk_finish && p.ns == 64 && p.fused == 1 && !p.ckpt && !p.merge && !mg && ov && sw != sk;
 	if (lw) {
 		if (ov && sw != sa) (void)hipStreamWaitEvent(sw, p.evx[0], 0);
-		launch_walks(p, sw);
+		launch_walks(p, sw, wf);
 	}
 	const bool gated = lw && ov && p.d_gate != nullptr && sw != sm;
 	const int rw = p.lanes8 && p.ns == 64 && p.fused ? 8 : 4;
-	if (gated) launch_gate(sm, p.d_gate, walk_blocks(p));
+	if (gated) launch_gate(sm, p.d_gate, walk_blocks(p, wf));
 	if (mg) {
 		launch_sweeps(p, sm, ff0, p.n_items_f - ff0, fb0, p.n_items_b - fb0 - p.n_B_b, true);
 		if (p.merge) launch_fwd_struct(p, sm, 6, 0, p.n_fix_f);
@@ -472,12 +473,22 @@
 		if (p.n_kc > 0) {
 			if (ov) (void)hipStreamWaitEvent(sk, p.evx[0], 0);
 			if (gated && sk != sm) launch_gate(sk, p.d_gate + 1, std::min(2048, mg ? (p.n_items_f - ff0 + rw - 1) / rw + (p.n_items_b - fb0 - p.n_B_b + rw - 1) / rw : (p.q_grid > 0 ? p.q_grid : (p.structured ? (p.n_items_f - ff0 + rw - 1) / rw : 0))));
-			launch_kchain(p, sk, sw, p.evx[8]);
-		}
-		(void)hipEventRecord(p.evx[6], sw);
-		if (lf) launch_fwd_struct(p, sw, 3, 0, p.n_mem_f);
-		(void)hipEventRecord(p.evx[7], sw);
-		if (ov) (void)hipStreamWaitEvent(sk, p.fused ? p.evx[7] : p.evx[6], 0);
+			launch_kchain(p, sk, wf ? sk : sw, p.evx[8], wf);
+		}
+		if (wf) {
+			(void)hipEventRecord(p.evx[13], sw);
+			if (p.n_kc <= 0) (void)hipStreamWaitEvent(sk, p.evx[0], 0);
+			if (p.n_mem_f0w > 0) (void)hipStreamWaitEvent(sk, p.evx[13], 0);
+			launch_fwd_struct(p, sk, 3, 0, p.n_mem_f0);
+			(void)hipStreamWaitEvent(sk, p.evx[13], 0);
+			(void)hipEventRecord(p.evx[6], sk);
+			(void)hipEventRecord(p.evx[7], sk);
+		} else {
+			(void)hipEventRecord(p.evx[6], sw);
+			if (lf) launch_fwd_struct(p, sw, 3, 0, p.n_mem_f);
+			(void)hipEventRecord(p.evx[7], sw);
+		}
+		if (ov && !wf) (void)hipStreamWaitEvent(sk, p.fused ? p.evx[7] : p.evx[6], 0);
 		if (lb && !p.fused) launch_bwd_struct(p, sk, 3, 0, p.n_mem_b);
 		if (p.fused != 2) (void)hipEventRecord(p.evx[9], sk);
 	}
diff --git a/psmc_amd/csrc/estep_struct.hip b/psmc_amd/csrc/estep_struct.hip
--- a/psmc_amd/csrc/estep_struct.hip
+++ b/psmc_amd/csrc/estep_struct.hip
@@ -505,18 +505,22 @@
 
 __device__ __forceinline__ double walk_ev(int sym, double e0, double e1) { return sym == 0 ? e0 : (sym == 1 ? e1 : 1.0); }
 
-__global__ __launch_bounds__(64) void k_walk1_struct(const double *__restrict__ sp, const double *__restrict__ e,
-                                                       const double *__restrict__ a0, const uint8_t *__restrict__ obs,
-                                                       const Chunk *__restrict__ chunks, const SweepItem *__restrict__ items_f,
-                                                       int n_f, const SweepItem *__restrict__ items_b, int n_b, int W, int T,
-                                                       double *__restrict__ entry, double *__restrict__ bentry,
-                                                       double *__restrict__ bexit, int *__restrict__ started)
-{
-	const int lane = threadIdx.x, block = (int)blockIdx.x;
-	announce_start(started);
+struct WalkArgs {
+	const double *sp, *e, *a0; const uint8_t *obs; const Chunk *chunks;
+	const SweepItem *items_f; int n_f; const SweepItem *items_b; int n_b; int W, T;
+	double *entry, *bentry, *bexit;
+};
+__device__ __forceinline__ void walk1_body(int lane, int block, int tblock, const WalkArgs &wa)
+{
+	const double *__restrict__ sp = wa.sp, *__restrict__ e = wa.e, *__restrict__ a0 = wa.a0;
+	const uint8_t *__restrict__ obs = wa.obs;
+	const Chunk *__restrict__ chunks = wa.chunks;
+	const SweepItem *__restrict__ items_f = wa.items_f, *__restrict__ items_b = wa.items_b;
+	const int n_f = wa.n_f, W = wa.W, T = wa.T;
+	double *__restrict__ entry = wa.entry, *__restrict__ bentry = wa.bentry, *__restrict__ bexit = wa.bexit;
 #ifdef PSMC_TRACE_SWEEP
-	PSMC_TRACE(g_trace_w, block, 0, wall_clock64()); PSMC_TRACE(g_trace_w, block, 3, trace_hw());
-	struct TraceEnd { int b; __device__ ~TraceEnd() { if (threadIdx.x == 0 && b < 16384) g_trace_w[4 * b + 2] = wall_clock64(); } } trace_end{block};
+	PSMC_TRACE(g_trace_w, tblock, 0, wall_clock64()); PSMC_TRACE(g_trace_w, tblock, 3, trace_hw());
+	struct TraceEnd { int b; __device__ ~TraceEnd() { if ((threadIdx.x & 63) == 0 && b < 16384) g_trace_w[4 * b + 2] = wall_clock64(); } } trace_end{tblock};
 #endif
 	__builtin_amdgcn_s_setprio(3);
 	const WaveScanMasks wm = wave_scan_masks(lane);
@@ -583,6 +587,27 @@
 	}
 }
 
+template <bool FINISH>
+__global__ __launch_bounds__(64) void k_walk1_struct(const WalkArgs wa, int *__restrict__ started, const int *__restrict__ fin,
+                                                       const SweepItem *__restrict__ members, double *__restrict__ f, double *__restrict__ invd,
+                                                       const FwdCtl ctl)
+{
+	const int lane = threadIdx.x, block = (int)blockIdx.x;
+	announce_start(started);
+	walk1_body(lane, block, block, wa);
+	if constexpr (FINISH) {
+		const int mo = block < wa.n_f ? fin[block] : -1;
+		if (mo >= 0) {
+			__threadfence_block();
+			fwd_struct_body<true, 4, false>(0, wa.sp, wa.e, wa.a0, wa.obs, wa.chunks, members + mo, 1 - wa.items_f[block].count, wa.W, wa.T,
+			                                SWEEP_FROM_ENTRY | SWEEP_NO_TOUCH, f, invd, wa.entry, nullptr, ctl);
+#ifdef PSMC_TRACE_SWEEP
+			PSMC_TRACE(g_trace_w, block, 1, wall_clock64());
+#endif
+		}
+	}
+}
+
 struct KcTile { int tile, dir; };
 __host__ __device__ inline void kc_range(const Chunk &c, int dir, int &lo, int &top)
 {
@@ -640,14 +665,21 @@
 template <int NQ>
 __global__ __launch_bounds__(64 * NQ) void k_kcol2_struct(const double *__restrict__ kcc, const uint8_t *__restrict__ obs,
                                                             const Chunk *__restrict__ chunks, const KcTile *__restrict__ kc, const int *__restrict__ uniq,
-                                                            double *__restrict__ Kcol, double *__restrict__ Kexp, int sub, int prio)
+                                                            double *__restrict__ Kcol, double *__restrict__ Kexp, int sub, int prio,
+                                                            const WalkArgs heads, int tr0)
 {
 	constexpr int S = 32 * NQ, NCG = S / 64, KD = 11 * S;
 	__shared__ double xch[2][NQ][2][64];
 	__shared__ double tab[KD];
 	const int lane = threadIdx.x & 63;
 	const int w = __builtin_amdgcn_readfirstlane((int)(threadIdx.x >> 6));
-	const int j = (int)blockIdx.x / NCG, cg = (int)blockIdx.x % NCG, jt = j / sub, js = j % sub;
+	const int n_heads = heads.n_f + heads.n_b;
+	if ((int)blockIdx.x < n_heads) {
+		if constexpr (NQ == 2) { if (w == 0) walk1_body(lane, (int)blockIdx.x, tr0 + (int)blockIdx.x, heads); }
+		return;
+	}
+	const int mb = (int)blockIdx.x - n_heads;
+	const int j = mb / NCG, cg = mb % NCG, jt = j / sub, js = j % sub;
 	const int col = 64 * cg + lane;
 	if (prio >= 2) __builtin_amdgcn_s_setprio(2); else if (prio == 1) __builtin_amdgcn_s_setprio(1);
 	const KcTile kt = kc[uniq[jt]];
@@ -1010,15 +1042,21 @@
 	return (int)hipGetLastError();
 }
 
-void launch_kchain(const EstepLaunch &p, hipStream_t st_cols, hipStream_t st_chain, hipEvent_t ev_cols)
+static WalkArgs walk_args(const EstepLaunch &p, int ff, int nf, int fb, int nb)
+{
+	return WalkArgs{p.d_sp, p.d_e, p.d_a0, p.d_obs, p.d_chunks, (const SweepItem *)p.d_wl_f + ff, nf, (const SweepItem *)p.d_wl_b + fb, nb,
+	                p.warmup, p.tile_len, p.d_entry, p.d_bentry, p.d_bexit};
+}
+void launch_kchain(const EstepLaunch &p, hipStream_t st_cols, hipStream_t st_chain, hipEvent_t ev_cols, bool heads)
 {
 	if (p.n_kc <= 0) return;
+	const WalkArgs hd = walk_args(p, 0, heads ? p.n_hd_f : 0, 0, heads ? p.n_hd_b : 0);
 	if (p.ns == 128)
 		hipLaunchKernelGGL(k_kcol_struct<8>, dim3(p.n_kuniq * 32), dim3(64), 0, st_cols, p.d_sp, p.d_e, p.d_obs, p.d_chunks,
 		                   (const KcTile *)p.d_kc, p.d_kuniq, p.d_Kcol, p.d_Kexp);
 	else
-		hipLaunchKernelGGL(k_kcol2_struct<2>, dim3(p.n_kuniq * p.kc_sub), dim3(128), 0, st_cols, p.d_kcc, p.d_obs, p.d_chunks, (const KcTile *)p.d_kc, p.d_kuniq,
-		                   p.d_Kcol, p.d_Kexp, p.kc_sub, p.kcol_prio);
+		hipLaunchKernelGGL(k_kcol2_struct<2>, dim3(hd.n_f + hd.n_b + p.n_kuniq * p.kc_sub), dim3(128), 0, st_cols, p.d_kcc, p.d_obs, p.d_chunks, (const KcTile *)p.d_kc, p.d_kuniq,
+		                   p.d_Kcol, p.d_Kexp, p.kc_sub, p.kcol_prio, hd, p.n_wl_f + p.n_wl_b - hd.n_f - hd.n_b);
 	if (st_cols != st_chain) { (void)hipEventRecord(ev_cols, st_cols); (void)hipStreamWaitEvent(st_chain, ev_cols, 0); }
 	if (p.ns == 128)
 		hipLaunchKernelGGL(k_kchain_struct<2>, dim3(p.n_chain_f + p.n_chain_b), dim3(512), 0, st_chain, (const KcRun *)p.d_kruns, p.n_chain_f, p.d_kslot,
@@ -1028,15 +1066,25 @@
 		                   p.d_Kcol, p.d_Kexp, p.d_sp, p.d_e, p.d_obs, p.d_chunks, p.d_entry, p.d_bentry, p.kc_sub);
 	PSMC_DBG("launch_kchain", p.n_kc, p.n_chain_f, p.n_chain_b);
 }
-int walk_blocks(const EstepLaunch &p) { return p.ns == 64 ? p.n_wl_f + p.n_wl_b : (p.n_wl_f + 3) / 4 + (p.n_wl_b + 3) / 4; }
-void launch_walks(const EstepLaunch &p, hipStream_t st)
-{
-	if (p.n_wl_f + p.n_wl_b <= 0) return;
+int walk_blocks(const EstepLaunch &p, bool finish)
+{
+	if (p.ns != 64) return (p.n_wl_f + 3) / 4 + (p.n_wl_b + 3) / 4;
+	return p.n_wl_f + p.n_wl_b - (finish ? p.n_hd_f + p.n_hd_b : 0);
+}
+void launch_walks(const EstepLaunch &p, hipStream_t st, bool finish)
+{
+	if (walk_blocks(p, finish) <= 0) return;
 	if (p.ns == 64) {
-		hipLaunchKernelGGL(k_walk1_struct, dim3(p.n_wl_f + p.n_wl_b), dim3(64), 0, st, p.d_sp, p.d_e, p.d_a0, p.d_obs, p.d_chunks,
-		                   (const SweepItem *)p.d_wl_f, p.n_wl_f, (const SweepItem *)p.d_wl_b, p.n_wl_b, p.warmup,
-		                   p.tile_len, p.d_entry, p.d_bentry, p.d_bexit, p.d_gate);
-		PSMC_DBG("launch_walks", p.n_wl_f, p.n_wl_b, 0);
+		const FwdCtl ctl = {nullptr, p.tol, nullptr, nullptr, p.d_fmerge, p.d_finv};
+		if (finish) {
+			const WalkArgs wa = walk_args(p, p.n_hd_f, p.n_wl_f - p.n_hd_f, p.n_hd_b, p.n_wl_b - p.n_hd_b);
+			hipLaunchKernelGGL(k_walk1_struct<true>, dim3(wa.n_f + wa.n_b), dim3(64), 0, st, wa, p.d_gate, p.d_wl_fin + p.n_hd_f,
+			                   (const SweepItem *)p.d_members_f, p.d_f, p.d_s, ctl);
+		} else {
+			const WalkArgs wa = walk_args(p, 0, p.n_wl_f, 0, p.n_wl_b);
+			hipLaunchKernelGGL(k_walk1_struct<false>, dim3(wa.n_f + wa.n_b), dim3(64), 0, st, wa, p.d_gate, nullptr, nullptr, nullptr, nullptr, ctl);
+		}
+		PSMC_DBG(finish ? "launch_walks (finish)" : "launch_walks", p.n_wl_f, p.n_wl_b, finish ? p.n_hd_f + p.n_hd_b : 0);
 		return;
 	}
 	hipLaunchKernelGGL(k_walk_struct<8>, dim3((p.n_wl_f + 3) / 4 + (p.n_wl_b + 3) / 4), dim3(64), 0, st, p.d_sp, p.d_e, p.d_a0, p.d_obs, p.d_chunks,
diff --git a/psmc_amd/csrc/psmc_hip_ctx.h b/psmc_amd/csrc/psmc_hip_ctx.h
--- a/psmc_amd/csrc/psmc_hip_ctx.h
+++ b/psmc_amd/csrc/psmc_hip_ctx.h
@@ -59,6 +59,9 @@
 	int warm_shift_used = 1, kc_sub_used = 4;
 	int kc_div = 16;
 	int kc_min = -1;
+	int walk_finish = 1;
+	int n_fin_r[5] = {0, 0, 0, 0, 0};
+	int n_hd_f = 0, n_hd_b = 0, n_mem_f0 = 0, n_mem_f0w = 0;
 	int n_wl_f = 0, n_wl_b = 0, n_kc = 0, n_chain_f = 0, n_chain_b = 0, n_singles_b = 0;
 	double *d_Kcol = nullptr; size_t kcol_cap = 0;
 	hipStream_t stream5 = nullptr;
diff --git a/psmc_amd/csrc/psmc_hip_internal.h b/psmc_amd/csrc/psmc_hip_internal.h
--- a/psmc_amd/csrc/psmc_hip_internal.h
+++ b/psmc_amd/csrc/psmc_hip_internal.h
@@ -78,6 +78,7 @@
 	int runs_in_b;
 	hipStream_t stream4, stream5;
 	const int *d_wl_f, *d_wl_b; int n_wl_f, n_wl_b;
+	int n_hd_f = 0, n_hd_b = 0, n_mem_f0 = 0, n_mem_f0w = 0, walk_finish = 0; const int *d_wl_fin = nullptr;
 	const int *d_kc, *d_kruns; int n_kc, n_chain_f, n_chain_b;
 	const int *d_kslot, *d_kuniq; int n_kuniq;
 	double *d_Kcol, *d_Kexp;
@@ -138,10 +139,10 @@
 void launch_compact(const EstepLaunch &p, hipStream_t st, bool bwd);
 void launch_gather_prev(const EstepLaunch &p, hipStream_t st, int first, int n_items, double *prevx);
 int launch_tile_allmiss(hipStream_t st, const uint8_t *d_obs, const Chunk *d_chunks, int n_chunks, int *d_flags);
-void launch_walks(const EstepLaunch &p, hipStream_t st);
+void launch_walks(const EstepLaunch &p, hipStream_t st, bool finish = false);
 void launch_gate(hipStream_t st, const int *ctr, int want);
-int walk_blocks(const EstepLaunch &p);
-void launch_kchain(const EstepLaunch &p, hipStream_t st_cols, hipStream_t st_chain, hipEvent_t ev_cols);
+int walk_blocks(const EstepLaunch &p, bool finish = false);
+void launch_kchain(const EstepLaunch &p, hipStream_t st_cols, hipStream_t st_chain, hipEvent_t ev_cols, bool heads = false);
 void launch_sweeps(const EstepLaunch &p, hipStream_t st, int ff, int nf, int fb, int nb, bool top_only);
 void launch_phase1_queue(const EstepLaunch &p, hipStream_t st, int ff, int nf, int fb, int nb);
 void launch_bwd_count(const EstepLaunch &p, hipStream_t st, int list, bool redo, bool all_from_bentry = false);
```

Result: slower. 2.372 billion bins/s (-3.0%).
